# PaddleCV-SIG/MedicalSeg

Hardware: AMD Instinct MI355X
Metric: 3D-voxels/sec fwd+bwd, VNet 128^3 fp32 (higher is better)
Workload: dtype f32

## Files before the change

include/msegk.h:

```cpp
#ifndef MSEGK_H
#define MSEGK_H

#include <stddef.h>
#include <stdint.h>

#ifdef __cplusplus
extern "C" {
#endif

typedef struct msk_ctx msk_ctx;

typedef struct {
  void* p;
  int32_t n, d, h, w, c;
  int32_t ld;
} msk_tensor;

typedef struct {
  int32_t kd, kh, kw;
  int32_t sd, sh, sw;
  int32_t pd, ph, pw;
} msk_conv_desc;

int msk_version(void);
// ... 20 lines not shown
int msk_timer_start(msk_ctx* ctx);
int msk_timer_stop(msk_ctx* ctx, float* ms);
int msk_mark(msk_ctx* ctx, int idx );
int msk_mark_elapsed(msk_ctx* ctx, int a, int b, float* ms);
int msk_ctx_wait(msk_ctx* ctx, msk_ctx* other);
int msk_prof_enable(msk_ctx* ctx, int on);
int msk_prof_reset(msk_ctx* ctx);
int msk_prof_report(msk_ctx* ctx, char* buf, int buflen, int* len);
int msk_set_option(msk_ctx* ctx, const char* key, int value);
int msk_get_option(msk_ctx* ctx, const char* key, int* value);

int msk_ncdhw_to_ndhwc(msk_ctx* ctx, const float* src, msk_tensor dst);
int msk_ndhwc_to_ncdhw(msk_ctx* ctx, msk_tensor src, float* dst);

int msk_conv3d_fwd(msk_ctx* ctx, msk_conv_desc cd, msk_tensor x, const float* w,
                   const float* bias , msk_tensor y);
int msk_conv_fold_bn(msk_ctx* ctx, const float* w, const float* bias, const float* scale, const float* shift,
                     int cout, long inner, float* w_folded, float* b_folded);
int msk_conv3d_fwd_act(msk_ctx* ctx, msk_conv_desc cd, msk_tensor x, const float* w, const float* bias,
                       const float* prelu_slope, msk_tensor y);
size_t msk_conv3d_xform_bytes(msk_ctx* ctx, msk_conv_desc cd, msk_tensor x, int cout);
int msk_conv3d_fwd_ex(msk_ctx* ctx, msk_conv_desc cd, msk_tensor x, const float* w, const float* bias ,
                      msk_tensor y, float* stats_local , void* xform );
int msk_conv3d_wgrad_ex(msk_ctx* ctx, msk_conv_desc cd, msk_tensor x, msk_tensor dy, float* dw, float* db ,
                        int accumulate, const void* xform );
float* msk_amax_new(msk_ctx* ctx, int n );
int msk_conv3d_fwd_ex2(msk_ctx* ctx, msk_conv_desc cd, msk_tensor x, const float* w, const float* bias ,
                       msk_tensor y, float* stats_local , void* xform , const float* x_amax );
int msk_affine_act_fwd_amax(msk_ctx* ctx, msk_tensor x, const float* scale, const float* shift, msk_tensor res,
                            const float* alpha, msk_tensor out, float* out_amax);
int msk_affine_act_join_fwd_amax(msk_ctx* ctx, msk_tensor y, const float* scale, const float* shift, const float* alpha_inner,
                                 msk_tensor res, const float* alpha_outer, msk_tensor out, float* out_amax);
int msk_copy_scale_amax(msk_ctx* ctx, msk_tensor src, const float* mask, msk_tensor dst, int accumulate, float* dst_amax);
int msk_conv3d_dgrad_ex(msk_ctx* ctx, msk_conv_desc cd, msk_tensor dy, const float* w, msk_tensor dx, int accumulate,
                        const float* dy_amax );
int msk_conv3d_wgrad_ex2(msk_ctx* ctx, msk_conv_desc cd, msk_tensor x, msk_tensor dy, float* dw, float* db ,
                         int accumulate, const void* xform , const float* dy_amax );
int msk_conv3d_wgrad_ex3(msk_ctx* ctx, msk_conv_desc cd, msk_tensor x, msk_tensor dy, float* dw, float* db ,
                         int accumulate, const void* xform , const float* dy_amax , const float* x_amax );
typedef struct msk_bn_fin {
  const float* gamma;
  const float* beta;
  float eps, momentum;
  double count;
  float* running_mean;
  float* running_var;
  float* save_mean;
  float* save_invstd;
  float* scale;
  float* shift;
} msk_bn_fin;
int msk_conv3d_fwd_ex3(msk_ctx* ctx, msk_conv_desc cd, msk_tensor x, const float* w, const float* bias ,
                       msk_tensor y, float* stats_local , void* xform , const float* x_amax ,
                       const msk_bn_fin* fin );
int msk_bn_stats_fin(msk_ctx* ctx, msk_tensor x, float* stats_local, const msk_bn_fin* fin );
int msk_conv3d_fwd_in(msk_ctx* ctx, msk_conv_desc cd, msk_tensor x, const float* w, const float* bias , msk_tensor y,
                      float* stats, void* xform , const float* x_amax , const msk_bn_fin* fin,
                      int fin_stride);
int msk_affine_act_bwd_reduce_pg(msk_ctx* ctx, msk_tensor x, const float* scale, const float* shift, msk_tensor res,
                                 const float* alpha, const float* mean, const float* invstd, msk_tensor dout, float* sums,
                                 float* maxes , int clear_maxes, float* dgamma, float* dbeta, float* dalpha);
int msk_add_act_join_bwd_pg(msk_ctx* ctx, msk_tensor y, const float* scale, const float* shift, const float* alpha_inner,
                            msk_tensor res, const float* alpha_outer, const float* mean, const float* invstd, msk_tensor dout,
                            msk_tensor da, msk_tensor dres, int dres_accumulate, float* dalpha_outer, float* unit_sums,
                            float* maxes , int clear_maxes, float* unit_dgamma, float* unit_dbeta, float* unit_dalpha);
size_t msk_conv3d_bwd_bnact_bytes(msk_ctx* ctx, msk_conv_desc cd, msk_tensor x, msk_tensor y);
int msk_conv3d_bwd_bnact(msk_ctx* ctx, msk_conv_desc cd, msk_tensor x, const float* w, msk_tensor y, const float* scale,
                         const float* shift, const float* alpha , const float* mean, const float* invstd,
                         const float* gamma, msk_tensor dout, const float* sums_total, double M_total,
                         msk_tensor dy_scratch, msk_tensor dx, int dx_accumulate, float* dw, int dw_accumulate,
                         const void* xform , void* ybuf ,
                         const float* maxes );
int msk_conv3d_bwd_bnact_split(msk_ctx* ctx, msk_conv_desc cd, msk_tensor x, const float* w, msk_tensor y, const float* scale,
                               const float* shift, const float* alpha , const float* mean, const float* invstd,
                               const float* gamma, msk_tensor dout, const float* sums_total, double M_total,
                               msk_tensor dy_scratch, msk_tensor dx, int dx_accumulate, float* dw, int dw_accumulate,
                               const void* xform , void* ybuf , const float* maxes ,
                               msk_tensor dx_lo, msk_tensor dx_hi, int* split_done);
int msk_conv3d_bwd_bnact_acc(msk_ctx* ctx, msk_conv_desc cd, msk_tensor x, const float* w, msk_tensor y, const float* scale,
                             const float* shift, const float* alpha, const float* mean, const float* invstd, const float* gamma,
                             msk_tensor dout, const float* sums_total, double M_total, msk_tensor dy_scratch, msk_tensor dx,
                             int dx_accumulate, float* dw, int dw_accumulate, const void* xform, void* ybuf, const float* maxes,
                             msk_tensor dx_old, msk_tensor dx_lo, msk_tensor dx_hi, int* split_done);
int msk_conv3d_bwd_bnact_join(msk_ctx* ctx, msk_conv_desc cd, msk_tensor x, const float* w, msk_tensor y, const float* scale,
                              const float* shift, const float* alpha , const float* mean, const float* invstd,
                              const float* gamma, msk_tensor dout, const float* sums_total, double M_total, msk_tensor dy,
                              float* dy_amax , float* dw, int dw_accumulate, const void* xform ,
                              const float* x_amax , msk_tensor jy, const float* jscale, const float* jshift,
                              const float* jalpha_inner, msk_tensor jres, const float* jalpha_outer, const float* jmean,
                              const float* jinvstd, msk_tensor da, int da_accumulate, msk_tensor dres ,
                              int dres_accumulate, float* dalpha_outer, float* unit_sums, float* maxes, int clear_maxes,
                              float* unit_dgamma , float* unit_dbeta , float* unit_dalpha );
int msk_convT3d_bwd_bnact(msk_ctx* ctx, msk_conv_desc cd, msk_tensor x, const float* w, msk_tensor y, const float* scale,
                          const float* shift, const float* alpha , const float* mean, const float* invstd,
                          msk_tensor dout, const float* sums_total, double M_total, msk_tensor dy_scratch, msk_tensor dx,
                          int dx_accumulate, float* dw, int dw_accumulate);
int msk_conv3d_bwd_inact(msk_ctx* ctx, msk_conv_desc cd, msk_tensor x, const float* w, msk_tensor y, const float* scale,
                         const float* shift, const float* alpha , const float* mean, const float* invstd, int coef_stride,
                         msk_tensor dout, const float* sums, int sums_stride, double M_sample, msk_tensor dx, int dx_accumulate,
                         float* dw, int dw_accumulate, const void* xform, void* ybuf, const float* maxes );
int msk_conv3d_bwd_bnact_c1(msk_ctx* ctx, msk_conv_desc cd, msk_tensor x, msk_tensor y, const float* scale, const float* shift,
                            const float* alpha , const float* mean, const float* invstd, msk_tensor res,
                            msk_tensor dout, const float* sums_total, double M_total, float* dw, int dw_accumulate);
int msk_conv3d_dgrad(msk_ctx* ctx, msk_conv_desc cd, msk_tensor dy, const float* w,
                     msk_tensor dx, int accumulate);
int msk_conv3d_wgrad(msk_ctx* ctx, msk_conv_desc cd, msk_tensor x, msk_tensor dy,
                     float* dw, float* db , int accumulate);
int msk_convT3d_fwd(msk_ctx* ctx, msk_conv_desc cd, msk_tensor x, const float* w,
                    const float* bias , msk_tensor y);
int msk_convT3d_fwd_ex(msk_ctx* ctx, msk_conv_desc cd, msk_tensor x, const float* w, const float* bias, msk_tensor y,
                       float* stats_local, const msk_bn_fin* fin );
int msk_convT3d_dgrad(msk_ctx* ctx, msk_conv_desc cd, msk_tensor dy, const float* w,
                      msk_tensor dx, int accumulate);
int msk_convT3d_wgrad(msk_ctx* ctx, msk_conv_desc cd, msk_tensor x, msk_tensor dy,
                      float* dw, float* db , int accumulate);

int msk_bn_stats(msk_ctx* ctx, msk_tensor x, float* stats_local);
int msk_bn_finalize(msk_ctx* ctx, const float* gathered, int world, double count_per_rank,
                    int C, const float* gamma, const float* beta, float eps, float momentum,
                    float* running_mean, float* running_var, float* save_mean,
                    float* save_invstd, float* scale, float* shift);
int msk_bn_eval_coeffs(msk_ctx* ctx, int C, const float* gamma, const float* beta,
                       const float* running_mean, const float* running_var, float eps,
                       float* save_mean, float* save_invstd, float* scale, float* shift);
int msk_affine_act_fwd(msk_ctx* ctx, msk_tensor x, const float* scale, const float* shift,
                       msk_tensor res, const float* alpha, msk_tensor out);
int msk_affine_act_fwd_amax2(msk_ctx* ctx, msk_tensor x, const float* scale, const float* shift, msk_tensor res,
                             const float* alpha, msk_tensor out, float* out_amax , msk_tensor out2);
int msk_affine_act_bwd_reduce(msk_ctx* ctx, msk_tensor x, const float* scale, const float* shift,
                              msk_tensor res, const float* alpha, const float* mean,
                              const float* invstd, msk_tensor dout, float* sums);
int msk_affine_act_bwd_reduce_ex(msk_ctx* ctx, msk_tensor x, const float* scale, const float* shift,
                                 msk_tensor res, const float* alpha, const float* mean,
                                 const float* invstd, msk_tensor dout, float* sums, float* maxes );
int msk_affine_act_bwd_apply(msk_ctx* ctx, msk_tensor x, const float* scale, const float* shift,
                             msk_tensor res, const float* alpha, const float* mean,
                             const float* invstd, const float* gamma, msk_tensor dout,
                             const float* sums_total, double M_total, int bn_mode,
                             msk_tensor dx, msk_tensor dres, int dres_acc);
int msk_affine_act_bwd_apply_amax(msk_ctx* ctx, msk_tensor x, const float* scale, const float* shift,
                                  msk_tensor res, const float* alpha, const float* mean,
                                  const float* invstd, const float* gamma, msk_tensor dout,
                                  const float* sums_total, double M_total, int bn_mode,
                                  msk_tensor dx, msk_tensor dres, int dres_acc, float* dx_amax );
int msk_affine_act_param_grads(msk_ctx* ctx, int C, const float* sums, float* dgamma,
                               float* dbeta, float* dalpha, int accumulate);

int msk_copy_scale(msk_ctx* ctx, msk_tensor src, const float* mask, msk_tensor dst, int accumulate);
int msk_dropout_mask(msk_ctx* ctx, uint64_t seed, uint64_t step, uint32_t site, int count,
                     float p, float* mask);
int msk_channel_sum(msk_ctx* ctx, msk_tensor x, float* out, int accumulate);
int msk_argmax_c(msk_ctx* ctx, msk_tensor x, int32_t* out);
int msk_softmax_c(msk_ctx* ctx, msk_tensor x, msk_tensor out);

int msk_flip_axes(msk_ctx* ctx, msk_tensor src, msk_tensor dst, int mask);
int msk_tta_accumulate(msk_ctx* ctx, msk_tensor logits, int mask, msk_tensor acc, int first);
int msk_tta_finish(msk_ctx* ctx, msk_tensor acc, int passes, msk_tensor probs, int32_t* pred);

int msk_sw_gather(msk_ctx* ctx, msk_tensor vol, msk_tensor patches, const int32_t* origins, float cval);
int msk_sw_accumulate(msk_ctx* ctx, msk_tensor logits, const int32_t* origins, const float* td, int nd, const float* th, int nh,
                      const float* tw, int nw, msk_tensor acc);

int msk_class_weights(msk_ctx* ctx, msk_tensor logits, float* weights);
int msk_loss_fwd(msk_ctx* ctx, msk_tensor logits, const int32_t* labels, const float* weights,
                 int ignore_index, float* out, double* stats);
int msk_loss_bwd(msk_ctx* ctx, msk_tensor logits, const int32_t* labels, const float* weights,
// ... 100 lines not shown
```

medicalseg_amd/_lib.py:

```python
from __future__ import annotations

import ctypes as C
import os

_HERE = os.path.dirname(os.path.abspath(__file__))
LIB_PATH = os.environ.get("MSEGK_LIB") or os.path.join(_HERE, "lib", "libmsegk.so")


class MskError(RuntimeError):
    pass


class MskTensor(C.Structure):
    _fields_ = [("p", C.c_void_p), ("n", C.c_int32), ("d", C.c_int32), ("h", C.c_int32),
                ("w", C.c_int32), ("c", C.c_int32), ("ld", C.c_int32)]


class MskConvDesc(C.Structure):
    _fields_ = [("kd", C.c_int32), ("kh", C.c_int32), ("kw", C.c_int32),
                ("sd", C.c_int32), ("sh", C.c_int32), ("sw", C.c_int32),
                ("pd", C.c_int32), ("ph", C.c_int32), ("pw", C.c_int32)]


class MskBnFin(C.Structure):
    _fields_ = [("gamma", C.c_void_p), ("beta", C.c_void_p), ("eps", C.c_float), ("momentum", C.c_float),
                ("count", C.c_double), ("running_mean", C.c_void_p), ("running_var", C.c_void_p),
                ("save_mean", C.c_void_p), ("save_invstd", C.c_void_p), ("scale", C.c_void_p), ("shift", C.c_void_p)]


NULL_TENSOR = MskTensor(None, 0, 0, 0, 0, 0, 0)

_vp, _i, _f, _d, _sz = C.c_void_p, C.c_int, C.c_float, C.c_double, C.c_size_t
_u64, _u32 = C.c_uint64, C.c_uint32
_T, _CD = MskTensor, MskConvDesc

SIGNATURES = {
    "msk_version": (_i, []),
    "msk_device_count": (_i, [C.POINTER(_i)]),
    "msk_ctx_create": (_i, [_i, C.POINTER(_vp)]),
    "msk_ctx_destroy": (_i, [_vp]),
    "msk_last_error": (C.c_char_p, [_vp]),
    "msk_sync": (_i, [_vp]),
    "msk_join_side": (_i, [_vp]),
    "msk_device_name": (_i, [_vp, C.c_char_p, _i]),
    "msk_device_pci_bus_id": (_i, [_vp, C.c_char_p, _i]),
    "msk_malloc": (_i, [_vp, _sz, C.POINTER(_vp)]),
    "msk_free": (_i, [_vp, _vp]),
    "msk_memset": (_i, [_vp, _vp, _i, _sz]),
    "msk_weights_changed": (_i, [_vp, _vp, _sz]),
    "msk_h2d": (_i, [_vp, _vp, _vp, _sz]),
    "msk_d2h": (_i, [_vp, _vp, _vp, _sz]),
    "msk_h2d_async": (_i, [_vp, _vp, _vp, _sz]),
    "msk_d2d": (_i, [_vp, _vp, _vp, _sz]),
    "msk_pinned_alloc": (_i, [_vp, _sz, C.POINTER(_vp)]),
    "msk_pinned_free": (_i, [_vp, _vp]),
    "msk_mem_info": (_i, [_vp, C.POINTER(_sz), C.POINTER(_sz)]),
    "msk_timer_start": (_i, [_vp]),
    "msk_timer_stop": (_i, [_vp, C.POINTER(_f)]),
    "msk_mark": (_i, [_vp, _i]),
    "msk_ctx_wait": (_i, [_vp, _vp]),
    "msk_mark_elapsed": (_i, [_vp, _i, _i, C.POINTER(_f)]),
    "msk_prof_enable": (_i, [_vp, _i]),
    "msk_prof_reset": (_i, [_vp]),
    "msk_prof_report": (_i, [_vp, C.c_char_p, _i, C.POINTER(_i)]),
    "msk_set_option": (_i, [_vp, C.c_char_p, _i]),
    "msk_get_option": (_i, [_vp, C.c_char_p, C.POINTER(_i)]),
    "msk_ncdhw_to_ndhwc": (_i, [_vp, _vp, _T]),
    "msk_ndhwc_to_ncdhw": (_i, [_vp, _T, _vp]),
    "msk_conv3d_fwd": (_i, [_vp, _CD, _T, _vp, _vp, _T]),
    "msk_conv_fold_bn": (_i, [_vp, _vp, _vp, _vp, _vp, _i, C.c_long, _vp, _vp]),
    "msk_conv3d_fwd_act": (_i, [_vp, _CD, _T, _vp, _vp, _vp, _T]),
    "msk_conv3d_xform_bytes": (_sz, [_vp, _CD, _T, _i]),
    "msk_conv3d_fwd_ex": (_i, [_vp, _CD, _T, _vp, _vp, _T, _vp, _vp]),
    "msk_conv3d_wgrad_ex": (_i, [_vp, _CD, _T, _T, _vp, _vp, _i, _vp]),
    "msk_amax_new": (_vp, [_vp, _i]),
    "msk_conv3d_fwd_ex3": (_i, [_vp, _CD, _T, _vp, _vp, _T, _vp, _vp, _vp, _vp]),
    "msk_conv3d_fwd_in": (_i, [_vp, _CD, _T, _vp, _vp, _T, _vp, _vp, _vp, _vp, _i]),
    "msk_bn_stats_fin": (_i, [_vp, _T, _vp, _vp]),
    "msk_affine_act_bwd_reduce_pg": (_i, [_vp, _T, _vp, _vp, _T, _vp, _vp, _vp, _T, _vp, _vp, _i, _vp, _vp, _vp]),
    "msk_add_act_join_bwd_pg": (_i, [_vp, _T, _vp, _vp, _vp, _T, _vp, _vp, _vp, _T, _T, _T, _i, _vp, _vp, _vp, _i, _vp, _vp, _vp]),
    "msk_conv3d_fwd_ex2": (_i, [_vp, _CD, _T, _vp, _vp, _T, _vp, _vp, _vp]),
    "msk_affine_act_fwd_amax": (_i, [_vp, _T, _vp, _vp, _T, _vp, _T, _vp]),
    "msk_affine_act_fwd_amax2": (_i, [_vp, _T, _vp, _vp, _T, _vp, _T, _vp, _T]),
    "msk_affine_act_join_fwd_amax": (_i, [_vp, _T, _vp, _vp, _vp, _T, _vp, _T, _vp]),
    "msk_copy_scale_amax": (_i, [_vp, _T, _vp, _T, _i, _vp]),
    "msk_conv3d_bwd_bnact_bytes": (_sz, [_vp, _CD, _T, _T]),
    "msk_conv3d_bwd_bnact": (_i, [_vp, _CD, _T, _vp, _T, _vp, _vp, _vp, _vp, _vp, _vp, _T, _vp, _d, _T, _T, _i, _vp, _i, _vp, _vp, _vp]),
    "msk_convT3d_bwd_bnact": (_i, [_vp, _CD, _T, _vp, _T, _vp, _vp, _vp, _vp, _vp, _T, _vp, _d, _T, _T, _i, _vp, _i]),
    "msk_conv3d_bwd_bnact_split": (_i, [_vp, _CD, _T, _vp, _T, _vp, _vp, _vp, _vp, _vp, _vp, _T, _vp, _d, _T, _T, _i, _vp, _i, _vp, _vp, _vp, _T, _T, C.POINTER(_i)]),
    "msk_conv3d_bwd_bnact_acc": (_i, [_vp, _CD, _T, _vp, _T, _vp, _vp, _vp, _vp, _vp, _vp, _T, _vp, _d, _T, _T, _i, _vp, _i, _vp, _vp, _vp, _T, _T, _T, C.POINTER(_i)]),
    "msk_conv3d_bwd_inact": (_i, [_vp, _CD, _T, _vp, _T, _vp, _vp, _vp, _vp, _vp, _i, _T, _vp, _i, _d, _T, _i, _vp, _i, _vp, _vp, _vp]),
    "msk_conv3d_bwd_bnact_join": (_i, [_vp, _CD, _T, _vp, _T, _vp, _vp, _vp, _vp, _vp, _vp, _T, _vp, _d, _T, _vp, _vp, _i, _vp, _vp,
                                       _T, _vp, _vp, _vp, _T, _vp, _vp, _vp, _T, _i, _T, _i, _vp, _vp, _vp, _i, _vp, _vp, _vp]),
    "msk_conv3d_bwd_bnact_c1": (_i, [_vp, _CD, _T, _T, _vp, _vp, _vp, _vp, _vp, _T, _T, _vp, _d, _vp, _i]),
    "msk_conv3d_dgrad": (_i, [_vp, _CD, _T, _vp, _T, _i]),
    "msk_conv3d_dgrad_ex": (_i, [_vp, _CD, _T, _vp, _T, _i, _vp]),
    "msk_conv3d_wgrad_ex2": (_i, [_vp, _CD, _T, _T, _vp, _vp, _i, _vp, _vp]),
    "msk_conv3d_wgrad_ex3": (_i, [_vp, _CD, _T, _T, _vp, _vp, _i, _vp, _vp, _vp]),
    "msk_conv3d_wgrad": (_i, [_vp, _CD, _T, _T, _vp, _vp, _i]),
    "msk_convT3d_fwd": (_i, [_vp, _CD, _T, _vp, _vp, _T]),
    "msk_convT3d_fwd_ex": (_i, [_vp, _CD, _T, _vp, _vp, _T, _vp, _vp]),
    "msk_convT3d_dgrad": (_i, [_vp, _CD, _T, _vp, _T, _i]),
    "msk_convT3d_wgrad": (_i, [_vp, _CD, _T, _T, _vp, _vp, _i]),
    "msk_bn_stats": (_i, [_vp, _T, _vp]),
    "msk_bn_finalize": (_i, [_vp, _vp, _i, _d, _i, _vp, _vp, _f, _f, _vp, _vp, _vp, _vp, _vp, _vp]),
    "msk_bn_eval_coeffs": (_i, [_vp, _i, _vp, _vp, _vp, _vp, _f, _vp, _vp, _vp, _vp]),
    "msk_affine_act_fwd": (_i, [_vp, _T, _vp, _vp, _T, _vp, _T]),
    "msk_affine_act_bwd_reduce": (_i, [_vp, _T, _vp, _vp, _T, _vp, _vp, _vp, _T, _vp]),
    "msk_affine_act_bwd_reduce_ex": (_i, [_vp, _T, _vp, _vp, _T, _vp, _vp, _vp, _T, _vp, _vp]),
    "msk_affine_act_bwd_apply": (_i, [_vp, _T, _vp, _vp, _T, _vp, _vp, _vp, _vp, _T, _vp, _d, _i, _T, _T, _i]),
    "msk_affine_act_bwd_apply_amax": (_i, [_vp, _T, _vp, _vp, _T, _vp, _vp, _vp, _vp, _T, _vp, _d, _i, _T, _T, _i, _vp]),
    "msk_affine_act_param_grads": (_i, [_vp, _i, _vp, _vp, _vp, _vp, _i]),
    "msk_add_act_bwd": (_i, [_vp, _T, _T, _vp, _T, _T, _T, _i, _vp]),
    "msk_affine_act_join_fwd": (_i, [_vp, _T, _vp, _vp, _vp, _T, _vp, _T]),
    "msk_add_act_join_bwd": (_i, [_vp, _T, _vp, _vp, _vp, _T, _vp, _T, _T, _T, _i, _vp]),
    "msk_add_act_join_bwd_ex": (_i, [_vp, _T, _vp, _vp, _vp, _T, _vp, _vp, _vp, _T, _T, _T, _i, _vp, _vp, _vp]),
    "msk_bn_bias_grad": (_i, [_vp, _i, _vp, _vp, _vp, _i]),
    "msk_copy_scale": (_i, [_vp, _T, _vp, _T, _i]),
    "msk_dropout_mask": (_i, [_vp, _u64, _u64, _u32, _i, _f, _vp]),
    "msk_channel_sum": (_i, [_vp, _T, _vp, _i]),
    "msk_argmax_c": (_i, [_vp, _T, _vp]),
    "msk_softmax_c": (_i, [_vp, _T, _T]),
    "msk_flip_axes": (_i, [_vp, _T, _T, _i]),
    "msk_tta_accumulate": (_i, [_vp, _T, _i, _T, _i]),
    "msk_tta_finish": (_i, [_vp, _T, _i, _T, _vp]),
    "msk_sw_gather": (_i, [_vp, _T, _T, _vp, _f]),
    "msk_sw_accumulate": (_i, [_vp, _T, _vp, _vp, _i, _vp, _i, _vp, _i, _T]),
    "msk_class_weights": (_i, [_vp, _T, _vp]),
    "msk_loss_fwd": (_i, [_vp, _T, _vp, _vp, _i, _vp, _vp]),
    "msk_loss_bwd": (_i, [_vp, _T, _vp, _vp, _i, _vp, _f, _f, _T]),
    "msk_elu_fwd": (_i, [_vp, _T, _f, _T]),
    "msk_elu_bwd": (_i, [_vp, _T, _T, _f, _T, _i]),
    "msk_loss_fwd_ex": (_i, [_vp, _T, _vp, _vp, _i, _i, _vp, _vp, _vp]),
    "msk_loss_bwd_ex": (_i, [_vp, _T, _vp, _vp, _i, _i, _vp, _vp, _f, _f, _T]),
    "msk_bce_fwd": (_i, [_vp, _T, _vp, _i, _i, _i, _f, _vp, _vp]),
    "msk_bce_bwd": (_i, [_vp, _T, _vp, _i, _vp, _f, _i, _T]),
    "msk_sgd_momentum": (_i, [_vp, _vp, _vp, _vp, _sz, _f, _f, _f, _f]),
    "msk_sgd_momentum_eager": (_i, [_vp, _vp, _vp, _vp, _sz, _f, _f, _f, _f]),
    "msk_sgd_momentum_finish": (_i, [_vp]),
    "msk_adam": (_i, [_vp, _vp, _vp, _vp, _vp, _sz, _f, _f, _f, _f, _d, _d, _f, _f]),
    "msk_resample3d": (_i, [_vp, _vp, _i, _i, _i, _vp, _i, _i, _i, _i, _i]),
    "msk_crop_resample3d": (_i, [_vp, _vp, _i, _i, _i, _i, _i, _i, _i, _i, _i, _vp, _i, _i, _i, _i, _i]),
    "msk_flip3d": (_i, [_vp, _vp, _vp, _i, _i, _i, _i, _i]),
    "msk_rotate3d": (_i, [_vp, _vp, _vp, _i, _i, _i, _i, _i, _d, _i, _d, _i]),
    "msk_hu_norm": (_i, [_vp, _vp, _vp, _sz, _f, _f, _f]),
    "msk_minmax_norm": (_i, [_vp, _vp, _vp, _sz, _i, _f, _f]),
    "msk_max_norm": (_i, [_vp, _vp, _vp, _sz]),
    "msk_label_remap": (_i, [_vp, _vp, _sz, _vp, _vp, _i]),
    "msk_connected_components3d": (_i, [_vp, _vp, _vp, _i, _i, _i, _i, _i, _i, _i, _vp, _vp]),
    "msk_confusion3d": (_i, [_vp, _vp, _vp, _i, C.c_long, _i, _i, _vp, _i]),
    "msk_auc_pack": (_i, [_vp, _T, _vp, _vp, C.c_long, C.c_long, _vp]),
    "msk_auc_workspace": (_i, [C.c_long, _i, C.POINTER(_sz)]),
    "msk_auc_counts": (_i, [_vp, _vp, C.c_long, C.c_long, _i, _vp, _sz, _vp]),
    "msk_edt3d": (_i, [_vp, _vp, _i, _i, _i, _i, _i, _vp, _vp]),
    "msk_surface_count": (_i, [_vp, _vp, _i, _i, _i, _i, _vp]),
    "msk_surface_gather": (_i, [_vp, _vp, _i, _i, _i, _i, _vp, _vp, C.c_long, _vp]),
    "msk_interp_trilinear_fwd": (_i, [_vp, _T, _T]),
    "msk_interp_scratch_bytes": (_i, [_vp, _T, _T, C.POINTER(_sz)]),
    "msk_interp_trilinear_bwd": (_i, [_vp, _T, _T, _i, _vp, _sz]),
    "msk_dp_unique_id": (_i, [C.c_char_p]),
    "msk_dp_rccl_version": (_i, [C.POINTER(_i)]),
    "msk_dp_init": (_i, [_vp, C.c_char_p, _i, _i]),
    "msk_dp_allreduce_sum": (_i, [_vp, _vp, _sz]),
    "msk_dp_allreduce_stats": (_i, [_vp, _vp, _sz]),
    "msk_dp_allreduce_async": (_i, [_vp, _vp, _sz]),
    "msk_dp_wait": (_i, [_vp]),
    "msk_dp_allgather": (_i, [_vp, _vp, _vp, _sz]),
    "msk_dp_broadcast": (_i, [_vp, _vp, _sz, _i]),
    "msk_dp_barrier": (_i, [_vp]),
    "msk_dp_destroy": (_i, [_vp]),
}

UNIQUE_ID_BYTES = 128
# ... 38 lines not shown
```

medicalseg_amd/csrc/msk_common.h:

```cpp
#pragma once
#include <hip/hip_runtime.h>
#include <hip/hip_ext.h>

#include <cstdint>
#include <cstdio>
#include <cstring>
#include <map>
#include <set>
#include <string>
#include <utility>
#include <vector>

#include "msegk.h"

struct msk_prof_entry {
  double total_ms = 0.0;
  long calls = 0;
};

struct msk_pending_event {
  hipEvent_t a, b;
  const char* tag;
};

// ... 27 lines not shown
  bool xform_written = false;
  std::set<const void*> xform_ok;
  bool conv_fp16 = false;
  int wbf_tin_map = 1;
  int wbf_mr4 = 1;
  int wbf_variant = -1;
  int halo_tile = -1;
  int wgrad_chunk = -1;
  char prof_prefix[48] = {0};
  long wgrad_async_max_m = 0;
  float* scalar_ring = nullptr;
  int scalar_next = 0;
  long scalar_served = 0;
  float* scalar_ring_side = nullptr;
  int scalar_next_side = 0;
  long scalar_served_side = 0;
  int wbf_tpb = 0;
  void* wpack = nullptr;
  int wbf_pack_cache = 1;
  void* spack = nullptr;
  int wbf_pack_lds = 1;
  int wbf_bpf = 1;
  int wbf_ks_blocks = 2;
  int noop_after_merge = 0;
  int wgrad_c1_wpc = 2;
  int eager_tail_main = 1;
  int prof_paused = 0;
  int prof_attach = 1;
  int small_pack_cache = 1;
  int wbf_prepack = 1;
  int ks_legacy = 0;
  int wgrad_fork = 1;
  int wbf_fused_bl = 2;
  int wbf_fuse = 1;
  int conv_split = 2;
  int bwd_fuse = -1;
  int foldn_wgs = 0;
  int wgrad_wino_rounds = 0;
  int wgrad_rounds = 8;
  int poison = -1;
  hipStream_t side = nullptr;
  void* ws_side = nullptr;
  size_t ws_side_bytes = 0;
  void* ws3_side = nullptr;
  size_t ws3_side_bytes = 0;
  hipEvent_t ev_fork = nullptr, ev_join = nullptr;
  hipEvent_t ev_late = nullptr;
  bool late_valid = false;
  const float* late_ptr = nullptr;
  size_t late_count = 0;
  float* late_alpha = nullptr;
  struct { float* param = nullptr; const float* grad = nullptr; float* velocity = nullptr; size_t count = 0;
           float lr = 0, momentum = 0, weight_decay = 0, grad_scale = 0; } late_piece;
  int late_split = 1;
  bool wgrad_async = false;
  bool side_dirty = false;
  hipEvent_t fork_event = nullptr;
  int fork_attach = 1;
  bool fork_recorded = false;
  void* stage[2] = {nullptr, nullptr};
  size_t stage_bytes[2] = {0, 0};
  hipEvent_t stage_ev[2] = {nullptr, nullptr};
  int stage_next = 0;
  void* comm = nullptr;
  void* comm_grad = nullptr;
  hipStream_t comm_stream = nullptr;
  hipEvent_t ev_comm_main = nullptr, ev_comm_side = nullptr, ev_comm_done = nullptr, ev_comm_back = nullptr;
  int c1_h2 = 1;
  int dst_split = 1;
  int wgrad_reduce_rows = 1;
  int ks_stats = 1;
  int ks_lds = 1;
  int ks_nr_max = 4;
  int wgrad_lds_pad = 0;
  int kst_pair = 1;
  int tile_staging = 7;
  int wgrad_renorm = 1;
  int dy_bound_shift = 0;
  int dp_mode = 0;
  bool comm_pending = false;
  bool host_transport = false;
  std::vector<int> host_fds;
  int rank = 0, world = 1;
  int tk_join = 1;
  int num_cu = 256;
};

extern thread_local std::string g_msk_global_err;

int msk_fail(msk_ctx* ctx, const char* file, int line, const char* what, const char* detail);
void* msk_workspace(msk_ctx* ctx, size_t bytes);
void* msk_workspace2(msk_ctx* ctx, size_t bytes);
void* msk_workspace3(msk_ctx* ctx, size_t bytes);
hipEvent_t msk_prof_event(msk_ctx* ctx);
void msk_prof_begin(msk_ctx* ctx, const char* tag);
void msk_prof_end(msk_ctx* ctx);
const char* msk_intern_tag(msk_ctx* ctx, const std::string& s);
int msk_join_side_impl(msk_ctx* ctx);
void msk_set_dense12(int v);
void msk_set_reduce_vpl(int v);
void msk_set_reduce_vpl_site(int v);
void msk_set_ew_caps(int ew, int red);
void msk_weights_changed_impl(msk_ctx* ctx, const void* p, size_t bytes);
void msk_weights_freed_impl(msk_ctx* ctx, const void* p, size_t bytes);
int msk_wbf_prepack_impl(msk_ctx* ctx);
int msk_wbf_prepack_range_impl(msk_ctx* ctx, const void* p, size_t bytes);
void msk_wbf_pack_cache_free(msk_ctx* ctx);
void msk_small_pack_changed(msk_ctx* ctx, const void* p, size_t bytes);
void msk_small_pack_freed(msk_ctx* ctx, const void* p, size_t bytes);
int msk_small_prepack(msk_ctx* ctx, const void* p, size_t bytes);
void msk_small_pack_free(msk_ctx* ctx);
int msk_dp_wait_impl(msk_ctx* ctx);
int msk_join_sums_merge(msk_ctx* ctx, const float* partial, int nb, int C, float* unit_sums, float* u_dbeta, float* u_dgamma,
                        float* u_dalpha, float* dalpha);

struct msk_side_scope {
  msk_ctx* ctx;
  bool active;
  explicit msk_side_scope(msk_ctx* c, bool want = true) : ctx(c), active(want && c->wgrad_async && c->side != nullptr) {
    const bool forked = ctx->fork_recorded;
    hipEvent_t fev = forked && ctx->fork_event ? ctx->fork_event : ctx->ev_fork;
    ctx->fork_recorded = false;
    ctx->fork_event = nullptr;
    if (!active) return;
    if (!forked) hipEventRecord(ctx->ev_fork, ctx->stream);
    hipStreamWaitEvent(ctx->side, fev, 0);
    std::swap(ctx->stream, ctx->side);
    std::swap(ctx->ws, ctx->ws_side);
    std::swap(ctx->ws_bytes, ctx->ws_side_bytes);
    std::swap(ctx->ws3, ctx->ws3_side);
    std::swap(ctx->ws3_bytes, ctx->ws3_side_bytes);
    std::swap(ctx->scalar_ring, ctx->scalar_ring_side);
    std::swap(ctx->scalar_next, ctx->scalar_next_side);
    std::swap(ctx->scalar_served, ctx->scalar_served_side);
    ctx->side_dirty = true;
  }
  ~msk_side_scope() {
    if (!active) return;
    std::swap(ctx->stream, ctx->side);
    std::swap(ctx->ws, ctx->ws_side);
    std::swap(ctx->ws_bytes, ctx->ws_side_bytes);
    std::swap(ctx->ws3, ctx->ws3_side);
    std::swap(ctx->ws3_bytes, ctx->ws3_side_bytes);
    std::swap(ctx->scalar_ring, ctx->scalar_ring_side);
    std::swap(ctx->scalar_next, ctx->scalar_next_side);
    std::swap(ctx->scalar_served, ctx->scalar_served_side);
  }
};

#define MSK_CHECK_HIP(ctx, expr)                                                        \
  do {                                                                                  \
    hipError_t _e = (expr);                                                             \
    if (_e != hipSuccess) return msk_fail(ctx, __FILE__, __LINE__, #expr, hipGetErrorString(_e)); \
  } while (0)

#define MSK_REQUIRE(ctx, cond, msg)                                       \
  do {                                                                    \
    if (!(cond)) return msk_fail(ctx, __FILE__, __LINE__, #cond, msg);    \
  } while (0)

static inline bool msk_prof_selected(const msk_ctx* c, const char* tag) {
  return c->prof && ((!c->prof_paused && (c->prof_prefix[0] == 0 || strncmp(tag, c->prof_prefix, strlen(c->prof_prefix)) == 0)) ||
                     strncmp(tag, "rccl_", 5) == 0);
}
struct msk_launch_scope {
  msk_ctx* ctx;
// ... 71 lines not shown
```

medicalseg_amd/csrc/msk_conv.h:

```cpp
#pragma once
#include "msk_common.h"
struct WbfBnBwd;

struct GConv {
  const float* src;
  int sld;
  float* dst;
  int dld;
  int N, SD, SH, SW, DD, DH, DW;
  int CK, CN;
  int kd, kh, kw, sd, sh, sw, pd, ph, pw;
  int transposed;
  const float* bias;
  int accumulate;
  int flip;
  float* stats;
  void* xform;
  const float* w_amax;
  const float* in_amax;
  const struct WbfBnBwd* fuse;
  const msk_bn_fin* fin;
  int ck_real;
  int stats_ps;
  int fin_stride;
  bool w_persistent;
  float* dst_lo;
  float* dst_hi;
  int dst_csplit;
  const float* acc_src;
  const float* prelu;
};

struct WGrad {
  const float* A;
  int ald;
  const float* B;
  int bld;
  int N, AD, AH, AW, BD, BH, BW;
  int CA, CB;
  int kd, kh, kw, sd, sh, sw, pd, ph, pw;
  const void* xform;
  const void* yform;
  const float* y_amax;
  const float* y_cmax;
  const float* b_amax;
  int cb_real;
  const float* a_amax;
  const struct WbfBnBwd* yfuse;
  float* dw;
  int accumulate;
  float* db;
  int db_src;
  long vsn;
  int vsd, vsh, vsw;
};

int msk_pack_weights(msk_ctx* ctx, const float* w, int A, int B, int taps, int swap, int flip_taps,
                     int kd, int kh, int kw, int mfma, int K, int N, int KC, int npad, float* out);

const float* msk_pack_weights_get(msk_ctx* ctx, const float* w, int A, int B, int taps, int swap, int flip_taps, int kd, int kh,
                                  int kw, int mfma, int K, int N, int KC, int npad);
const float* msk_pack_scatter_get(msk_ctx* ctx, const float* w, int A, int B, int taps, int swap, int CK, int CN, int KC, int jpad);

int msk_gconv_halo_mfma(msk_ctx* ctx, const GConv& g, const float* w_canon, int A, int B, int swap);
int msk_gconv_gather_mfma(msk_ctx* ctx, const GConv& g, const float* w_canon, int A, int B, int swap);
int msk_gconv_halo_tightk(msk_ctx* ctx, const GConv& g, const float* w_canon, int A, int B, int swap);
int msk_gconv_tk_h2(msk_ctx* ctx, const GConv& g, const float* w_canon, int A, int B, int swap, struct TKJoin* join = nullptr);
struct TKJoin {
  const float* x;
  int xld;
  const float* b;
  int bld;
  float* db;
  int dbld;
  const float *scale, *shift, *alpha_in, *alpha, *mean, *invstd;
  float* maxes;
  const float* partial;
  int nb;
};
bool msk_gconv_tk_h2_accepts(const msk_ctx* ctx, const GConv& g, const struct TKJoin* join);
int msk_gconv_c1_mfma(msk_ctx* ctx, const GConv& g, const float* w_canon, int A, int B, int swap);
int msk_gconv_c1_h2(msk_ctx* ctx, const GConv& g, const float* w_canon, int A, int B, int swap);
int msk_gconv_halo_valu2(msk_ctx* ctx, const GConv& g, const float* w_canon, int A, int B, int swap);
int msk_gconv_halo_foldn(msk_ctx* ctx, const GConv& g, const float* w_canon, int A, int B, int swap, bool* act_fused);
int msk_gconv_halo_wino(msk_ctx* ctx, const GConv& g, const float* w_canon, int A, int B, int swap);
int msk_gconv_wino_bf3(msk_ctx* ctx, const GConv& g, const float* w_canon, int A, int B, int swap);
bool msk_gconv_wino_bf3_accepts(msk_ctx* ctx, const GConv& g);
int msk_wgrad_wbf(msk_ctx* ctx, const WGrad& g);
bool msk_wgrad_wbf_accepts(msk_ctx* ctx, const WGrad& g);
bool msk_wgrad_wbf_fusable(msk_ctx* ctx, const WGrad& g, size_t* y_bytes);
int msk_gconv_scatter_mfma(msk_ctx* ctx, const GConv& g, const float* w_canon, int A, int B, int swap);
int msk_gconv_ks_fwd(msk_ctx* ctx, const GConv& g, const float* w_canon, int A, int B, int swap);
int msk_gconv_ks_fwd_bnbwd(msk_ctx* ctx, const GConv& g, const float* w_canon, int A, int B, int swap, const float* y, int yld,
                           const float* dout, int dld, const float* scale, const float* shift, const float* alpha, const float* mean,
                           const float* invstd, const float* sums, double M_total, bool dry);
int msk_gconv_kst(msk_ctx* ctx, const GConv& g, const float* w_canon, int A, int B, int swap);
int msk_wgrad_mfma(msk_ctx* ctx, const WGrad& g);
bool msk_gconv_foldn_h2_accepts(const msk_ctx* ctx, msk_conv_desc cd, msk_tensor x, int cout);
int msk_wgrad_cbs(msk_ctx* ctx, const WGrad& g);
int msk_wgrad_c1(msk_ctx* ctx, const WGrad& g);
int msk_wgrad_ks(msk_ctx* ctx, const WGrad& g);
int msk_wgrad_wino(msk_ctx* ctx, const WGrad& g);

const float* msk_absmax(msk_ctx* ctx, const float* x, int ld, int C, long voxels, float* dst = nullptr);
float* msk_scalar_slots(msk_ctx* ctx, int n);
const float* msk_bn_bwd_bound(msk_ctx* ctx, int C, const float* scale, const float* sums, double M_total, const float* maxes);
int msk_wgrad_reduce_ex(msk_ctx* ctx, const float* partial, int splits, long pitch, int taps, int CA, int CB, float* dw,
                        int accumulate, int nbias, float* db, int db_accumulate);
int msk_wgrad_reduce(msk_ctx* ctx, const float* partial, int splits, int taps, int CA, int CB, float* dw,
                     int accumulate);
```

medicalseg_amd/csrc/msk_conv.hip:

```cpp
#include "msk_conv.h"
#include "msk_wbf.h"

namespace {

constexpr int kThreads = 256;

__device__ __forceinline__ float pack_weights_elem(const float* __restrict__ w, int B, int taps, int swap, int flip, int kd, int kh,
                                                   int kw, int mfma, int K, int N, int KC, int npad, long idx) {
  int tap, k, n;
  if (mfma) {
    int q = (int)(idx & 3);
    long r = idx >> 2;
    n = (int)(r % npad);
    r /= npad;
    int h = (int)(r & 1);
    r >>= 1;
    int kc = (int)(r % KC);
    tap = (int)(r / KC);
    k = kc * 8 + h * 4 + q;
  } else {
    const int NP = npad > 0 ? npad : N;
    n = (int)(idx % NP);
    long r = idx / NP;
    k = (int)(r % K);
// ... 1467 lines not shown
int msk_conv3d_wgrad(msk_ctx* ctx, msk_conv_desc cd, msk_tensor x, msk_tensor dy, float* dw, float* db, int accumulate) {
  if (check_conv_shapes(ctx, cd, x, dy, false) != 0) return -1;
  msk_side_scope side(ctx, ctx->wgrad_async_max_m <= 0 || msk_voxels(dy) <= ctx->wgrad_async_max_m);
  WGrad g{};
  g.A = (const float*)x.p; g.ald = x.ld; g.B = (const float*)dy.p; g.bld = dy.ld;
  g.N = x.n; g.AD = x.d; g.AH = x.h; g.AW = x.w; g.BD = dy.d; g.BH = dy.h; g.BW = dy.w;
  g.CA = x.c; g.CB = dy.c;
  g.kd = cd.kd; g.kh = cd.kh; g.kw = cd.kw; g.sd = cd.sd; g.sh = cd.sh; g.sw = cd.sw;
  g.pd = cd.pd; g.ph = cd.ph; g.pw = cd.pw;
  g.dw = dw; g.accumulate = accumulate;
  return run_wgrad(ctx, g, dy, db, accumulate);
}

}

static int bwd_bnact_c1(msk_ctx* ctx, const WGrad& gw, msk_tensor y, const float* scale, const float* shift, const float* alpha,
                        const float* mean, const float* invstd, msk_tensor dout, const float* sums_total, double M_total,
                        int res_is_input) {
  if (ctx->bwd_fuse == 0 || ctx->conv_impl != 0) return 1;
  if (gw.BW * 4 < ((gw.BW + 31) / 32) * 32 * 3) return 1;
  WbfBnBwd bn{};
  bn.y = (const float*)y.p; bn.yld = y.ld; bn.dout = (const float*)dout.p; bn.dld = dout.ld;
  bn.scale = scale; bn.shift = shift; bn.alpha = alpha; bn.mean = mean; bn.invstd = invstd; bn.sums = sums_total;
  bn.invM = (float)(1.0 / M_total);
  bn.res_is_input = res_is_input;
  WGrad gc = gw;
  gc.B = nullptr;
  gc.xform = nullptr;
  gc.yfuse = &bn;
  if (ctx->late_split && ctx->wgrad_async && ctx->side != nullptr) {
    msk_side_scope side(ctx, true);
    if (side.active) {
      if (!ctx->late_alpha) MSK_CHECK_HIP(ctx, hipMalloc((void**)&ctx->late_alpha, 1024 * sizeof(float)));
      if (alpha && gw.CB <= 1024) {
        MSK_CHECK_HIP(ctx, hipMemcpyAsync(ctx->late_alpha, alpha, (size_t)gw.CB * sizeof(float), hipMemcpyDeviceToDevice, ctx->stream));
        bn.alpha = ctx->late_alpha;
      }
      hipEventRecord(ctx->ev_late, ctx->stream);
    }
    const int r = msk_wgrad_c1(ctx, gc);
    if (r == 1 && side.active) {
      ctx->late_valid = true;
      ctx->late_ptr = gw.dw;
      ctx->late_count = (size_t)gw.CA * gw.CB * gw.kd * gw.kh * gw.kw;
    }
    return r < 0 ? r : (r == 1 ? 0 : 1);
  }
  const int r = msk_wgrad_c1(ctx, gc);
  return r < 0 ? r : (r == 1 ? 0 : 1);
}

extern "C" {

int msk_conv3d_bwd_bnact_c1(msk_ctx* ctx, msk_conv_desc cd, msk_tensor x, msk_tensor y, const float* scale, const float* shift,
                            const float* alpha, const float* mean, const float* invstd, msk_tensor res, msk_tensor dout,
                            const float* sums_total, double M_total, float* dw, int dw_accumulate) {
  if (check_conv_shapes(ctx, cd, x, y, false) != 0) return -1;
  MSK_REQUIRE(ctx, scale && shift && mean && invstd && sums_total && M_total > 0, "training-mode BatchNorm coefficients required");
  MSK_REQUIRE(ctx, dout.n == y.n && dout.d == y.d && dout.h == y.h && dout.w == y.w && dout.c == y.c, "dout must match y");
  if (x.c != 1) return 1;
  if (res.p && !(res.p == x.p && res.ld == x.ld && res.c == 1 && res.n == x.n && res.d == x.d && res.h == x.h && res.w == x.w)) return 1;
  const size_t per = (size_t)x.d * x.h * x.w * (x.ld > y.ld ? x.ld : y.ld) * sizeof(float);
  if (per > 0 && (size_t)x.n > kChunkBytes / per) return 1;
  WGrad gw{};
  gw.A = (const float*)x.p; gw.ald = x.ld; gw.bld = y.ld;
  gw.N = x.n; gw.AD = x.d; gw.AH = x.h; gw.AW = x.w; gw.BD = y.d; gw.BH = y.h; gw.BW = y.w;
  gw.CA = x.c; gw.CB = y.c;
  gw.kd = cd.kd; gw.kh = cd.kh; gw.kw = cd.kw; gw.sd = cd.sd; gw.sh = cd.sh; gw.sw = cd.sw;
  gw.pd = cd.pd; gw.ph = cd.ph; gw.pw = cd.pw;
  gw.dw = dw; gw.accumulate = dw_accumulate;
  return bwd_bnact_c1(ctx, gw, y, scale, shift, alpha, mean, invstd, dout, sums_total, M_total, res.p ? 1 : 0);
}

size_t msk_conv3d_bwd_bnact_bytes(msk_ctx* ctx, msk_conv_desc cd, msk_tensor x, msk_tensor y) {
  if (x.c != y.c || x.d != y.d || x.h != y.h || x.w != y.w) return 0;
  return msk_conv3d_xform_bytes(ctx, cd, y, y.c);
}

static int conv3d_bwd_bnact_impl(msk_ctx* ctx, msk_conv_desc cd, msk_tensor x, const float* w, msk_tensor y, const float* scale,
                                 const float* shift, const float* alpha, const float* mean, const float* invstd, const float* gamma,
                                 msk_tensor dout, const float* sums_total, double M_total, msk_tensor dy_scratch, msk_tensor dx,
                                 int dx_accumulate, float* dw, int dw_accumulate, const void* xform, void* ybuf, const float* maxes,
                                 int coef_stride, int sums_stride, bool fused_only, float* dx_lo = nullptr, float* dx_hi = nullptr,
                                 int dx_csplit = 0, const float* dx_old = nullptr);

int msk_conv3d_bwd_bnact(msk_ctx* ctx, msk_conv_desc cd, msk_tensor x, const float* w, msk_tensor y, const float* scale,
                         const float* shift, const float* alpha, const float* mean, const float* invstd, const float* gamma,
                         msk_tensor dout, const float* sums_total, double M_total, msk_tensor dy_scratch, msk_tensor dx,
                         int dx_accumulate, float* dw, int dw_accumulate, const void* xform, void* ybuf, const float* maxes) {
  return conv3d_bwd_bnact_impl(ctx, cd, x, w, y, scale, shift, alpha, mean, invstd, gamma, dout, sums_total, M_total, dy_scratch, dx,
                               dx_accumulate, dw, dw_accumulate, xform, ybuf, maxes, 0, 0, false);
}

int msk_conv3d_bwd_bnact_split(msk_ctx* ctx, msk_conv_desc cd, msk_tensor x, const float* w, msk_tensor y, const float* scale,
                               const float* shift, const float* alpha, const float* mean, const float* invstd, const float* gamma,
                               msk_tensor dout, const float* sums_total, double M_total, msk_tensor dy_scratch, msk_tensor dx,
                               int dx_accumulate, float* dw, int dw_accumulate, const void* xform, void* ybuf, const float* maxes,
                               msk_tensor dx_lo, msk_tensor dx_hi, int* split_done) {
  MSK_REQUIRE(ctx, split_done != nullptr, "msk_conv3d_bwd_bnact_split: split_done required");
  *split_done = 0;
  const bool ok = dx.p && dx_lo.p && dx_hi.p && dx.c % 2 == 0 && dx_lo.c == dx.c / 2 && dx_hi.c == dx.c / 2 && dx_lo.ld == dx.c / 2 &&
                  dx_hi.ld == dx.c / 2 && dx.ld == dx.c && msk_voxels(dx_lo) == msk_voxels(dx) && msk_voxels(dx_hi) == msk_voxels(dx) &&
                  dx_accumulate && ctx->dst_split != 0;
  const int rc = conv3d_bwd_bnact_impl(ctx, cd, x, w, y, scale, shift, alpha, mean, invstd, gamma, dout, sums_total, M_total, dy_scratch, dx,
                                       dx_accumulate, dw, dw_accumulate, xform, ybuf, maxes, 0, 0, false, ok ? (float*)dx_lo.p : nullptr,
                                       ok ? (float*)dx_hi.p : nullptr, ok ? dx.c / 2 : 0);
  if (rc == 0 && ctx->dst_split_done) *split_done = 1;
  ctx->dst_split_done = false;
  return rc;
}

int msk_conv3d_bwd_bnact_acc(msk_ctx* ctx, msk_conv_desc cd, msk_tensor x, const float* w, msk_tensor y, const float* scale,
                             const float* shift, const float* alpha, const float* mean, const float* invstd, const float* gamma,
                             msk_tensor dout, const float* sums_total, double M_total, msk_tensor dy_scratch, msk_tensor dx,
                             int dx_accumulate, float* dw, int dw_accumulate, const void* xform, void* ybuf, const float* maxes,
                             msk_tensor dx_old, msk_tensor dx_lo, msk_tensor dx_hi, int* split_done) {
  if (split_done) *split_done = 0;
  if (dx_old.p) {
    MSK_REQUIRE(ctx, dx.p && dx_old.n == dx.n && dx_old.d == dx.d && dx_old.h == dx.h && dx_old.w == dx.w && dx_old.c == dx.c &&
                         dx_old.ld == dx.ld && dx_old.p != dx.p, "dx_old must have the geometry and voxel stride of dx");
    dx_accumulate = 1;
  }
  const bool ok = split_done && dx.p && dx_lo.p && dx_hi.p && dx.c % 2 == 0 && dx_lo.c == dx.c / 2 && dx_hi.c == dx.c / 2 &&
                  dx_lo.ld == dx.c / 2 && dx_hi.ld == dx.c / 2 && dx.ld == dx.c && msk_voxels(dx_lo) == msk_voxels(dx) &&
                  msk_voxels(dx_hi) == msk_voxels(dx) && dx_accumulate && ctx->dst_split != 0;
  const int rc = conv3d_bwd_bnact_impl(ctx, cd, x, w, y, scale, shift, alpha, mean, invstd, gamma, dout, sums_total, M_total, dy_scratch, dx,
                                       dx_accumulate, dw, dw_accumulate, xform, ybuf, maxes, 0, 0, false, ok ? (float*)dx_lo.p : nullptr,
                                       ok ? (float*)dx_hi.p : nullptr, ok ? dx.c / 2 : 0, (const float*)dx_old.p);
  if (rc == 0 && ok && ctx->dst_split_done) *split_done = 1;
  ctx->dst_split_done = false;
  return rc;
}

int msk_conv3d_bwd_bnact_join(msk_ctx* ctx, msk_conv_desc cd, msk_tensor x, const float* w, msk_tensor y, const float* scale,
                              const float* shift, const float* alpha, const float* mean, const float* invstd, const float* gamma,
                              msk_tensor dout, const float* sums_total, double M_total, msk_tensor dy, float* dy_amax, float* dw,
                              int dw_accumulate, const void* xform, const float* x_amax, msk_tensor jy, const float* jscale,
                              const float* jshift, const float* jalpha_inner, msk_tensor jres, const float* jalpha_outer,
                              const float* jmean, const float* jinvstd, msk_tensor da, int da_accumulate, msk_tensor dres,
                              int dres_accumulate, float* dalpha_outer, float* unit_sums, float* maxes, int clear_maxes,
                              float* unit_dgamma, float* unit_dbeta, float* unit_dalpha) {
  if (check_conv_shapes(ctx, cd, x, y, false) != 0) return -1;
  MSK_REQUIRE(ctx, scale && shift && mean && invstd && sums_total && M_total > 0 && w && dw, "training-mode BatchNorm coefficients required");
  MSK_REQUIRE(ctx, dy.p && dy.n == y.n && dy.d == y.d && dy.h == y.h && dy.w == y.w && dy.c == y.c, "dy must match y");
  MSK_REQUIRE(ctx, jscale && jshift && jalpha_inner && jalpha_outer && jmean && jinvstd && dalpha_outer && unit_sums && maxes,
              "the join's coefficients, statistics, sums and maxima buffers");
  const bool same = jy.n == x.n && jy.d == x.d && jy.h == x.h && jy.w == x.w && jy.c == x.c && jres.n == x.n && jres.d == x.d &&
                    jres.h == x.h && jres.w == x.w && jres.c == x.c && da.n == x.n && da.d == x.d && da.h == x.h && da.w == x.w &&
                    da.c == x.c && jy.p && jres.p && da.p;
  MSK_REQUIRE(ctx, same, "the join's tensors must have the shape of x");
  MSK_REQUIRE(ctx, !dres.p || (dres.n == x.n && dres.d == x.d && dres.h == x.h && dres.w == x.w && dres.c == x.c), "dres must have the shape of x");
  if (ctx->conv_impl != 0 || x.c != 32 || da_accumulate || (dres.p && dres_accumulate)) return 1;
  GConv g{};
  g.src = (const float*)dy.p; g.sld = dy.ld; g.dst = (float*)da.p; g.dld = da.ld;
  g.N = x.n; g.SD = dy.d; g.SH = dy.h; g.SW = dy.w; g.DD = x.d; g.DH = x.h; g.DW = x.w;
  g.CK = dy.c; g.CN = x.c;
  g.kd = cd.kd; g.kh = cd.kh; g.kw = cd.kw; g.sd = cd.sd; g.sh = cd.sh; g.sw = cd.sw;
  g.pd = cd.pd; g.ph = cd.ph; g.pw = cd.pw;
  g.transposed = 1; g.bias = nullptr; g.accumulate = 0; g.flip = 1;
  g.w_persistent = true;
  g.in_amax = dy_amax;
  TKJoin j{};
  j.x = (const float*)jy.p; j.xld = jy.ld; j.b = (const float*)jres.p; j.bld = jres.ld;
  j.scale = jscale; j.shift = jshift; j.alpha_in = jalpha_inner; j.alpha = jalpha_outer; j.mean = jmean; j.invstd = jinvstd;
  j.maxes = maxes;
  j.db = (float*)dres.p; j.dbld = dres.ld;
  const size_t per = (size_t)x.d * x.h * x.w * (x.ld > da.ld ? x.ld : da.ld) * sizeof(float);
  if (per > 0 && (size_t)x.n > kChunkBytes / per) return 1;
  if ((size_t)x.n * x.d * x.h * x.w >= (1ull << 31) / 64) return 1;
  if (!msk_gconv_tk_h2_accepts(ctx, g, &j)) return 1;
  if (int rc = msk_affine_act_bwd_apply_amax(ctx, y, scale, shift, msk_tensor{}, alpha, mean, invstd, gamma, dout, sums_total, M_total, 1,
                                             dy, msk_tensor{}, 0, dy_amax))
    return rc;
  if (int rc = conv3d_wgrad_impl(ctx, cd, x, dy, dw, nullptr, dw_accumulate, xform, dy_amax, x_amax)) return rc;
  if (clear_maxes) MSK_CHECK_HIP(ctx, hipMemsetAsync(maxes, 0, 2 * kWbfAmaxWays * sizeof(float), ctx->stream));
  const int r = msk_gconv_tk_h2(ctx, g, w, dy.c, x.c, 0, &j);
  if (r < 0) return r;
  if (r == 0) return msk_fail(ctx, __FILE__, __LINE__, "msk_conv3d_bwd_bnact_join", "the data-gradient kernel declined a problem its plan accepted");
  return msk_join_sums_merge(ctx, j.partial, j.nb, x.c, unit_sums, unit_dbeta, unit_dgamma, unit_dalpha, dalpha_outer);
}

int msk_conv3d_bwd_inact(msk_ctx* ctx, msk_conv_desc cd, msk_tensor x, const float* w, msk_tensor y, const float* scale,
                         const float* shift, const float* alpha, const float* mean, const float* invstd, int coef_stride,
                         msk_tensor dout, const float* sums, int sums_stride, double M_sample, msk_tensor dx, int dx_accumulate,
                         float* dw, int dw_accumulate, const void* xform, void* ybuf, const float* maxes) {
  MSK_REQUIRE(ctx, coef_stride >= y.c && sums_stride >= 2 * y.c, "msk_conv3d_bwd_inact: strides smaller than the records");
  return conv3d_bwd_bnact_impl(ctx, cd, x, w, y, scale, shift, alpha, mean, invstd, nullptr, dout, sums, M_sample, msk_tensor{}, dx,
                               dx_accumulate, dw, dw_accumulate, xform, ybuf, maxes, coef_stride, sums_stride, true);
}

static int conv3d_bwd_bnact_impl(msk_ctx* ctx, msk_conv_desc cd, msk_tensor x, const float* w, msk_tensor y, const float* scale,
                                 const float* shift, const float* alpha, const float* mean, const float* invstd, const float* gamma,
                                 msk_tensor dout, const float* sums_total, double M_total, msk_tensor dy_scratch, msk_tensor dx,
                                 int dx_accumulate, float* dw, int dw_accumulate, const void* xform, void* ybuf, const float* maxes,
                                 int coef_stride, int sums_stride, bool fused_only, float* dx_lo, float* dx_hi, int dx_csplit,
                                 const float* dx_old) {
  if (check_conv_shapes(ctx, cd, x, y, false) != 0) return -1;
  ctx->dst_split_done = false;
  if (!dx_accumulate || !dx.p) dx_old = nullptr;
  MSK_REQUIRE(ctx, scale && shift && mean && invstd && sums_total && M_total > 0, "training-mode BatchNorm coefficients required");
  MSK_REQUIRE(ctx, dout.n == y.n && dout.d == y.d && dout.h == y.h && dout.w == y.w && dout.c == y.c, "dout must match y");
  MSK_REQUIRE(ctx, fused_only || (dy_scratch.p && dy_scratch.n == y.n && dy_scratch.d == y.d && dy_scratch.h == y.h && dy_scratch.w == y.w &&
                                  dy_scratch.c == y.c), "dy_scratch must match y");
  if (xform && !ctx->xform_ok.count(xform)) xform = nullptr;
  const bool split2 = wbf_pieces(ctx, cd.kd) != 3;
  bool fused = ctx->bwd_fuse != 0 && (!split2 || maxes != nullptr) && ybuf != nullptr && xform != nullptr && dx.p != nullptr && ctx->wbf && !ctx->no_winograd && ctx->conv_impl == 0 &&
               x.c == y.c && y.ld % 4 == 0 && dout.ld % 4 == 0 && (((uintptr_t)y.p) & 15) == 0 && (((uintptr_t)dout.p) & 15) == 0;
  const size_t per = (size_t)x.d * x.h * x.w * (x.ld > y.ld ? x.ld : y.ld) * sizeof(float);
  if (per > 0 && (size_t)x.n > kChunkBytes / per) fused = false;
  WGrad gw{};
  gw.A = (const float*)x.p; gw.ald = x.ld; gw.B = (const float*)dy_scratch.p; gw.bld = dy_scratch.ld;
  gw.N = x.n; gw.AD = x.d; gw.AH = x.h; gw.AW = x.w; gw.BD = y.d; gw.BH = y.h; gw.BW = y.w;
  gw.CA = x.c; gw.CB = y.c;
  gw.kd = cd.kd; gw.kh = cd.kh; gw.kw = cd.kw; gw.sd = cd.sd; gw.sh = cd.sh; gw.sw = cd.sw;
  gw.pd = cd.pd; gw.ph = cd.ph; gw.pw = cd.pw;
  gw.dw = dw; gw.accumulate = dw_accumulate;
  gw.xform = xform;
  if (x.c == 1 && !dx.p && !fused_only && !(per > 0 && (size_t)x.n > kChunkBytes / per)) {
    const int r = bwd_bnact_c1(ctx, gw, y, scale, shift, alpha, mean, invstd, dout, sums_total, M_total, 0);
    if (r <= 0) return r;
  }
  size_t y_bytes = 0;
  if (fused && !msk_wgrad_wbf_fusable(ctx, gw, &y_bytes)) fused = false;
  if (fused) {
    GConv g{};
    g.src = (const float*)dy_scratch.p; g.sld = dy_scratch.ld; g.dst = (float*)dx.p; g.dld = dx.ld;
    g.N = dx.n; g.SD = y.d; g.SH = y.h; g.SW = y.w; g.DD = dx.d; g.DH = dx.h; g.DW = dx.w;
    g.CK = y.c; g.CN = dx.c;
    g.kd = cd.kd; g.kh = cd.kh; g.kw = cd.kw; g.sd = cd.sd; g.sh = cd.sh; g.sw = cd.sw;
    g.pd = cd.pd; g.ph = cd.ph; g.pw = cd.pw;
    g.transposed = 1; g.bias = nullptr; g.accumulate = dx_accumulate; g.flip = 1;
    g.w_persistent = true;
    g.dst_lo = dx_lo; g.dst_hi = dx_hi; g.dst_csplit = dx_csplit;
    g.acc_src = dx_old;
    WbfBnBwd bn{};
    bn.y = (const float*)y.p; bn.yld = y.ld; bn.dout = (const float*)dout.p; bn.dld = dout.ld;
    bn.scale = scale; bn.shift = shift; bn.alpha = alpha; bn.mean = mean; bn.invstd = invstd; bn.sums = sums_total;
    bn.invM = (float)(1.0 / M_total);
    bn.Y = (char*)ybuf;
    bn.coef_stride = coef_stride; bn.sums_stride = sums_stride;
    bn.y_xi = (long)(y_bytes / ((cd.kd == 5) ? 8 : 6));
    if (split2) g.w_amax = (const float*)xform + kWbfAmaxWays;

    const bool side_on = ctx->wgrad_async && ctx->side != nullptr &&
                         (ctx->wgrad_async_max_m <= 0 || msk_voxels(y) <= ctx->wgrad_async_max_m);
    int form = ctx->bwd_fuse > 0 ? ctx->bwd_fuse : ((side_on && !split2) ? 2 : 1);
    if (fused_only) form = 1;
    if (fused_only && split2 && !maxes) return 1;
    if (wbf_pieces(ctx, cd.kd) == 2 && form == 1) {
      bn.y_cmax = msk_scalar_slots(ctx, (y.c + kWbfAmaxWays - 1) / kWbfAmaxWays);
      if (!bn.y_cmax) return -1;
    }
    if (split2) {
      if (form == 1) {
        float* slot = msk_scalar_slots(ctx, 1);
        if (!slot) return -1;
        bn.amax = slot;
        bn.maxes = maxes;
      } else {
        bn.amax = msk_bn_bwd_bound(ctx, y.c, scale, sums_total, M_total, maxes);
        if (!bn.amax) return -1;
      }
    }
    if (form == 2) {
      bn.Y = nullptr;
      g.fuse = &bn;
      if (msk_gconv_wino_bf3_accepts(ctx, g)) {
        {
          msk_side_scope side(ctx, side_on);
          gw.yfuse = &bn;
          const int rw = msk_wgrad_wbf(ctx, gw);
          if (rw < 0) return rw;
          if (rw == 0) return msk_fail(ctx, __FILE__, __LINE__, "msk_conv3d_bwd_bnact", "weight-gradient pipeline declined a problem its plan accepted");
        }
        const int r = msk_gconv_wino_bf3(ctx, g, w, y.c, x.c, 0);
        if (r < 0) return r;
        if (r == 0) return msk_fail(ctx, __FILE__, __LINE__, "msk_conv3d_bwd_bnact", "data-gradient pipeline declined a problem its plan accepted");
        return 0;
      }
    } else {
      g.fuse = &bn;
      const int r = msk_gconv_wino_bf3(ctx, g, w, y.c, x.c, 0);
      if (r < 0) return r;
      if (r == 1) {
        msk_side_scope side(ctx, side_on);
        gw.yform = ybuf;
        gw.y_amax = bn.amax;
        gw.y_cmax = bn.y_cmax;
        const int rw = msk_wgrad_wbf(ctx, gw);
        if (rw < 0) return rw;
        if (rw == 0) return msk_fail(ctx, __FILE__, __LINE__, "msk_conv3d_bwd_bnact", "weight-gradient pipeline declined a problem its plan accepted");
        return 0;
      }
    }
  }
  if (fused_only) return 1;
  (void)gamma;
  if (dx_old) {
    msk_tensor so = dx;
    so.p = (void*)dx_old;
    if (int rc = msk_copy_scale(ctx, so, nullptr, dx, 0)) return rc;
  }
  if (int rc = msk_affine_act_bwd_apply(ctx, y, scale, shift, msk_tensor{}, alpha, mean, invstd, gamma, dout, sums_total, M_total, 1,
                                        dy_scratch, msk_tensor{}, 0))
    return rc;
  const float* dy_amax = nullptr;
  if (ctx->conv_split == 2 && ctx->conv_impl == 0 && y.c <= 4 && cd.kd == 5 && cd.kh == 5 && cd.kw == 5) {
    dy_amax = msk_absmax(ctx, (const float*)dy_scratch.p, dy_scratch.ld, dy_scratch.c, msk_voxels(dy_scratch));
    if (!dy_amax) return -1;
  }
  if (int rc = conv3d_wgrad_impl(ctx, cd, x, dy_scratch, dw, nullptr, dw_accumulate, xform, dy_amax)) return rc;
  if (dx.p) return conv3d_dgrad_impl(ctx, cd, dy_scratch, w, dx, dx_accumulate, dy_amax);
  return 0;
}

int msk_convT3d_fwd(msk_ctx* ctx, msk_conv_desc cd, msk_tensor x, const float* w, const float* bias, msk_tensor y) {
  if (check_conv_shapes(ctx, cd, x, y, true) != 0) return -1;
  GConv g{};
  g.src = (const float*)x.p; g.sld = x.ld; g.dst = (float*)y.p; g.dld = y.ld;
  g.N = x.n; g.SD = x.d; g.SH = x.h; g.SW = x.w; g.DD = y.d; g.DH = y.h; g.DW = y.w;
  g.CK = x.c; g.CN = y.c;
  g.kd = cd.kd; g.kh = cd.kh; g.kw = cd.kw; g.sd = cd.sd; g.sh = cd.sh; g.sw = cd.sw;
  g.pd = 0; g.ph = 0; g.pw = 0;
  g.transposed = 1; g.bias = bias; g.accumulate = 0; g.flip = 0;
  return run_gconv(ctx, g, w, x.c, y.c, 0, "convT3d_fwd_direct");
}

int msk_convT3d_fwd_ex(msk_ctx* ctx, msk_conv_desc cd, msk_tensor x, const float* w, const float* bias, msk_tensor y,
                       float* stats_local, const msk_bn_fin* fin) {
  if (check_conv_shapes(ctx, cd, x, y, true) != 0) return -1;
  if (fin && !fin->scale) fin = nullptr;
  MSK_REQUIRE(ctx, stats_local != nullptr, "msk_convT3d_fwd_ex: stats_local required");
  GConv g{};
  g.src = (const float*)x.p; g.sld = x.ld; g.dst = (float*)y.p; g.dld = y.ld;
  g.N = x.n; g.SD = x.d; g.SH = x.h; g.SW = x.w; g.DD = y.d; g.DH = y.h; g.DW = y.w;
  g.CK = x.c; g.CN = y.c;
  g.kd = cd.kd; g.kh = cd.kh; g.kw = cd.kw; g.sd = cd.sd; g.sh = cd.sh; g.sw = cd.sw;
  g.pd = 0; g.ph = 0; g.pw = 0;
  g.transposed = 1; g.bias = bias; g.accumulate = 0; g.flip = 0;
  g.w_persistent = true;
  const size_t sper = (size_t)g.SD * g.SH * g.SW * g.sld * sizeof(float), dper = (size_t)g.DD * g.DH * g.DW * g.dld * sizeof(float);
  const size_t per = sper > dper ? sper : dper;
  const bool chunked = per > 0 && (size_t)g.N > kChunkBytes / per;
  ctx->stats_fused = false;
  if (!chunked) {
    g.stats = stats_local;
    g.fin = fin;
  }
  if (int rc = run_gconv(ctx, g, w, x.c, y.c, 0, "convT3d_fwd_direct")) return rc;
  if (!ctx->stats_fused) return msk_bn_stats_fin(ctx, y, stats_local, fin);
  return 0;
}

int msk_convT3d_dgrad(msk_ctx* ctx, msk_conv_desc cd, msk_tensor dy, const float* w, msk_tensor dx, int accumulate) {
  if (check_conv_shapes(ctx, cd, dx, dy, true) != 0) return -1;
  GConv g{};
  g.src = (const float*)dy.p; g.sld = dy.ld; g.dst = (float*)dx.p; g.dld = dx.ld;
  g.N = dx.n; g.SD = dy.d; g.SH = dy.h; g.SW = dy.w; g.DD = dx.d; g.DH = dx.h; g.DW = dx.w;
  g.CK = dy.c; g.CN = dx.c;
  g.kd = cd.kd; g.kh = cd.kh; g.kw = cd.kw; g.sd = cd.sd; g.sh = cd.sh; g.sw = cd.sw;
  g.pd = 0; g.ph = 0; g.pw = 0;
  g.transposed = 0; g.bias = nullptr; g.accumulate = accumulate; g.flip = 0;
  return run_gconv(ctx, g, w, dx.c, dy.c, 1, "convT3d_dgrad_direct");
}

int msk_convT3d_bwd_bnact(msk_ctx* ctx, msk_conv_desc cd, msk_tensor x, const float* w, msk_tensor y, const float* scale,
                          const float* shift, const float* alpha, const float* mean, const float* invstd, msk_tensor dout,
                          const float* sums_total, double M_total, msk_tensor dy, msk_tensor dx, int dx_accumulate, float* dw,
                          int dw_accumulate) {
  if (check_conv_shapes(ctx, cd, x, y, true) != 0) return -1;
  MSK_REQUIRE(ctx, scale && shift && mean && invstd && sums_total && w && dw, "msk_convT3d_bwd_bnact: null argument");
  MSK_REQUIRE(ctx, dout.c == y.c && msk_voxels(dout) == msk_voxels(y) && dy.c == y.c && msk_voxels(dy) == msk_voxels(y) &&
                       dx.c == x.c && msk_voxels(dx) == msk_voxels(x), "msk_convT3d_bwd_bnact: shape mismatch");
  GConv g{};
  g.src = (const float*)y.p; g.sld = y.ld; g.dst = (float*)dx.p; g.dld = dx.ld;
  g.N = dx.n; g.SD = y.d; g.SH = y.h; g.SW = y.w; g.DD = dx.d; g.DH = dx.h; g.DW = dx.w;
  g.CK = y.c; g.CN = dx.c;
  g.kd = cd.kd; g.kh = cd.kh; g.kw = cd.kw; g.sd = cd.sd; g.sh = cd.sh; g.sw = cd.sw;
  g.transposed = 0; g.bias = nullptr; g.accumulate = dx_accumulate; g.flip = 0;
// ... 39 lines not shown
```

medicalseg_amd/csrc/msk_conv_wbf.hip:

```cpp
#include <type_traits>
#include "msk_wbf.h"
#ifndef WBF_TIN_SYNC
#define WBF_TIN_SYNC 1
#endif

#ifndef WBF_PROBE
#define WBF_PROBE 0
#endif
typedef _Float16 f16x8 __attribute__((ext_vector_type(8)));
typedef _Float16 f16x2 __attribute__((ext_vector_type(2)));

namespace {

constexpr int nxi_of(int K) { return K == 5 ? 8 : 6; }

__device__ __forceinline__ void split3_one(float x, unsigned short& hi, unsigned short& mid, unsigned short& lo) {
  hi = __builtin_bit_cast(unsigned short, (__bf16)x);
  const float r = x - __uint_as_float((unsigned)hi << 16);
  mid = __builtin_bit_cast(unsigned short, (__bf16)r);
  const float r2 = r - __uint_as_float((unsigned)mid << 16);
  lo = __builtin_bit_cast(unsigned short, (__bf16)r2);
}
__device__ __forceinline__ unsigned pack_f16_pair(float a, float b) {
  f32x2 v = {a, b};
// ... 740 lines not shown
      const int cur = tap & 1, nx = cur ^ 1;
      const int bcur = tap % BR;
      if (tap + BPF < T2) {
        const unsigned ub = (unsigned)(tap + BPF) * utap + ukc;
#pragma unroll
        for (int p = 0; p < NP; ++p) {
          bq[(tap + BPF) % BR][p] = buf_load16(ures, ulane, ub + p * ustep);
        }
      }
      if (tap + 1 < T2) {
#pragma unroll
        for (int mr = 0; mr < MR; ++mr) {
          const uint4* ap = lds + arow[mr] + ((tap + 1) / K) * HPt + ((tap + 1) % K);
#pragma unroll
          for (int p = 0; p < NP; ++p) {
            aq[nx][mr][p] = ap[p * 2 * NSLOT];
          }
        }
      }
      __builtin_amdgcn_sched_barrier(0);
      if (NP == 3) {
#pragma unroll
        for (int mr = 0; mr < MR; ++mr) WBF_MFMA(acc[mr], aq[cur][mr][NP - 1], bq[bcur][0]);
#pragma unroll
        for (int mr = 0; mr < MR; ++mr) WBF_MFMA(acc[mr], aq[cur][mr][0], bq[bcur][NP - 1]);
#pragma unroll
        for (int mr = 0; mr < MR; ++mr) WBF_MFMA(acc[mr], aq[cur][mr][NP / 2], bq[bcur][NP / 2]);
#pragma unroll
        for (int mr = 0; mr < MR; ++mr) WBF_MFMA(acc[mr], aq[cur][mr][NP / 2], bq[bcur][0]);
#pragma unroll
        for (int mr = 0; mr < MR; ++mr) WBF_MFMA(acc[mr], aq[cur][mr][0], bq[bcur][NP / 2]);
#pragma unroll
        for (int mr = 0; mr < MR; ++mr) WBF_MFMA(acc[mr], aq[cur][mr][0], bq[bcur][0]);
      } else if (NP == 2) {
        const uint4 bdown = wbf_hi_down(bq[bcur][0]);
#pragma unroll
        for (int mr = 0; mr < MR; ++mr) WBF_MFMA_H(acc[mr], aq[cur][mr][NP - 1], bdown);
#pragma unroll
        for (int mr = 0; mr < MR; ++mr) WBF_MFMA_H(acc[mr], aq[cur][mr][0], bq[bcur][NP - 1]);
#pragma unroll
        for (int mr = 0; mr < MR; ++mr) WBF_MFMA_H(acc[mr], aq[cur][mr][0], bq[bcur][0]);
      } else {
#pragma unroll
        for (int mr = 0; mr < MR; ++mr) WBF_MFMA_H(acc[mr], aq[cur][mr][0], bq[bcur][0]);
      }
      __builtin_amdgcn_sched_barrier(0);
    }
  }

  const int co = (grp * WN + wn) * 32 + li;
  float* mbase = a.M + ((long)ks * NXI + xi) * a.m_xi + ((long)(n * a.T + t) * a.LD) * a.LH * a.CN + co;
#pragma unroll
  for (int mr = 0; mr < MR; ++mr) {
#pragma unroll
    for (int j = 0; j < 16; ++j) {
      int fa, fb;
      frag_pos<TH>((j & 3) + 8 * (j >> 2) + 4 * lh, fa, fb);
      const int d = tdi * TD + (wm * MR + mr) * (32 / TH) + fa, h = thi * TH + fb;
      if (d < a.LD && h < a.LH) mbase[((long)d * a.LH + h) * a.CN] = acc[mr][j];
    }
  }
  }
}

struct FusedArgs {
  GemmArgs g;
  float* dst;
  int dld;
  long dvn;
  int dvd, dvh, dvw;
  const float* bias;
  const float* prelu;
  int accumulate;
  const float* in_amax;
  const float* w_amax;
  int scaled;
  float* stat_partial;
  int per_xcd;
  int LW;
  float* st_lo;
  float* st_hi;
  int csplit;
  const float* acc_src;
};

struct WfRec {
  float n, mean, m2;
};
__device__ __forceinline__ WfRec wfrec_merge(WfRec a, WfRec b) {
  if (b.n == 0.f) return a;
  if (a.n == 0.f) return b;
  WfRec r;
  r.n = a.n + b.n;
  const float d = b.mean - a.mean, f = b.n / r.n;
  r.mean = a.mean + d * f;
  r.m2 = a.m2 + b.m2 + d * d * a.n * f;
  return r;
}

template <int K>
__device__ __forceinline__ void at_column(int xi, float& c0, float& c1, float& c2, float& c3) {
  const int last = K == 5 ? 7 : 5;
  c0 = xi == last ? 0.f : 1.f;
  if (xi == 0) { c1 = c2 = c3 = 0.f; return; }
  if (xi == last) { c1 = c2 = 0.f; c3 = 1.f; return; }
  const float sg = (xi & 1) ? 1.f : -1.f;
  const int pr = (xi - 1) >> 1;
  const float p = pr == 0 ? 1.f : (pr == 1 ? 2.f : 0.5f);
  c1 = sg * p;
  c2 = p * p;
  c3 = sg * p * p * p;
}

#ifndef WBF_FUSED_BPF
#define WBF_FUSED_BPF 3
#endif
template <int MR, int WM, int WN, int TD, int TH, int K, int NP, bool STATS, int BPF = (NP == 2 ? WBF_FUSED_BPF : 1), int BL = 0>
__global__ void __launch_bounds__(WM * WN * 64, 2)
wbf_gemm_fused_k(FusedArgs f) {
  static_assert(WM * WN == 4 && WM * MR * 32 == TD * TH, "tile shape");
  const GemmArgs& a = f.g;
  constexpr int NT = WM * WN * 64;
  constexpr int NXI = nxi_of(K), T2 = K * K, PADK = (K - 1) / 2;
  constexpr int HDt = TD + K - 1, HPt = TH + K - 1, NSLOT = HDt * HPt, NPL = 2 * NP, NIT = NPL * NSLOT, ROUNDS = (NIT + NT - 1) / NT;
  constexpr int NBF = T2 * NP;
  constexpr int BROUNDS = (NBF + WM * WN - 1) / (WM * WN);
  static_assert(BL == 0 || NIT % 64 == 0, "weights through LDS: wave-granular tile");
  static_assert(BL != 1 || WN == 1, "B through LDS, whole stage: one column fragment");
  constexpr int PH = WN == 1 ? 4 : 5;
  constexpr int PQ_T[6] = {0, T2 * 1 / PH, T2 * 2 / PH, T2 * 3 / PH, PH > 4 ? T2 * 4 / PH : T2, T2};
  constexpr int PQ_FR = (T2 - PQ_T[PH - 1]) * NP * WN;
  constexpr int PQ_SLOT = PQ_FR * 64;
  static_assert(BL != 2 || (NP == 2 && WM * WN == 4 && WN <= 2 && PQ_T[1] * NP * WN >= 4), "pipelined form: fp16 x 2 pieces, four wavefronts");
  __shared__ uint4 lds[BL == 2 ? 2 * NIT + 2 * PQ_SLOT : (BL ? NIT + NBF * 64 : ROUNDS * NT)];

  const int tid = threadIdx.x;
  const int wave = __builtin_amdgcn_readfirstlane(tid >> 6), lane = tid & 63, li = lane & 31, lh = lane >> 5;
  const int wm = wave / WN, wn = wave % WN;

  int b = (blockIdx.x & 7) * f.per_xcd + (blockIdx.x >> 3);
  if ((int)(blockIdx.x >> 3) >= f.per_xcd || b >= a.nblk) return;
  const int tile_id = b;
  const int thi = b % a.tiles_h;
  b /= a.tiles_h;
  const int tdi = b % a.tiles_d;
  b /= a.tiles_d;
  const int t = b % a.T;
  const int n = b / a.T;

  unsigned voff[ROUNDS];
#pragma unroll
  for (int r = 0; r < ROUNDS; ++r) {
    int it = r * NT + tid;
    if (it >= NIT) it = 0;
    const int pk = it / NSLOT, slot = it - pk * NSLOT;
    const int row = slot / HPt, col = slot - row * HPt;
    voff[r] = (unsigned)(pk * a.v_plane + ((long)row * a.HP + col) * 16);
  }
  const char* vtile0 = a.V + ((long)(n * a.T + t) * a.KC) * NPL * a.v_plane +
                       ((long)(tdi * TD + 2 - PADK) * a.HP + thi * TH + 2 - PADK) * 16;
  const unsigned ulane = (unsigned)(lh * a.CN + wn * 32 + li) * 16u;
  const unsigned ustep = (unsigned)a.CN * 32u;
  const unsigned uchunk = (unsigned)NP * ustep;
  const unsigned utap = (unsigned)a.KC * uchunk;

  int arow[MR];
#pragma unroll
  for (int mr = 0; mr < MR; ++mr) {
    int fa, fb;
    frag_pos<TH>(li, fa, fb);
    arow[mr] = lh * NSLOT + ((wm * MR + mr) * (32 / TH) + fa) * HPt + fb;
  }

  f32x16 yo[4][MR];
#pragma unroll
  for (int i = 0; i < 4; ++i)
#pragma unroll
    for (int mr = 0; mr < MR; ++mr)
#pragma unroll
      for (int j = 0; j < 16; ++j) yo[i][mr][j] = 0.f;

  if constexpr (BL == 2) {
    const unsigned lds0 = (unsigned)(unsigned long)(__attribute__((address_space(3))) void*)lds;
    const int NS = NXI * a.KC;
    const unsigned voff_last = (ROUNDS - 1) * NT + wave * 64 < NIT ? voff[ROUNDS - 1] : voff[ROUNDS - 2];
    const int r_last = (ROUNDS - 1) * NT + wave * 64 < NIT ? ROUNDS - 1 : ROUNDS - 2;
    auto rsrc_of = [](const char* p_) {
      const unsigned long pa = (unsigned long)p_;
      i32x4 r_ = {(int)__builtin_amdgcn_readfirstlane((unsigned)pa), (int)(__builtin_amdgcn_readfirstlane((unsigned)(pa >> 32)) & 0xffffu),
                  (int)0xFFFFFFF0u, 0x00020000};
      return r_;
    };
    auto fill_tile = [&](int s_) {
      const int xi_ = s_ / a.KC, kc_ = s_ - xi_ * a.KC;
      const i32x4 vr = rsrc_of(vtile0 + (long)xi_ * a.v_xi);
      const unsigned so = (unsigned)(kc_ * NPL * a.v_plane);
      const unsigned dst = lds0 + (unsigned)((s_ & 1) * NIT + wave * 64) * 16u;
#pragma unroll
      for (int r = 0; r < ROUNDS - 1; ++r) wbf_dma16(vr, dst + (unsigned)(r * NT) * 16u, voff[r], so);
      wbf_dma16(vr, dst + (unsigned)(r_last * NT) * 16u, voff_last, so);
    };
    auto fill_weights = [&](int s_, auto qc) {
// ... 212 lines not shown
        for (int p = 0; p < NP; ++p) aq[0][mr][p] = ap[p * 2 * NSLOT];
      }
#pragma unroll
      for (int tap = 0; tap < T2; ++tap) {
        const int cur = tap & 1, nx = cur ^ 1;
        const int bcur = tap % BR;
        if (tap + BPF < T2) {
          const unsigned ub = (unsigned)(tap + BPF) * utap + ukc;
#pragma unroll
          for (int p = 0; p < NP; ++p) { if (WBF_PROBE & 2) bq[(tap + BPF) % BR][p] = bq[bcur][p]; else bq[(tap + BPF) % BR][p] = buf_load16(ures, ulane, ub + p * ustep); }
        }
        if (tap + 1 < T2) {
#pragma unroll
          for (int mr = 0; mr < MR; ++mr) {
            const uint4* ap = lds + arow[mr] + ((tap + 1) / K) * HPt + ((tap + 1) % K);
#pragma unroll
            for (int p = 0; p < NP; ++p) { if (WBF_PROBE & 4) aq[nx][mr][p] = aq[cur][mr][p]; else aq[nx][mr][p] = ap[p * 2 * NSLOT]; }
          }
        }
        __builtin_amdgcn_sched_barrier(0);
        if (NP == 3) {
#pragma unroll
          for (int mr = 0; mr < MR; ++mr) WBF_MFMA(acc[mr], aq[cur][mr][NP - 1], bq[bcur][0]);
#pragma unroll
          for (int mr = 0; mr < MR; ++mr) WBF_MFMA(acc[mr], aq[cur][mr][0], bq[bcur][NP - 1]);
#pragma unroll
          for (int mr = 0; mr < MR; ++mr) WBF_MFMA(acc[mr], aq[cur][mr][NP / 2], bq[bcur][NP / 2]);
#pragma unroll
          for (int mr = 0; mr < MR; ++mr) WBF_MFMA(acc[mr], aq[cur][mr][NP / 2], bq[bcur][0]);
#pragma unroll
          for (int mr = 0; mr < MR; ++mr) WBF_MFMA(acc[mr], aq[cur][mr][0], bq[bcur][NP / 2]);
#pragma unroll
          for (int mr = 0; mr < MR; ++mr) WBF_MFMA(acc[mr], aq[cur][mr][0], bq[bcur][0]);
        } else if (NP == 2 && (WBF_PROBE & 16)) {
#pragma unroll
          for (int mr = 0; mr < MR; ++mr)
#pragma unroll
            for (int p = 0; p < NP; ++p)
              asm volatile("" ::"v"(aq[cur][mr][p].x), "v"(aq[cur][mr][p].y), "v"(aq[cur][mr][p].z), "v"(aq[cur][mr][p].w),
                           "v"(bq[bcur][p].x), "v"(bq[bcur][p].y), "v"(bq[bcur][p].z), "v"(bq[bcur][p].w));
        } else if (NP == 2) {
          const uint4 bdown = wbf_hi_down(bq[bcur][0]);
#pragma unroll
          for (int mr = 0; mr < MR; ++mr) WBF_MFMA_H(acc[mr], aq[cur][mr][NP - 1], bdown);
#pragma unroll
          for (int mr = 0; mr < MR; ++mr) WBF_MFMA_H(acc[mr], aq[cur][mr][0], bq[bcur][NP - 1]);
#pragma unroll
          for (int mr = 0; mr < MR; ++mr) WBF_MFMA_H(acc[mr], aq[cur][mr][0], bq[bcur][0]);
        } else {
#pragma unroll
          for (int mr = 0; mr < MR; ++mr) WBF_MFMA_H(acc[mr], aq[cur][mr][0], bq[bcur][0]);
        }
        __builtin_amdgcn_sched_barrier(0);
      }
      }
    }
    float c0, c1, c2, c3;
    at_column<K>(xi, c0, c1, c2, c3);
#pragma unroll
    for (int mr = 0; mr < MR; ++mr)
#pragma unroll
      for (int j = 0; j < 16; ++j) {
        const float m = acc[mr][j];
        yo[0][mr][j] = fmaf(c0, m, yo[0][mr][j]);
        yo[1][mr][j] = fmaf(c1, m, yo[1][mr][j]);
        yo[2][mr][j] = fmaf(c2, m, yo[2][mr][j]);
        yo[3][mr][j] = fmaf(c3, m, yo[3][mr][j]);
      }
  }

  }
  const int co = wn * 32 + li;
  const float osc = f.scaled ? 1.f / (wbf_scale_of(f.in_amax) * wbf_scale_of(f.w_amax)) : 1.f;
  const float bv = f.bias ? f.bias[co] : 0.f;
  const float sl = f.prelu ? f.prelu[co] : 1.f;
  float* obase = f.dst + ((long)n * f.dvn + (long)(4 * t) * f.dvw) * f.dld + co;
  const long wst = (long)f.dvw * f.dld;
  const bool split_st = f.st_lo != nullptr;
  float* sbase = split_st ? (co < f.csplit ? f.st_lo + co : f.st_hi + (co - f.csplit)) + (((long)n * f.dvn + (long)(4 * t) * f.dvw) * f.dld >> 1) : obase;
  const long swst = split_st ? (wst >> 1) : wst;
  const long aoff = f.acc_src ? (f.acc_src - f.dst) : 0;
  const int wlim = f.LW - 4 * t;
  float sk = 0.f, s1 = 0.f, s2 = 0.f, cnt = 0.f;
#pragma unroll
  for (int mr = 0; mr < MR; ++mr) {
#pragma unroll
    for (int jq = 0; jq < 4; ++jq) {
      float* op[4];
      bool ok[4];
#pragma unroll
      for (int jj = 0; jj < 4; ++jj) {
        int fa, fb;
        frag_pos<TH>(jj + 8 * jq + 4 * lh, fa, fb);
        const int d = tdi * TD + (wm * MR + mr) * (32 / TH) + fa, h = thi * TH + fb;
        ok[jj] = d < a.LD && h < a.LH;
        op[jj] = obase + ((long)d * f.dvd + (long)h * f.dvh) * f.dld;
      }
      float old[4][4];
      if (f.accumulate) {
#pragma unroll
        for (int jj = 0; jj < 4; ++jj)
#pragma unroll
          for (int i = 0; i < 4; ++i) old[jj][i] = (ok[jj] && i < wlim) ? __builtin_nontemporal_load(op[jj] + aoff + i * wst) : 0.f;
      }
#pragma unroll
      for (int jj = 0; jj < 4; ++jj) {
        if (!ok[jj]) continue;
#pragma unroll
        for (int i = 0; i < 4; ++i) {
          if (i >= wlim) break;
          float r = fmaf(yo[i][mr][jq * 4 + jj], osc, bv);
          if (f.accumulate) r += old[jj][i];
          if (f.prelu) r = r > 0.f ? r : sl * r;
          if ((WBF_PROBE & 8) && r != 12345.678f) continue;
          if (split_st) sbase[((op[jj] - obase) >> 1) + i * swst] = r;
          else op[jj][i * wst] = r;
          if (STATS) {
            if (cnt == 0.f) sk = r;
            const float dlt = r - sk;
            s1 += dlt;
            s2 = fmaf(dlt, dlt, s2);
            cnt += 1.f;
          }
        }
      }
    }
  }
  if (STATS) {
    WfRec w = {0.f, 0.f, 0.f};
    if (cnt > 0.f) {
      w.n = cnt;
      w.mean = sk + s1 / cnt;
      w.m2 = fmaxf(s2 - s1 * s1 / cnt, 0.f);
    }
    WfRec o;
    o.n = __shfl_xor(w.n, 32, 64);
    o.mean = __shfl_xor(w.mean, 32, 64);
    o.m2 = __shfl_xor(w.m2, 32, 64);
    w = lh == 0 ? wfrec_merge(w, o) : wfrec_merge(o, w);
    __syncthreads();
    float* sh = reinterpret_cast<float*>(lds);
    if (lh == 0) {
      float* p_ = sh + (wave * 32 + li) * 3;
      p_[0] = w.n; p_[1] = w.mean; p_[2] = w.m2;
    }
    __syncthreads();
    if (wm == 0 && lh == 0) {
      WfRec r = w;
#pragma unroll
      for (int q = 1; q < WM; ++q) {
        const float* p_ = sh + ((q * WN + wn) * 32 + li) * 3;
        WfRec e = {p_[0], p_[1], p_[2]};
        r = wfrec_merge(r, e);
      }
      float* g_ = f.stat_partial + ((long)tile_id * a.CN + co) * 3;
      g_[0] = r.n; g_[1] = r.mean; g_[2] = r.m2;
    }
  }
}

struct ToutArgs {
  const float* M;
  long m_xi;
  int ksplit;
  int N, T, LD, LH, LW, CN;
  float* dst;
  int dld;
  long dvn;
  int dvd, dvh, dvw;
  const float* bias;
  const float* prelu;
  int accumulate;
  const float* acc_src;
  const float* in_amax;
  const float* w_amax;
  int scaled;
  float* stat_partial;
};

template <int K>
__device__ __forceinline__ void at_apply(const float (&m)[8], float (&y)[4]) {
  const float s12 = m[1] + m[2], d12 = m[1] - m[2];
  const float s34 = m[3] + m[4], d34 = m[3] - m[4];
  if (K == 5) {
    const float s56 = m[5] + m[6], d56 = m[5] - m[6];
    y[0] = ((m[0] + s12) + s34) + s56;
    y[1] = (d12 + 2.f * d34) + 0.5f * d56;
    y[2] = (s12 + 4.f * s34) + 0.25f * s56;
    y[3] = ((d12 + 8.f * d34) + 0.125f * d56) + m[7];
  } else {
    y[0] = (m[0] + s12) + s34;
    y[1] = d12 + 2.f * d34;
    y[2] = s12 + 4.f * s34;
    y[3] = (d12 + 8.f * d34) + m[5];
  }
}

template <bool STATS, int K>
__global__ void __launch_bounds__(256)
wbf_tout_k(ToutArgs a) {
  constexpr int NXI = nxi_of(K);
  const int c4n = a.CN >> 2;
  float sk[4] = {0.f, 0.f, 0.f, 0.f}, s1[4] = {0.f, 0.f, 0.f, 0.f}, s2[4] = {0.f, 0.f, 0.f, 0.f};
  float cnt = 0.f;
  const float osc = a.scaled ? 1.f / (wbf_scale_of(a.in_amax) * wbf_scale_of(a.w_amax)) : 1.f;
  const long total = (long)a.N * a.T * a.LD * a.LH * c4n;
  for (long idx = (long)blockIdx.x * blockDim.x + threadIdx.x; idx < total; idx += (long)gridDim.x * blockDim.x) {
    const int c4 = (int)(idx % c4n);
    long r_ = idx / c4n;
    const int h = (int)(r_ % a.LH);
    r_ /= a.LH;
    const int d = (int)(r_ % a.LD);
    r_ /= a.LD;
    const int t = (int)(r_ % a.T);
    const int n = (int)(r_ / a.T);
    float mx[8], my[8], mz[8], mw[8];
    {
      float4 s[NXI];
#pragma unroll
      for (int xi = 0; xi < NXI; ++xi) s[xi] = *reinterpret_cast<const float4*>(a.M + (long)xi * a.m_xi + idx * 4);
      for (int z = 1; z < a.ksplit; ++z) {
        float4 q[NXI];
#pragma unroll
        for (int xi = 0; xi < NXI; ++xi) q[xi] = *reinterpret_cast<const float4*>(a.M + ((long)z * NXI + xi) * a.m_xi + idx * 4);
#pragma unroll
        for (int xi = 0; xi < NXI; ++xi) {
          s[xi].x += q[xi].x; s[xi].y += q[xi].y; s[xi].z += q[xi].z; s[xi].w += q[xi].w;
        }
      }
#pragma unroll
      for (int xi = 0; xi < 8; ++xi) {
        if (xi < NXI) {
          mx[xi] = s[xi < NXI ? xi : 0].x; my[xi] = s[xi < NXI ? xi : 0].y; mz[xi] = s[xi < NXI ? xi : 0].z; mw[xi] = s[xi < NXI ? xi : 0].w;
        } else {
          mx[xi] = my[xi] = mz[xi] = mw[xi] = 0.f;
        }
      }
    }
    float yx[4], yy[4], yz[4], yw[4];
    at_apply<K>(mx, yx);
    at_apply<K>(my, yy);
    at_apply<K>(mz, yz);
    at_apply<K>(mw, yw);
    float4 bv = make_float4(0.f, 0.f, 0.f, 0.f), sl = make_float4(1.f, 1.f, 1.f, 1.f);
    if (a.bias) bv = reinterpret_cast<const float4*>(a.bias)[c4];
    if (a.prelu) sl = reinterpret_cast<const float4*>(a.prelu)[c4];
    float* o = a.dst + ((long)n * a.dvn + (long)d * a.dvd + (long)h * a.dvh + (long)(4 * t) * a.dvw) * a.dld + c4 * 4;
    float4 old4[4];
#pragma unroll
    for (int i = 0; i < 4; ++i)
      old4[i] = (a.accumulate && 4 * t + i < a.LW) ? *reinterpret_cast<const float4*>((a.acc_src ? a.acc_src + (o - a.dst) : o) + (long)i * a.dvw * a.dld) : make_float4(0.f, 0.f, 0.f, 0.f);
#pragma unroll
    for (int i = 0; i < 4; ++i) {
      if (4 * t + i < a.LW) {
        float4* op = reinterpret_cast<float4*>(o + (long)i * a.dvw * a.dld);
        float4 r = make_float4(fmaf(yx[i], osc, bv.x), fmaf(yy[i], osc, bv.y), fmaf(yz[i], osc, bv.z), fmaf(yw[i], osc, bv.w));
        if (a.accumulate) {
          const float4 e = old4[i];
          r.x += e.x; r.y += e.y; r.z += e.z; r.w += e.w;
        }
        r.x = r.x > 0.f ? r.x : sl.x * r.x;
        r.y = r.y > 0.f ? r.y : sl.y * r.y;
        r.z = r.z > 0.f ? r.z : sl.z * r.z;
        r.w = r.w > 0.f ? r.w : sl.w * r.w;
        *op = r;
        if (STATS) {
          const float rv[4] = {r.x, r.y, r.z, r.w};
          if (cnt == 0.f) {
#pragma unroll
            for (int j = 0; j < 4; ++j) sk[j] = rv[j];
          }
#pragma unroll
          for (int j = 0; j < 4; ++j) {
            const float dlt = rv[j] - sk[j];
            s1[j] += dlt;
            s2[j] = fmaf(dlt, dlt, s2[j]);
          }
          cnt += 1.f;
        }
      }
    }
  }
  if (STATS) {
    __shared__ WfRec sh[4][256];
    const int t = threadIdx.x, vl = t / c4n, VL = 256 / c4n;
#pragma unroll
    for (int j = 0; j < 4; ++j) {
      WfRec w = {0.f, 0.f, 0.f};
      if (cnt > 0.f) {
        w.n = cnt;
        w.mean = sk[j] + s1[j] / cnt;
        w.m2 = fmaxf(s2[j] - s1[j] * s1[j] / cnt, 0.f);
      }
      sh[j][t] = w;
    }
    __syncthreads();
    for (int s_ = VL >> 1; s_ > 0; s_ >>= 1) {
      if (vl < s_) {
#pragma unroll
        for (int j = 0; j < 4; ++j) sh[j][t] = wfrec_merge(sh[j][t], sh[j][t + s_ * c4n]);
      }
      __syncthreads();
    }
    if (vl == 0) {
      const int c = (t % c4n) * 4;
#pragma unroll
      for (int j = 0; j < 4; ++j) {
        float* p_ = a.stat_partial + ((long)blockIdx.x * a.CN + c + j) * 3;
        p_[0] = sh[j][t].n;
        p_[1] = sh[j][t].mean;
        p_[2] = sh[j][t].m2;
      }
    }
  }
}

template <int MR, int WM, int WN, int TD, int TH, int K, int NP>
void launch_gemm(msk_ctx* ctx, const char* tag, const GemmArgs& a, long nblk) {
  GemmArgs b = a;
  b.nblk = (int)nblk;
  int tpb = ctx->wbf_tpb > 0 ? ctx->wbf_tpb : 1;
  while (tpb > 1 && nblk / tpb < 6L * ctx->num_cu) tpb >>= 1;
  long grid = (nblk + tpb - 1) / tpb;
  grid = (grid + 7) & ~7L;
  b.tpb = (int)((nblk + grid - 1) / grid);
  const bool deep = MR == 2 && (ctx->wbf_bpf == 4 || (ctx->wbf_bpf == 0 && nblk <= 8L * ctx->num_cu));
  if constexpr (MR == 2) {
    if (deep) {
      MSK_LAUNCH_TIMED(ctx, tag, (wbf_gemm_k<MR, WM, WN, TD, TH, K, NP, 4>), dim3((unsigned)grid), dim3(WM * WN * 64), 0, b);
      return;
    }
  }
  MSK_LAUNCH_TIMED(ctx, tag, (wbf_gemm_k<MR, WM, WN, TD, TH, K, NP>), dim3((unsigned)grid), dim3(WM * WN * 64), 0, b);
}

struct Var { int id, MR, WM, WN, TD, TH; };
const Var kVars[7] = {{4, 2, 4, 1, 16, 16}, {0, 4, 4, 1, 16, 32},
                      {5, 2, 2, 2, 8, 16},  {1, 4, 2, 2, 16, 16},
                      {3, 2, 1, 4, 8, 8},   {2, 4, 1, 4, 8, 16},
                      {6, 4, 2, 1, 16, 16}};
const Var* pick_variant(const msk_ctx* ctx, const WbfGeom& geo, int CN, int K) {
  int v0;
  if (CN == 32) v0 = 0;
  else if (CN == 64) v0 = 2;
  else if (CN >= 128 && CN % 128 == 0) v0 = 4;
  else return nullptr;
  if (K == 5 && CN == 32 && ctx->wbf_variant == 6 && wbf_tile_ok(geo, 16, 16)) return &kVars[6];
  if (K == 5 && ctx->wbf_variant < 0 && ctx->wbf_mr4 && CN >= 64) {
    const Var& m4 = kVars[v0 + 1];
    bool first = wbf_tile_ok(geo, m4.TD, m4.TH);
    if (first && CN == 64) {
      const Var& m2 = kVars[v0];
      const long tiles2 = (long)geo.T * ((geo.LD + m2.TD - 1) / m2.TD) * ((geo.LH + m2.TH - 1) / m2.TH);
      first = ctx->wbf_fuse == 0 || (ctx->wbf_fuse != 2 && tiles2 < (long)ctx->num_cu);
    }
    if (first) return &m4;
  }
  for (int c = v0; c < v0 + (K == 5 ? 2 : 1); ++c) {
    const Var& v = kVars[c];
    if (K == 5 && ctx->wbf_variant >= 0 && ctx->wbf_variant != v.id) continue;
    if (wbf_tile_ok(geo, v.TD, v.TH)) return &v;
  }
  return nullptr;
}

template <int K, int NP>
void launch_gemm_variant(msk_ctx* ctx, const char* tag, int variant, const GemmArgs& ga, long nblk) {
  switch (variant) {
    case 3: launch_gemm<2, 1, 4, 8, 8, K, NP>(ctx, tag, ga, nblk); break;
    case 4: launch_gemm<2, 4, 1, 16, 16, K, NP>(ctx, tag, ga, nblk); break;
    case 5: launch_gemm<2, 2, 2, 8, 16, K, NP>(ctx, tag, ga, nblk); break;
    default:
      if constexpr (K == 5) {
        if (variant == 6) launch_gemm<4, 2, 1, 16, 16, 5, NP>(ctx, tag, ga, nblk);
        else if (variant == 0) launch_gemm<4, 4, 1, 16, 32, 5, NP>(ctx, tag, ga, nblk);
        else if (variant == 1) launch_gemm<4, 2, 2, 16, 16, 5, NP>(ctx, tag, ga, nblk);
        else launch_gemm<4, 1, 4, 8, 16, 5, NP>(ctx, tag, ga, nblk);
      }
      break;
  }
}

struct WbfPackEntry {
  WbfPackDesc d{};
  int K = 0, NP = 0;
  size_t u_bytes = 0;
  bool live = false, valid = false;
  long last_use = 0;
};
struct WbfPackCache {
  static constexpr int kRows = 250;
  WbfPackEntry e[kRows];
  WbfPackDesc* table = nullptr;
  float* amax = nullptr;
  long epoch = 1;
};
// ... 46 lines not shown
  for (const auto& kc : kClasses) {
    WbfPackList l{};
    long most = 0;
    for (int r : rows) {
      const WbfPackEntry& e = c->e[r];
      if (e.K != kc[0] || e.NP != kc[1]) continue;
      l.row[l.n++] = (unsigned char)r;
      const long blocks = ((long)e.K * e.K * e.d.KC * 16 * e.d.CN + 255) / 256;
      if (blocks > most) most = blocks;
    }
    if (l.n == 0) continue;
    bool lds_ok = ctx->wbf_pack_lds != 0;
    long most_lds = 0;
    for (int i = 0; i < l.n && lds_ok; ++i) {
      const WbfPackDesc& dd = c->e[l.row[i]].d;
      lds_ok = dd.CK == dd.KC * 16 && dd.CN % 8 == 0 && dd.B % 4 == 0 && (((uintptr_t)dd.w) & 15) == 0 &&
               (dd.swap ? dd.B >= dd.CK : dd.B >= dd.CN);
      const long blocks = (long)dd.KC * (dd.CN / 8);
      if (blocks > most_lds) most_lds = blocks;
    }
    if (lds_ok) {
      if (most_lds > 4L * ctx->num_cu) most_lds = 4L * ctx->num_cu;
      const dim3 grid((unsigned)most_lds, (unsigned)l.n);
      if (one) l.n = -1;
      const size_t lds = (size_t)128 * kc[0] * kc[0] * kc[0] * sizeof(float);
      msk_launch_scope ls(ctx, "wbf_pack_weights");
      if (kc[0] == 5 && kc[1] == 2) hipLaunchKernelGGL((wbf_pack_weights_lds_k<5, 2>), grid, dim3(256), lds, ctx->stream, c->table, l, single);
      else if (kc[0] == 5) hipLaunchKernelGGL((wbf_pack_weights_lds_k<5, 3>), grid, dim3(256), lds, ctx->stream, c->table, l, single);
      else if (kc[1] == 2) hipLaunchKernelGGL((wbf_pack_weights_lds_k<3, 2>), grid, dim3(256), lds, ctx->stream, c->table, l, single);
      else if (kc[1] == 3) hipLaunchKernelGGL((wbf_pack_weights_lds_k<3, 3>), grid, dim3(256), lds, ctx->stream, c->table, l, single);
      else hipLaunchKernelGGL((wbf_pack_weights_lds_k<3, 1>), grid, dim3(256), lds, ctx->stream, c->table, l, single);
      MSK_LAUNCH_CHECK(ctx);
      continue;
    }
    if (most > 8L * ctx->num_cu) most = 8L * ctx->num_cu;
    const dim3 grid((unsigned)most, (unsigned)l.n);
    if (one) l.n = -1;
    msk_launch_scope ls(ctx, "wbf_pack_weights");
    if (kc[0] == 5 && kc[1] == 2) hipLaunchKernelGGL((wbf_pack_weights_k<5, 2>), grid, dim3(256), 0, ctx->stream, c->table, l, single);
    else if (kc[0] == 5) hipLaunchKernelGGL((wbf_pack_weights_k<5, 3>), grid, dim3(256), 0, ctx->stream, c->table, l, single);
    else if (kc[1] == 2) hipLaunchKernelGGL((wbf_pack_weights_k<3, 2>), grid, dim3(256), 0, ctx->stream, c->table, l, single);
    else if (kc[1] == 3) hipLaunchKernelGGL((wbf_pack_weights_k<3, 3>), grid, dim3(256), 0, ctx->stream, c->table, l, single);
    else hipLaunchKernelGGL((wbf_pack_weights_k<3, 1>), grid, dim3(256), 0, ctx->stream, c->table, l, single);
    MSK_LAUNCH_CHECK(ctx);
  }
  for (int r : rows) c->e[r].valid = true;
  return 0;
}

int pack_row_lookup(msk_ctx* ctx, WbfPackCache* c, const WbfPackDesc& key, int K, int NP, size_t u_bytes) {
  int free_row = -1, lru = -1;
  for (int r = 0; r < WbfPackCache::kRows - 1; ++r) {
    WbfPackEntry& e = c->e[r];
    if (!e.live) {
      if (free_row < 0) free_row = r;
      continue;
    }
    const WbfPackDesc& d = e.d;
    if (d.w == key.w && e.K == K && e.NP == NP && d.A == key.A && d.B == key.B && d.swap == key.swap && d.flip == key.flip &&
        d.CK == key.CK && d.CN == key.CN && d.KC == key.KC && d.tsd == key.tsd && d.tsh == key.tsh && d.tsw == key.tsw) {
      e.last_use = c->epoch;
      return r;
    }
    if (lru < 0 || e.last_use < c->e[lru].last_use) lru = r;
  }
  if (free_row < 0) {
    pack_row_drop(ctx, c->e[lru]);
    free_row = lru;
  }
  WbfPackEntry& e = c->e[free_row];
  e.d = key;
  e.K = K; e.NP = NP; e.u_bytes = u_bytes;
  if (hipMalloc((void**)&e.d.out, u_bytes) != hipSuccess) {
    msk_fail(ctx, __FILE__, __LINE__, "pack_row_lookup", "hipMalloc failed");
    return -1;
  }
  e.d.amax = c->amax + (size_t)free_row * kWbfAmaxWays;
  e.live = true; e.valid = false; e.last_use = c->epoch;
  hipLaunchKernelGGL(wbf_pack_desc_store_k, dim3(1), dim3(1), 0, ctx->stream, c->table + free_row, e.d);
  return free_row;
}

template <int MR, int WM, int WN, int TD, int TH, int K, int NP>
void launch_fused(msk_ctx* ctx, const char* tag, const FusedArgs& fa, bool stats, bool fork) {
  const dim3 grid((unsigned)(8 * fa.per_xcd));
  constexpr int NITc = 2 * NP * (TD + K - 1) * (TH + K - 1);
  if constexpr (WN == 2 && WM == 2 && NP == 2 && NITc % 64 == 0) {
    if (ctx->wbf_fused_bl == 2 && fa.g.CN == 64) {
      if (stats) MSK_LAUNCH_TIMED_F(ctx, tag, fork, (wbf_gemm_fused_k<MR, WM, WN, TD, TH, K, NP, true, 1, 2>), grid, dim3(WM * WN * 64), 0, fa);
      else MSK_LAUNCH_TIMED_F(ctx, tag, fork, (wbf_gemm_fused_k<MR, WM, WN, TD, TH, K, NP, false, 1, 2>), grid, dim3(WM * WN * 64), 0, fa);
      return;
    }
  }
  if constexpr (WN == 1 && NP == 2 && NITc % 64 == 0) {
    if (ctx->wbf_fused_bl == 2 && fa.g.CN == 32) {
      if (stats) MSK_LAUNCH_TIMED_F(ctx, tag, fork, (wbf_gemm_fused_k<MR, WM, WN, TD, TH, K, NP, true, 1, 2>), grid, dim3(WM * WN * 64), 0, fa);
      else MSK_LAUNCH_TIMED_F(ctx, tag, fork, (wbf_gemm_fused_k<MR, WM, WN, TD, TH, K, NP, false, 1, 2>), grid, dim3(WM * WN * 64), 0, fa);
      return;
    }
    if (ctx->wbf_fused_bl && fa.g.CN == 32) {
      if (stats) MSK_LAUNCH_TIMED_F(ctx, tag, fork, (wbf_gemm_fused_k<MR, WM, WN, TD, TH, K, NP, true, 1, 1>), grid, dim3(WM * WN * 64), 0, fa);
      else MSK_LAUNCH_TIMED_F(ctx, tag, fork, (wbf_gemm_fused_k<MR, WM, WN, TD, TH, K, NP, false, 1, 1>), grid, dim3(WM * WN * 64), 0, fa);
      return;
    }
  }
  if (stats) MSK_LAUNCH_TIMED_F(ctx, tag, fork, (wbf_gemm_fused_k<MR, WM, WN, TD, TH, K, NP, true>), grid, dim3(WM * WN * 64), 0, fa);
  else MSK_LAUNCH_TIMED_F(ctx, tag, fork, (wbf_gemm_fused_k<MR, WM, WN, TD, TH, K, NP, false>), grid, dim3(WM * WN * 64), 0, fa);
}
template <int K, int NP>
void launch_fused_variant(msk_ctx* ctx, const char* tag, int variant, const FusedArgs& fa, bool stats, bool fork) {
  switch (variant) {
    case 3: launch_fused<2, 1, 4, 8, 8, K, NP>(ctx, tag, fa, stats, fork); break;
    case 4: launch_fused<2, 4, 1, 16, 16, K, NP>(ctx, tag, fa, stats, fork); break;
    default: launch_fused<2, 2, 2, 8, 16, K, NP>(ctx, tag, fa, stats, fork); break;
  }
}

template <int K, int NP>
int run_pipeline(msk_ctx* ctx, const GConv& g, const float* w_canon, int A, int B, int swap, const WbfGeom& geo, const Var* bv, bool dry) {
  constexpr int NXI = nxi_of(K), NPL = 2 * NP;
  const int TD = bv->TD, TH = bv->TH, variant = bv->id;
  const int* pm = geo.perm;
  const int LD = geo.LD, LH = geo.LH, LW = geo.LW;
  const int vstr[3] = {g.DH * g.DW, g.DW, 1};
  const int tstr[3] = {K * K, K, 1};
  const int T = geo.T, KC = g.CK / 16;
  const int tiles_d = (LD + TD - 1) / TD, tiles_h = (LH + TH - 1) / TH;
  const int DP = geo.DP, HP = geo.HP;
  const int WN = bv->WN;
  const int ngrp = g.CN / (WN * 32);

  const long base_blocks = (long)NXI * ngrp * tiles_h * tiles_d * T * g.N;
  int ksplit = 1, kc_per = KC;
  if (base_blocks < 3L * ctx->num_cu && ctx->wbf_fuse != 2) {
    long want = ((long)ctx->wbf_ks_blocks * ctx->num_cu + base_blocks - 1) / base_blocks;
    if (want > KC) want = KC;
    kc_per = (int)((KC + want - 1) / want);
    ksplit = (KC + kc_per - 1) / kc_per;
  }
  const long nblk = base_blocks * ksplit;
  if (nblk > 0x7fffffffL) return 0;

  const size_t v_plane = (size_t)DP * HP * 16;
  const size_t v_xi = (size_t)g.N * T * KC * NPL * v_plane;
  const size_t m_xi = (size_t)g.N * T * LD * LH * g.CN;
  if (v_xi >= 0xFFFFFFF0ull) return 0;
  const size_t u_xi = (size_t)K * K * KC * NPL * g.CN * 16;
  if (u_xi >= 0xFFFFFFF0ull) return 0;
  if (dry) return 1;
  const bool fuse_out = ctx->wbf_fuse != 0 && ksplit == 1 && ngrp == 1 && (variant == 3 || variant == 4 || variant == 5) &&
                        NXI * u_xi <= ((size_t)3584 << 10) && (base_blocks / NXI >= 2L * ctx->num_cu || ctx->wbf_fuse == 2);
  const size_t v_bytes = (NXI * v_xi + 255) & ~(size_t)255;
  const size_t m_bytes = fuse_out ? 0 : (((size_t)ksplit * NXI * m_xi * sizeof(float) + 255) & ~(size_t)255);
  long tout_blocks = ((long)m_xi / 4 + 255) / 256;
  if (tout_blocks > 16L * ctx->num_cu) tout_blocks = 16L * ctx->num_cu;
  const int c4n = g.CN / 4;
  const bool fuse_stats = g.stats != nullptr && !g.accumulate && !g.prelu && (fuse_out || (!g.stats_ps && c4n <= 256 && (c4n & (c4n - 1)) == 0));
  const long stat_rows = fuse_out ? base_blocks / NXI : tout_blocks;
  const size_t s_bytes = fuse_stats ? (size_t)stat_rows * g.CN * 3 * sizeof(float) : 0;
  char* wsp = (char*)msk_workspace(ctx, (g.xform ? 0 : v_bytes) + m_bytes + s_bytes + 256);
  if (!wsp) return -1;
  char* V = g.xform ? (char*)g.xform + kWbfXformHeader : wsp;
  float* M = (float*)(g.xform ? wsp : wsp + v_bytes);
  float* SP = (float*)((char*)M + m_bytes);
  char* U = nullptr;
  const float* w_amax = nullptr;
  {
    WbfPackDesc key{};
    key.w = w_canon; key.A = A; key.B = B; key.swap = swap; key.flip = g.transposed ? 1 : 0; key.CK = g.CK; key.CN = g.CN; key.KC = KC;
    key.tsd = tstr[pm[0]]; key.tsh = tstr[pm[1]]; key.tsw = tstr[pm[2]];
    key.xi_stride = (long)(u_xi / 2);
    key.count = (long)K * K * K * A * B;
    WbfPackCache* c = pack_cache(ctx);
    if (!c) return -1;
    const bool cached = g.w_persistent && ctx->wbf_pack_cache != 0;
    int row;
    if (cached) {
      row = pack_row_lookup(ctx, c, key, K, NP, NXI * u_xi);
      if (row < 0) return -1;
    } else {
      row = WbfPackCache::kRows - 1;
      WbfPackEntry& e = c->e[row];
      key.out = (unsigned short*)msk_workspace2(ctx, NXI * u_xi);
      if (!key.out) return -1;
      key.amax = c->amax + (size_t)row * kWbfAmaxWays;
      e.d = key; e.K = K; e.NP = NP; e.valid = false; e.live = false;
    }
    if (!c->e[row].valid) {
      if (pack_rows_build(ctx, c, std::vector<int>{row}) != 0) return -1;
      if (!cached) c->e[row].valid = false;
    }
    U = (char*)c->e[row].d.out;
    w_amax = c->e[row].d.amax;
  }
  const float* in_amax = nullptr;
  if (NP != 3) {
    if (g.fuse) in_amax = g.fuse->amax;
    else if (g.in_amax) in_amax = g.in_amax;
    else in_amax = msk_absmax(ctx, g.src, g.sld, g.ck_real > 0 ? g.ck_real : g.CK, (long)g.N * g.SD * g.SH * g.SW, g.xform ? (float*)g.xform : nullptr);
    if (!in_amax) return -1;
  }
  float* hdr_copy = (NP != 3 && g.xform && !g.fuse && in_amax != (const float*)g.xform) ? (float*)g.xform : nullptr;

  {
    WbfTinArgs ta{};
    ta.src = g.src; ta.sld = g.sld;
    ta.svn = (long)g.DD * g.DH * g.DW; ta.svd = vstr[pm[0]]; ta.svh = vstr[pm[1]]; ta.svw = vstr[pm[2]];
    ta.N = g.N; ta.LD = LD; ta.LH = LH; ta.LW = LW; ta.T = T; ta.CK = g.CK; ta.KC = KC;
    ta.DP = DP; ta.HP = HP; ta.V = V; ta.v_xi = (long)v_xi;
    ta.amax = in_amax;
    ta.amax_copy = hdr_copy;
    ta.c_real = g.ck_real;
    if (g.fuse) {
      if (msk_wbf_transform_dual(ctx, K, NP, ta, *g.fuse, true) != 0) return -1;
      if (g.fuse->Y && ctx->wgrad_async && ctx->side != nullptr && ctx->wgrad_fork == 0) {
        hipEventRecord(ctx->ev_fork, ctx->stream);
        ctx->fork_recorded = true;
      }
    } else if (msk_wbf_transform(ctx, 0, K, NP, ta) != 0) {
      return -1;
    }
  }
  const bool fork_after = g.fuse && g.fuse->Y && ctx->wgrad_async && ctx->side != nullptr && ctx->wgrad_fork == 1 && ctx->fork_attach != 0;
  GemmArgs ga{};
  ga.V = V; ga.U = U; ga.M = M;
  ga.N = g.N; ga.T = T; ga.KC = KC; ga.CN = g.CN; ga.LD = LD; ga.LH = LH; ga.DP = DP; ga.HP = HP;
  ga.tiles_d = tiles_d; ga.tiles_h = tiles_h; ga.ngrp = ngrp; ga.ksplit = ksplit; ga.kc_per = kc_per;
  ga.v_xi = (long)v_xi; ga.v_plane = (long)v_plane; ga.u_xi = (long)u_xi; ga.m_xi = (long)m_xi;
  const char* tag = NP == 3 ? "wbf_gemm_k" : (NP == 2 ? "wbf_gemm_h2_k" : "wbf_gemm_f16_k");
  if (ctx->prof && ctx->prof_shapes) {
    char buf[200];
    snprintf(buf, sizeof(buf), "%s[ck=%d,cn=%d,n=%d,dhw=%dx%dx%d,k=%d,ks=%d%s]", tag, g.CK, g.CN, g.N, g.DD, g.DH, g.DW, K, ksplit,
             fuse_out ? ",fused" : "");
    tag = msk_intern_tag(ctx, buf);
  }
  if (fuse_out) {
    FusedArgs fa{};
    fa.g = ga;
    fa.g.nblk = (int)(base_blocks / NXI);
    fa.dst = g.dst; fa.dld = g.dld;
    fa.dvn = (long)g.DD * g.DH * g.DW; fa.dvd = vstr[pm[0]]; fa.dvh = vstr[pm[1]]; fa.dvw = vstr[pm[2]];
    fa.bias = g.bias; fa.prelu = g.prelu; fa.accumulate = g.accumulate;
    fa.acc_src = g.accumulate ? g.acc_src : nullptr;
    fa.in_amax = in_amax; fa.w_amax = w_amax; fa.scaled = NP != 3 ? 1 : 0;
    fa.stat_partial = SP;
    fa.per_xcd = (fa.g.nblk + 7) / 8;
    fa.LW = LW;
    if (g.dst_lo && g.dst_hi && g.dst_csplit > 0 && g.accumulate && g.dld == 2 * g.dst_csplit && g.CN == 2 * g.dst_csplit && !fuse_stats) {
      fa.st_lo = g.dst_lo; fa.st_hi = g.dst_hi; fa.csplit = g.dst_csplit;
      ctx->dst_split_done = true;
    }
    launch_fused_variant<K, NP>(ctx, tag, variant, fa, fuse_stats, fork_after);
    MSK_LAUNCH_CHECK(ctx);
    if (fuse_stats) {
      if (g.stats_ps) {
        const int tps = fa.g.nblk / g.N;
        for (int n = 0; n < g.N; ++n) {
          msk_bn_fin fn{};
          if (g.fin) {
            fn = *g.fin;
            const long o = (long)n * g.fin_stride;
            fn.save_mean += o; fn.save_invstd += o; fn.scale += o; fn.shift += o;
          }
          if (msk_bn_stats_merge(ctx, SP + (size_t)n * tps * g.CN * 3, tps, g.CN, g.stats + (size_t)n * 2 * g.CN, g.fin ? &fn : nullptr) != 0) return -1;
        }
      } else if (msk_bn_stats_merge(ctx, SP, fa.g.nblk, g.CN, g.stats, g.fin) != 0) {
        return -1;
      }
      ctx->stats_fused = true;
    }
    if (g.xform) ctx->xform_written = true;
    return 1;
  }
  launch_gemm_variant<K, NP>(ctx, tag, variant, ga, nblk);
  MSK_LAUNCH_CHECK(ctx);
  {
    ToutArgs oa{};
    oa.M = M; oa.m_xi = (long)m_xi; oa.ksplit = ksplit;
    oa.N = g.N; oa.T = T; oa.LD = LD; oa.LH = LH; oa.LW = LW; oa.CN = g.CN;
    oa.dst = g.dst; oa.dld = g.dld;
    oa.dvn = (long)g.DD * g.DH * g.DW; oa.dvd = vstr[pm[0]]; oa.dvh = vstr[pm[1]]; oa.dvw = vstr[pm[2]];
    oa.bias = g.bias; oa.prelu = g.prelu; oa.accumulate = g.accumulate;
    oa.acc_src = g.accumulate ? g.acc_src : nullptr;
    oa.stat_partial = SP;
    oa.in_amax = in_amax;
    oa.w_amax = w_amax;
    oa.scaled = NP != 3 ? 1 : 0;
    if (fuse_stats) MSK_LAUNCH_TIMED_F(ctx, "wbf_tout_k", false, (wbf_tout_k<true, K>), dim3((unsigned)tout_blocks), dim3(256), 0, oa);
    else MSK_LAUNCH_TIMED_F(ctx, "wbf_tout_k", fork_after, (wbf_tout_k<false, K>), dim3((unsigned)tout_blocks), dim3(256), 0, oa);
    MSK_LAUNCH_CHECK(ctx);
    if (fuse_stats) {
      if (msk_bn_stats_merge(ctx, SP, (int)tout_blocks, g.CN, g.stats, g.fin) != 0) return -1;
      ctx->stats_fused = true;
    }
  }
  if (g.xform) ctx->xform_written = true;
  return 1;
}

}

#ifndef WBF_TIN_MIN_PER
#define WBF_TIN_MIN_PER 2
#endif
static int wbf_tiles_per_group(const msk_ctx* ctx, long groups, int T) {
  const long want = ctx->wbf_tin_groups >= 0 ? ctx->wbf_tin_groups : 8L * ctx->num_cu;
  if (groups >= want || T <= WBF_TIN_MIN_PER) return T;
  long chunks = (want + groups - 1) / groups;
  int per = (int)((T + chunks - 1) / chunks);
  if (per < WBF_TIN_MIN_PER) per = WBF_TIN_MIN_PER;
  return per;
}

int msk_wbf_transform(msk_ctx* ctx, int mode, int K, int NP, const WbfTinArgs& ta_in) {
  WbfTinArgs ta = ta_in;
  ta.lane_map = ctx->wbf_tin_map;
  const int pblocks = (ta.DP * ta.HP + 63) / 64;
  ta.t_per = wbf_tiles_per_group(ctx, (long)pblocks * (ta.CK / 32) * ta.N, ta.T);
  const dim3 grid((unsigned)(pblocks * (ta.CK / 32)), ta.N, (unsigned)((ta.T + ta.t_per - 1) / ta.t_per));
  const char* tag = mode == 0 ? "wbf_tin_k" : "wbf_ty_k";
  if (ctx->prof && ctx->prof_shapes) {
    char buf[160];
    snprintf(buf, sizeof(buf), "%s[c=%d,n=%d,l=%dx%dx%d,k=%d,np=%d]", tag, ta.CK, ta.N, ta.LD, ta.LH, ta.LW, K, NP);
    tag = msk_intern_tag(ctx, buf);
  }
  msk_launch_scope ls(ctx, tag);
#define WBF_TIN_LAUNCH(M_, K_, P_) hipLaunchKernelGGL((wbf_tin_k<M_, K_, P_>), grid, dim3(256), 0, ctx->stream, ta)
  if (K == 5 && NP == 2) {
    if (mode == 0) WBF_TIN_LAUNCH(0, 5, 2);
    else WBF_TIN_LAUNCH(1, 5, 2);
  } else if (K == 5) {
    if (mode == 0) WBF_TIN_LAUNCH(0, 5, 3);
    else WBF_TIN_LAUNCH(1, 5, 3);
  } else if (NP == 2) {
    if (mode == 0) WBF_TIN_LAUNCH(0, 3, 2);
    else WBF_TIN_LAUNCH(1, 3, 2);
  } else if (NP == 3) {
    if (mode == 0) WBF_TIN_LAUNCH(0, 3, 3);
    else WBF_TIN_LAUNCH(1, 3, 3);
  } else {
    if (mode == 0) WBF_TIN_LAUNCH(0, 3, 1);
    else WBF_TIN_LAUNCH(1, 3, 1);
  }
#undef WBF_TIN_LAUNCH
  MSK_LAUNCH_CHECK(ctx);
  return 0;
}

int msk_wbf_transform_dual(msk_ctx* ctx, int K, int NP, const WbfTinArgs& ta_in, const WbfBnBwd& bn, bool write_v) {
  DualArgs da{};
  da.t = ta_in;
  da.t.lane_map = 1;
  da.y = bn.y; da.yld = bn.yld; da.dout = bn.dout; da.dld = bn.dld;
  da.scale = bn.scale; da.shift = bn.shift; da.alpha = bn.alpha; da.mean = bn.mean; da.invstd = bn.invstd; da.sums = bn.sums;
  da.invM = bn.invM; da.C = ta_in.CK; da.Y = bn.Y; da.y_xi = bn.y_xi; da.amax = bn.amax; da.maxes = bn.maxes;
  da.y_cmax = bn.Y ? bn.y_cmax : nullptr;
  da.coef_stride = bn.coef_stride; da.sums_stride = bn.sums_stride;
  da.bound_shift = ctx->dy_bound_shift;
  const bool write_y = bn.Y != nullptr;
  if (!write_v && !write_y) return 0;
  const int pblocks = (da.t.DP * da.t.HP + 63) / 64;
  da.t.t_per = wbf_tiles_per_group(ctx, (long)pblocks * (da.t.CK / 32) * da.t.N, da.t.T);
  const dim3 grid((unsigned)(pblocks * (da.t.CK / 32)), da.t.N, (unsigned)((da.t.T + da.t.t_per - 1) / da.t.t_per));
  const char* tag = write_v ? (write_y ? "wbf_tin_dual_k" : "wbf_tin_bn_k") : "wbf_ty_bn_k";
  if (ctx->prof && ctx->prof_shapes) {
    char buf[160];
    snprintf(buf, sizeof(buf), "%s[c=%d,n=%d,l=%dx%dx%d,k=%d,np=%d]", tag, da.t.CK, da.t.N, da.t.LD, da.t.LH, da.t.LW, K, NP);
    tag = msk_intern_tag(ctx, buf);
  }
  msk_launch_scope ls(ctx, tag);
#define WBF_DUAL_LAUNCH(K_, P_)                                                                                        \
  do {                                                                                                                 \
    if (write_v && write_y) hipLaunchKernelGGL((wbf_tin_dual_k<K_, P_, true, true>), grid, dim3(256), 0, ctx->stream, da);   \
// ... 126 lines not shown
```

medicalseg_amd/csrc/msk_ctx.hip:

```cpp
#include <cstdlib>

#include "msk_common.h"

thread_local std::string g_msk_global_err;

int msk_fail(msk_ctx* ctx, const char* file, int line, const char* what, const char* detail) {
  char buf[1024];
  const char* base = strrchr(file, '/');
  snprintf(buf, sizeof(buf), "%s:%d: %s: %s", base ? base + 1 : file, line, what, detail ? detail : "");
  if (ctx) ctx->err = buf;
  g_msk_global_err = buf;
  return -1;
}

static void* grow(msk_ctx* ctx, void** p, size_t* cur, size_t bytes) {
  if (bytes <= *cur) return *p;
  if (*p) {
    hipStreamSynchronize(ctx->stream);
    hipFree(*p);
    *p = nullptr;
    *cur = 0;
  }
  size_t want = bytes + (bytes >> 2);
  if (hipMalloc(p, want) != hipSuccess) {
// ... 495 lines not shown
    ctx->ks_lds = value;
    return 0;
  }
  if (strcmp(key, "dense12") == 0) {
    msk_set_dense12(value);
    return 0;
  }
  if (strcmp(key, "reduce_vpl") == 0) {
    msk_set_reduce_vpl(value);
    return 0;
  }
  if (strcmp(key, "reduce_vpl_site") == 0) {
    msk_set_reduce_vpl_site(value);
    return 0;
  }
  if (strcmp(key, "reduce_cap") == 0) {
    msk_set_ew_caps(0, value);
    return 0;
  }
  if (strcmp(key, "dy_bound_shift") == 0) {
    ctx->dy_bound_shift = value;
    return 0;
  }
  if (strcmp(key, "late_split") == 0) {
    ctx->late_split = value != 0;
    return 0;
  }
  if (strcmp(key, "c1_h2") == 0) {
    ctx->c1_h2 = value < 0 ? 0 : (value > 2 ? 2 : value);
    return 0;
  }
  if (strcmp(key, "ks_nr_max") == 0) {
    ctx->ks_nr_max = value >= 4 ? 4 : (value >= 2 ? 2 : 1);
    return 0;
  }
  if (strcmp(key, "wgrad_lds_pad") == 0) {
    ctx->wgrad_lds_pad = value > 0 ? value : 0;
    return 0;
  }
  if (strcmp(key, "kst_pair") == 0) {
    ctx->kst_pair = value != 0;
    return 0;
  }
  if (strcmp(key, "tile_staging") == 0) {
    ctx->tile_staging = value;
    return 0;
  }
  if (strcmp(key, "wgrad_renorm") == 0) {
    ctx->wgrad_renorm = value != 0;
    return 0;
  }
  if (strcmp(key, "ks_legacy") == 0) {
    ctx->ks_legacy = value;
    return 0;
  }
  if (strcmp(key, "wgrad_fork") == 0) {
    ctx->wgrad_fork = value;
    return 0;
  }
  if (strcmp(key, "wbf_fuse") == 0) {
    ctx->wbf_fuse = value;
    return 0;
  }
  if (strcmp(key, "wbf_fused_bl") == 0) {
    ctx->wbf_fused_bl = value;
    return 0;
  }
  if (strcmp(key, "wbf_tpb") == 0) {
    ctx->wbf_tpb = value > 0 ? value : 0;
    return 0;
  }
  if (strcmp(key, "conv_split") == 0) {
    ctx->conv_split = value == 2 ? 2 : 3;
    return 0;
  }
  if (strcmp(key, "bwd_fuse") == 0) {
    ctx->bwd_fuse = value < 0 ? -1 : (value > 2 ? 2 : value);
    return 0;
  }
  if (strcmp(key, "tk_join") == 0) {
    ctx->tk_join = value != 0;
    return 0;
  }
  if (strcmp(key, "foldn_wgs") == 0) {
    ctx->foldn_wgs = value > 0 ? value : 0;
    return 0;
  }
  if (strcmp(key, "wgrad_wino_rounds") == 0) {
    ctx->wgrad_wino_rounds = value > 0 ? value : 0;
    return 0;
  }
  if (strcmp(key, "wgrad_rounds") == 0) {
    ctx->wgrad_rounds = value > 0 ? value : 8;
    return 0;
  }
  if (strcmp(key, "wgrad_chunk") == 0) {
    ctx->wgrad_chunk = value;
    return 0;
  }
  if (strcmp(key, "wgrad_async") == 0) {
    if (msk_join_side_impl(ctx) != 0) return -1;
    ctx->wgrad_async = value != 0;
    return 0;
  }
  if (strcmp(key, "prof_shapes") == 0) {
    ctx->prof_shapes = value != 0;
    return 0;
  }
  if (strcmp(key, "poison_scratch") == 0) {
    ctx->poison = value;
    if (value >= 0) {
      hipStreamSynchronize(ctx->stream);
      if (ctx->ws) hipMemsetAsync(ctx->ws, value, ctx->ws_bytes, ctx->stream);
      if (ctx->ws2) hipMemsetAsync(ctx->ws2, value, ctx->ws2_bytes, ctx->stream);
    }
    return 0;
  }
  return msk_fail(ctx, __FILE__, __LINE__, "msk_set_option", "unknown key");
}

}
```

medicalseg_amd/csrc/msk_elementwise.hip:

```cpp
#include "msk_common.h"
#include "msk_wbf.h"

namespace {

constexpr int kThreads = 256;

inline int pow2ceil(int v) {
  int p = 1;
  while (p < v) p <<= 1;
  return p;
}

struct ChanGeom {
  int CB, VPB, cblocks;
};
inline ChanGeom chan_geom(int C) {
  ChanGeom g;
  g.CB = pow2ceil(C) < kThreads ? pow2ceil(C) : kThreads;
  g.VPB = kThreads / g.CB;
  g.cblocks = (C + g.CB - 1) / g.CB;
  return g;
}

#ifndef EW_LB
// ... 1101 lines not shown
    }
    if (dx) st12(dx + 12 * g, o);
    if (dres) {
      if (dres_acc) {
        float a[12];
        ld12(dres + 12 * g, a);
#pragma unroll
        for (int s = 0; s < 12; ++s) du[s] += a[s];
      }
      st12(dres + 12 * g, du);
    }
  }
  if (dx_amax) block_atomic_max(dx_amax, mx);
}

inline bool d12_ok(const msk_tensor& t) { return t.p == nullptr || (t.ld == t.c && (((uintptr_t)t.p) % 16 == 0)); }
inline bool d12_shape(const msk_tensor& x, long voxels) {
  return (x.c == 1 || x.c == 2 || x.c == 3 || x.c == 6) && (voxels * x.c) % 12 == 0;
}
int g_dense12 = 1;

inline bool vec4_ok(const msk_tensor& t) {
  return t.p == nullptr || ((t.c % 4 == 0) && (t.ld % 4 == 0) && (((uintptr_t)t.p) % 16 == 0));
}
inline int ew_blocks(long total, int num_cu) {
  long b = (total + kThreads - 1) / kThreads;
  long cap = (long)num_cu * g_ew_cap;
  if (b > cap) b = cap;
  if (b < 1) b = 1;
  return (int)b;
}
inline bool same_shape(const msk_tensor& a, const msk_tensor& b) {
  return a.n == b.n && a.d == b.d && a.h == b.h && a.w == b.w && a.c == b.c;
}

}

extern "C" {

int msk_ncdhw_to_ndhwc(msk_ctx* ctx, const float* src, msk_tensor dst) {
  long V = (long)dst.d * dst.h * dst.w;
  msk_launch_scope ls(ctx, "layout_ncdhw_to_ndhwc");
  dim3 grid(msk_cdiv(V, 32), msk_cdiv(dst.c, 32), dst.n);
  hipLaunchKernelGGL(ncdhw_to_ndhwc_k, grid, dim3(256), 0, ctx->stream, src, (float*)dst.p, dst.ld, V, dst.c);
  MSK_LAUNCH_CHECK(ctx);
  return 0;
}
int msk_ndhwc_to_ncdhw(msk_ctx* ctx, msk_tensor src, float* dst) {
  long V = (long)src.d * src.h * src.w;
  msk_launch_scope ls(ctx, "layout_ndhwc_to_ncdhw");
  dim3 grid(msk_cdiv(V, 32), msk_cdiv(src.c, 32), src.n);
  hipLaunchKernelGGL(ndhwc_to_ncdhw_k, grid, dim3(256), 0, ctx->stream, (const float*)src.p, src.ld, dst, V, src.c);
  MSK_LAUNCH_CHECK(ctx);
  return 0;
}

}

namespace {
__global__ void noop_k() {}
inline void noop_launches(msk_ctx* ctx) {
  for (int i = 0; i < ctx->noop_after_merge; ++i) hipLaunchKernelGGL(noop_k, dim3(1), dim3(64), 0, ctx->stream);
}
}

int msk_bn_stats_merge(msk_ctx* ctx, const float* partial, int nb, int C, float* stats, const msk_bn_fin* fin) {
  msk_launch_scope ls(ctx, "bn_stats_merge");
  hipLaunchKernelGGL(bn_stats_merge, dim3(C), dim3(merge_threads(nb)), 0, ctx->stream, partial, nb, C, C, stats, fin ? *fin : msk_bn_fin{});
  MSK_LAUNCH_CHECK(ctx);
  noop_launches(ctx);
  return 0;
}

int msk_join_sums_merge(msk_ctx* ctx, const float* partial, int nb, int C, float* unit_sums, float* u_dbeta, float* u_dgamma,
                        float* u_dalpha, float* dalpha) {
  msk_launch_scope ls(ctx, "sums_merge");
  hipLaunchKernelGGL(sums_merge_k, dim3(4 * C), dim3(nb > 256 ? 256 : 64), 0, ctx->stream, partial, nb, C, 4 * pow2ceil(C / 4), 4, unit_sums, 0,
                     u_dbeta, u_dgamma, u_dalpha, dalpha);
  MSK_LAUNCH_CHECK(ctx);
  noop_launches(ctx);
  return 0;
}

extern "C" {

int msk_bn_stats(msk_ctx* ctx, msk_tensor x, float* stats_local) { return msk_bn_stats_fin(ctx, x, stats_local, nullptr); }

int msk_bn_stats_fin(msk_ctx* ctx, msk_tensor x, float* stats_local, const msk_bn_fin* fin) {
  const long voxels = msk_voxels(x);
  MSK_REQUIRE(ctx, voxels > 0 && x.c > 0, "empty tensor");
  if (x.c % 4 == 0 && x.c / 4 <= kThreads && vec4_ok(x)) {
    const int QCB = pow2ceil(x.c / 4), VL = kThreads / QCB;
    const int nb = reduce_blocks(voxels, VL, ctx->num_cu, 0);
    float* partial = (float*)msk_workspace(ctx, (size_t)nb * 4 * QCB * 3 * sizeof(float));
    if (!partial) return -1;
    {
      msk_launch_scope ls(ctx, "bn_stats_partial");
      hipLaunchKernelGGL(bn_stats_partial_v4, dim3(nb), dim3(kThreads), 0, ctx->stream, (const float*)x.p, voxels, x.c,
                         x.ld, QCB, VL, partial);
      MSK_LAUNCH_CHECK(ctx);
    }
    msk_launch_scope ls(ctx, "bn_stats_merge");
    hipLaunchKernelGGL(bn_stats_merge, dim3(x.c), dim3(merge_threads(nb)), 0, ctx->stream, partial, nb, x.c, 4 * QCB, stats_local,
                       fin ? *fin : msk_bn_fin{});
    MSK_LAUNCH_CHECK(ctx);
    noop_launches(ctx);
    return 0;
  }
  ChanGeom g = chan_geom(x.c);
  int nb = reduce_blocks(voxels, g.VPB, ctx->num_cu, 0);
  size_t bytes = (size_t)g.cblocks * nb * g.CB * 3 * sizeof(float);
  float* partial = (float*)msk_workspace(ctx, bytes);
  if (!partial) return -1;
  if (g_dense12 && d12_shape(x, voxels) && d12_ok(x)) {
    const long groups = voxels * x.c / 12;
    {
      msk_launch_scope ls(ctx, "bn_stats_partial");
#define D12_ST(C_) hipLaunchKernelGGL(bn_stats_partial_d12_k<C_>, dim3(nb), dim3(kThreads), 0, ctx->stream, (const float*)x.p, groups, g.CB, partial)
      if (x.c == 1) D12_ST(1); else if (x.c == 2) D12_ST(2); else if (x.c == 3) D12_ST(3); else D12_ST(6);
#undef D12_ST
      MSK_LAUNCH_CHECK(ctx);
    }
    msk_launch_scope ls(ctx, "bn_stats_merge");
    hipLaunchKernelGGL(bn_stats_merge, dim3(x.c), dim3(merge_threads(nb)), 0, ctx->stream, partial, nb, x.c, g.CB, stats_local,
                       fin ? *fin : msk_bn_fin{});
    MSK_LAUNCH_CHECK(ctx);
    noop_launches(ctx);
    return 0;
  }
  {
    msk_launch_scope ls(ctx, "bn_stats_partial");
    hipLaunchKernelGGL(bn_stats_partial, dim3(nb, g.cblocks), dim3(kThreads), 0, ctx->stream,
                       (const float*)x.p, voxels, x.c, x.ld, g.CB, g.VPB, partial);
    MSK_LAUNCH_CHECK(ctx);
  }
  {
    msk_launch_scope ls(ctx, "bn_stats_merge");
    hipLaunchKernelGGL(bn_stats_merge, dim3(x.c), dim3(merge_threads(nb)), 0, ctx->stream, partial, nb, x.c, g.CB, stats_local,
                       fin ? *fin : msk_bn_fin{});
    MSK_LAUNCH_CHECK(ctx);
    noop_launches(ctx);
  }
  return 0;
}

int msk_bn_finalize(msk_ctx* ctx, const float* gathered, int world, double count_per_rank, int C,
                    const float* gamma, const float* beta, float eps, float momentum,
                    float* running_mean, float* running_var, float* save_mean, float* save_invstd,
                    float* scale, float* shift) {
  msk_launch_scope ls(ctx, "bn_finalize");
  hipLaunchKernelGGL(bn_finalize_k, dim3(msk_cdiv(C, 64)), dim3(64), 0, ctx->stream, gathered, world,
                     count_per_rank, C, gamma, beta, eps, momentum, running_mean, running_var, save_mean,
                     save_invstd, scale, shift);
  MSK_LAUNCH_CHECK(ctx);
  return 0;
}

int msk_bn_eval_coeffs(msk_ctx* ctx, int C, const float* gamma, const float* beta, const float* running_mean,
                       const float* running_var, float eps, float* save_mean, float* save_invstd,
                       float* scale, float* shift) {
  msk_launch_scope ls(ctx, "bn_eval_coeffs");
  hipLaunchKernelGGL(bn_eval_coeffs_k, dim3(msk_cdiv(C, 64)), dim3(64), 0, ctx->stream, C, gamma, beta,
                     running_mean, running_var, eps, save_mean, save_invstd, scale, shift);
  MSK_LAUNCH_CHECK(ctx);
  return 0;
}
// ... 597 lines not shown
```

medicalseg_amd/csrc/msk_wbf.h:

```cpp
#pragma once
#include "msk_conv.h"

typedef __bf16 bf16x8 __attribute__((ext_vector_type(8)));
typedef __bf16 bf16x2 __attribute__((ext_vector_type(2)));
typedef float f32x16 __attribute__((ext_vector_type(16)));
typedef float f32x4 __attribute__((ext_vector_type(4)));
typedef float f32x2 __attribute__((ext_vector_type(2)));

__device__ __forceinline__ void wbf_split3_pair(float x0, float x1, unsigned& hi, unsigned& mid, unsigned& lo) {
  f32x2 x = {x0, x1};
  hi = __builtin_bit_cast(unsigned, __builtin_convertvector(x, bf16x2));
  f32x2 r = {x0 - __uint_as_float(hi << 16), x1 - __uint_as_float(hi & 0xffff0000u)};
  mid = __builtin_bit_cast(unsigned, __builtin_convertvector(r, bf16x2));
  f32x2 r2 = {r.x - __uint_as_float(mid << 16), r.y - __uint_as_float(mid & 0xffff0000u)};
  lo = __builtin_bit_cast(unsigned, __builtin_convertvector(r2, bf16x2));
}

typedef _Float16 wbf_f16x2 __attribute__((ext_vector_type(2)));
__device__ __forceinline__ void wbf_split2h_pair(float x0, float x1, unsigned& hi, unsigned& lo) {
  f32x2 x = {x0, x1};
  const wbf_f16x2 h = __builtin_convertvector(x, wbf_f16x2);
  hi = __builtin_bit_cast(unsigned, h);
  const f32x2 hf = __builtin_convertvector(h, f32x2);
  f32x2 r = {x0 - hf.x, x1 - hf.y};
// ... 47 lines not shown
    if (m > 0.f) (void)atomicMax(amax + (blockIdx.x + blockIdx.y * 7u) % kWbfAmaxWays, __float_as_uint(m));
  }
}

struct WbfTinArgs {
  const float* src;
  int sld;
  long svn;
  int svd, svh, svw;
  int N, LD, LH, LW, T, CK, KC;
  int DP, HP;
  char* V;
  long v_xi;
  int lane_map;
  const float* amax;
  float* amax_copy;
  int t_per;
  int c_real;
  float* cmax;
};
__device__ __forceinline__ int wbf_chan_shift(float tensor_amax, float chan_max) {
  if (!(chan_max > 0.f) || !(tensor_amax > 0.f) || !(tensor_amax < 3.0e38f)) return 0;
  int ea, ec;
  (void)frexpf(tensor_amax, &ea);
  (void)frexpf(chan_max, &ec);
  const int s = ea - ec;
  return s < 0 ? 0 : (s > 15 ? 15 : s);
}
#ifndef WBF_CMAX_PRECHECK
#define WBF_CMAX_PRECHECK 1
#endif
__device__ __forceinline__ void wbf_cmax_commit(float* cmax, int cg, float (&mx)[8], bool wave_cg) {
  unsigned* q = reinterpret_cast<unsigned*>(cmax) + cg * 8;
#if WBF_CMAX_PRECHECK
  const bool precheck = gridDim.x * gridDim.y * gridDim.z > 1024u;
  unsigned cur[8] = {0u, 0u, 0u, 0u, 0u, 0u, 0u, 0u};
  if (precheck) {
#pragma unroll
    for (int j = 0; j < 8; ++j) cur[j] = __hip_atomic_load(q + j, __ATOMIC_RELAXED, __HIP_MEMORY_SCOPE_AGENT);
  }
#endif
#pragma unroll
  for (int j = 0; j < 8; ++j) {
    float m = mx[j];
#pragma unroll
    for (int o = 32; o >= 4; o >>= 1) m = fmaxf(m, __shfl_xor(m, o, 64));
    if (wave_cg) {
      m = fmaxf(m, __shfl_xor(m, 2, 64));
      m = fmaxf(m, __shfl_xor(m, 1, 64));
    }
    mx[j] = m;
  }
  const int lane = threadIdx.x & 63;
  if (lane < (wave_cg ? 1 : 4)) {
#if WBF_CMAX_PRECHECK
#pragma unroll
    for (int j = 0; j < 8; ++j)
      if (mx[j] > 0.f && __float_as_uint(mx[j]) > cur[j]) atomicMax(q + j, __float_as_uint(mx[j]));
#else
#pragma unroll
    for (int j = 0; j < 8; ++j)
      if (mx[j] > 0.f) atomicMax(q + j, __float_as_uint(mx[j]));
#endif
  }
}
int msk_wbf_transform(msk_ctx* ctx, int mode, int K, int NP, const WbfTinArgs& a);

struct WbfBnBwd {
  const float* y;
  int yld;
  const float* dout;
  int dld;
  const float *scale, *shift, *alpha, *mean, *invstd, *sums;
  float invM;
  char* Y;
  const float* amax;
  long y_xi;
  const float* maxes;
  float* y_cmax;
  int coef_stride;
  int sums_stride;
  int res_is_input;
};
int msk_wbf_transform_dual(msk_ctx* ctx, int K, int NP, const WbfTinArgs& a, const WbfBnBwd& bn, bool write_v);
inline int wbf_pieces(const msk_ctx* ctx, int K) { return (K == 3 && ctx->conv_fp16) ? 1 : (ctx->conv_split == 2 ? 2 : 3); }

struct WbfGeom {
  int perm[3];
  int LD, LH, LW, T;
  int DP, HP;
  double max_pad;
};
inline void wbf_min_tile(int cout, int* td, int* th) {
  *td = cout == 32 ? 16 : 8;
  *th = cout <= 64 ? 16 : 8;
}
#ifndef WBF_RAGGED_W
#define WBF_RAGGED_W 1
#endif
constexpr bool kWbfRaggedW = WBF_RAGGED_W != 0;
constexpr double kWbfMaxPad = 1.8;
constexpr double kWbfMaxPadLast = 4.0;
inline bool wbf_pick_geom(int D, int H, int W, int minTD, int minTH, WbfGeom* out) {
  static const int kPerms[6][3] = {{0, 1, 2}, {1, 0, 2}, {0, 2, 1}, {2, 0, 1}, {1, 2, 0}, {2, 1, 0}};
  const int dims[3] = {D, H, W};
  int best = -1;
  double best_cost = 0, limit = kWbfMaxPad;
  for (int pass = 0; pass < 2 && best < 0; ++pass) {
    limit = pass == 0 ? kWbfMaxPad : kWbfMaxPadLast;
    for (int i = 0; i < 6; ++i) {
      const int ld = dims[kPerms[i][0]], lh = dims[kPerms[i][1]], lw = dims[kPerms[i][2]];
      const int lw4 = (lw + 3) / 4 * 4;
      if (lw % 4 && !kWbfRaggedW) continue;
      if ((double)((ld + minTD - 1) / minTD * minTD) * ((lh + minTH - 1) / minTH * minTH) * lw4 > limit * (double)ld * lh * lw) continue;
      const double cost = (double)((ld + 7) / 8 * 8) * ((lh + 7) / 8 * 8) * lw4 / ((double)ld * lh * lw);
      if (best < 0 || cost < best_cost - 1e-9) {
        best = i;
        best_cost = cost;
      }
    }
  }
  if (best < 0) return false;
  for (int j = 0; j < 3; ++j) out->perm[j] = kPerms[best][j];
  out->LD = dims[out->perm[0]];
  out->LH = dims[out->perm[1]];
  out->LW = dims[out->perm[2]];
  out->T = (out->LW + 3) / 4;
  out->max_pad = limit;
  const int rd = out->LD >= 16 ? 16 : 8, rh = out->LH >= 32 ? 32 : (out->LH >= 16 ? 16 : 8);
  out->DP = (out->LD + rd - 1) / rd * rd + 4;
  out->HP = (out->LH + rh - 1) / rh * rh + 4;
  return true;
}
inline bool wbf_tile_ok(const WbfGeom& g, int TD, int TH) {
  const int td = (g.LD + TD - 1) / TD * TD, th = (g.LH + TH - 1) / TH * TH;
  const int lw4 = (g.LW + 3) / 4 * 4;
  return td + 4 <= g.DP && th + 4 <= g.HP && (double)td * th * lw4 <= g.max_pad * (double)g.LD * g.LH * g.LW;
}
size_t msk_wbf_xform_bytes(int n, int d, int h, int w, int c, int cout, int K, int NP);
size_t msk_wbf_fwd_xform_bytes(const msk_ctx* ctx, int n, int d, int h, int w, int c, int cout, int K);
int msk_bn_stats_merge(msk_ctx* ctx, const float* partial, int nb, int C, float* stats, const msk_bn_fin* fin = nullptr);
```

medicalseg_amd/models/vnet.py:

```python
from __future__ import annotations

import os

import numpy as np

from .. import nn
from ..cvlibs import manager
from ..device import Tensor, get_device, to_tensor
from ..nn import AddAct, ConvBNAct, copy_scale

DENSE_TWIN = os.environ.get("MSEGK_DENSE_TWIN", "1") != "0"
SPLIT_CONCAT_GRAD = os.environ.get("MSEGK_SPLIT_CONCAT_GRAD", "1") != "0"


class LUConv(nn.Layer):

    def __init__(self, nchan, elu):
        super(LUConv, self).__init__()
        self.relu1 = nn.ELU() if elu else nn.PReLU(nchan)
        self.conv1 = nn.Conv3D(nchan, nchan, kernel_size=5, padding=2)
        self.bn1 = nn.BatchNorm3D(nchan)
        self._unit = ConvBNAct(self.conv1, self.bn1, self.relu1)

    def forward(self, x):
        return self._unit.forward(x)

    def backward(self, dout):
        self._unit.backward(dout)


def _join_fusable(t, res):
    return (t.c % 4 == 0 and res.c == t.c and all(x.ld % 4 == 0 and x.ptr % 16 == 0 for x in (t, res))
            and os.environ.get("MSEGK_JOIN_FUSE", "1") != "0")


def _run_ops(ops, x, res):
    ops = list(ops)
    out = x
    for op in ops[:-1]:
        out = op(out)
    if not ops:
        return out, None
    last = ops[-1]
    if isinstance(last, LUConv) and _join_fusable(out, res):
        out = last._unit.forward(out, defer_act=True)
        return out, (last._unit if last._unit.deferred else None)
    return last(out), None


def _make_nConv(nchan, depth, elu):
    return nn.Sequential(*[LUConv(nchan, elu) for _ in range(depth)])


class InputTransition(nn.Layer):

    def __init__(self, in_channels, elu):
        super(InputTransition, self).__init__()
        self.num_features = 16
        self.in_channels = in_channels
        if self.num_features % in_channels:
            raise ValueError("in_channels must divide 16 (x.tile in the reference, vnet.py:76-78)")
        self.conv1 = nn.Conv3D(self.in_channels, self.num_features, kernel_size=5, padding=2)
        self.bn1 = nn.BatchNorm3D(self.num_features)
        self.relu1 = nn.ELU() if elu else nn.PReLU(self.num_features)
        self._unit = ConvBNAct(self.conv1, self.bn1, self.relu1)

    def forward(self, x, out=None, out2=None):
        return self._unit.forward(x, res=x, out=out, out2=out2)

    def backward(self, dout):
        self._unit.backward(dout, need_dx=False, res_needs_grad=False)


class DownTransition(nn.Layer):

    def __init__(self, inChans, nConvs, elu, dropout=False, downsample_stride=(2, 2, 2), kernel=(2, 2, 2)):
        super(DownTransition, self).__init__()
        outChans = 2 * inChans
        self.if_dropout = dropout
        self.down_conv = nn.Conv3D(inChans, outChans, kernel_size=kernel, stride=downsample_stride)
        self.bn1 = nn.BatchNorm3D(outChans)
        self.relu1 = nn.ELU() if elu else nn.PReLU(outChans)
        self.relu2 = nn.ELU() if elu else nn.PReLU(outChans)
        self.dropout = nn.Dropout3D()
        self.ops = _make_nConv(outChans, nConvs, elu)
        self._down = ConvBNAct(self.down_conv, self.bn1, self.relu1)
        self._join = AddAct(self.relu2)

    def forward(self, x, out=None):
        down = self._down.forward(x)
        self._mask = self.dropout.make_mask(down) if self.if_dropout else None
        if self._mask is not None:
            t = down.empty_like()
            copy_scale(down, self._mask, t)
        else:
            t = down
        self._dropped = t
        self._t_down = down
        t, unit = _run_ops(self.ops, t, down)
        self._t_ops = t
        return self._join.forward(t, down, unit=unit, out=out)

    def backward(self, dout):
        down = self._t_down
        ops = list(self.ops)
        self._join.backward(dout, share_b=bool(ops) and self._mask is None and ops[0]._unit.x is down)
        for op in reversed(ops):
            g = op._unit.out.grad
            op.backward(g)
        nn.materialize_grad(down)
        if self._mask is not None:
            copy_scale(self._dropped.grad, self._mask, down.grad, accumulate=True)
        self._down.backward(down.grad)


class UpTransition(nn.Layer):

    def __init__(self, inChans, outChans, nConvs, elu, dropout=False, dropout2=False,
                 upsample_stride_size=(2, 2, 2), kernel=(2, 2, 2)):
        super(UpTransition, self).__init__()
        self.up_conv = nn.Conv3DTranspose(inChans, outChans // 2, kernel_size=kernel, stride=upsample_stride_size)
        self.bn1 = nn.BatchNorm3D(outChans // 2)
        self.relu1 = nn.ELU() if elu else nn.PReLU(outChans // 2)
        self.relu2 = nn.ELU() if elu else nn.PReLU(outChans)
        self.if_dropout = dropout
        self.if_dropout2 = dropout2
        self.dropout1 = nn.Dropout3D()
        self.dropout2 = nn.Dropout3D()
        self.ops = _make_nConv(outChans, nConvs, elu)
        self.outChans = outChans
        self._up = ConvBNAct(self.up_conv, self.bn1, self.relu1)
        self._join = AddAct(self.relu2)

    def reserve_concat(self, dev, n, dims):
        self._reserved = None
        if self.if_dropout2 or os.environ.get("MSEGK_ZERO_COPY_SKIP", "1") == "0":
            return None
        half = self.outChans // 2
        xcat = Tensor.empty(dev, n, dims[0], dims[1], dims[2], self.outChans)
        if nn.PRODUCER_AMAX:
            xcat.amax = dev.amax_new()
        self._reserved = xcat
        self._reserved_skip = xcat.channel_slice(half, self.outChans)
        return self._reserved_skip

    def forward(self, x, skipx):
        dev = x.dev
        self._x, self._skip = x, skipx
        self._m1 = self.dropout1.make_mask(x) if self.if_dropout else None
        self._m2 = self.dropout2.make_mask(skipx) if self.if_dropout2 else None
        xin = x
        if self._m1 is not None:
            xin = x.empty_like()
            copy_scale(x, self._m1, xin)
        self._xin = xin
        half = self.outChans // 2
        od, oh, ow = self.up_conv.out_dims(xin)
        if (od, oh, ow) != (skipx.d, skipx.h, skipx.w) or skipx.c != self.outChans - half:
            raise ValueError(f"skip connection shape {skipx.shape} does not match the up-sampled "
                             f"({x.n}, {half}, {od}, {oh}, {ow})")
        res = getattr(self, "_reserved", None)
        self._reserved = None
        self._skip_in_place = (res is not None and self._m2 is None and skipx.ld == res.ld and
                               skipx.ptr == res.ptr + 4 * half and res.gen == dev.arena.gen)
        if self._skip_in_place:
            xcat, s_skip = res, skipx
        else:
            xcat = Tensor.empty(dev, x.n, od, oh, ow, self.outChans)
            if nn.PRODUCER_AMAX:
                xcat.amax = dev.amax_new()
            s_skip = xcat.channel_slice(half, self.outChans)
        s_up = xcat.channel_slice(0, half)
        self._up.forward(xin, out=s_up)
        if not self._skip_in_place:
            copy_scale(skipx, self._m2, s_skip)
        if xcat.amax is None or s_up.amax != xcat.amax or s_skip.amax != xcat.amax:
            xcat.amax = None
        self._xcat = xcat
        out, unit = _run_ops(self.ops, xcat, xcat)
        return self._join.forward(out, xcat, unit=unit)

    def join_for_consumer(self):
        ops = list(self.ops)
        return self._join, bool(ops) and ops[0]._unit.x is self._xcat

    def backward(self, dout):
        xcat, half = self._xcat, self.outChans // 2
        ops = list(self.ops)
        self._join.backward(dout, share_b=bool(ops) and ops[0]._unit.x is xcat)
        g_lo = g_hi = None
        skip = self._skip
        first = ops[0]._unit if ops else None
        if (first is not None and SPLIT_CONCAT_GRAD and self._skip_in_place and skip.grad is None and half * 4 < 128 and self._m1 is None):
            dev = xcat.dev
            g_lo = Tensor.empty(dev, xcat.n, xcat.d, xcat.h, xcat.w, half)
            g_hi = Tensor.empty(dev, xcat.n, xcat.d, xcat.h, xcat.w, half)
            first.dx_split = (g_lo, g_hi)
        if first is not None:
            first.dx_split_done = False
        for op in reversed(ops):
            op.backward(op._unit.out.grad)
        nn.materialize_grad(xcat)
        gcat = xcat.grad
        split_done = g_lo is not None and getattr(first, "dx_split_done", False)
        if first is not None:
            first.dx_split = None
        if split_done:
            skip.grad = g_hi
        elif self._skip_in_place and skip.grad is None:
            skip.grad = gcat.channel_slice(half, self.outChans)
        else:
            sg = skip.ensure_grad()
            copy_scale(gcat.channel_slice(half, self.outChans), self._m2, sg, accumulate=skip.grad_written)
        skip.grad_written = True
        self._up.backward(g_lo if split_done else gcat.channel_slice(0, half))
        if self._m1 is not None:
            x = self._x
            xg = x.ensure_grad()
            copy_scale(self._xin.grad, self._m1, xg, accumulate=x.grad_written)
            x.grad_written = True


class OutputTransition(nn.Layer):

    def __init__(self, in_channels, num_classes, elu):
        super(OutputTransition, self).__init__()
        self.conv1 = nn.Conv3D(in_channels, num_classes, kernel_size=5, padding=2)
        self.bn1 = nn.BatchNorm3D(num_classes)
        self.conv2 = nn.Conv3D(num_classes, num_classes, kernel_size=1)
        self.relu1 = nn.ELU() if elu else nn.PReLU(num_classes)
        self._unit = ConvBNAct(self.conv1, self.bn1, self.relu1)

    def forward(self, x):
        o = self._unit.forward(x)
        self._o = o
        return self.conv2.run_forward(o)

    def backward(self, dlogits, join=None):
        self.conv2.run_backward(self._o, dlogits, need_dx=True)
        self._unit.backward(self._o.grad, join=join)


@manager.MODELS.add_component
class VNet(nn.Layer):

    def __init__(self, elu=False, in_channels=1, num_classes=4, pretrained=None,
                 kernel_size=((2, 2, 2), (2, 2, 2), (2, 2, 2), (2, 2, 2)),
                 stride_size=((2, 2, 2), (2, 2, 2), (2, 2, 2), (2, 2, 2))):
        super().__init__()
        self.best_loss = 1000000
        self.num_classes = num_classes
        self.in_channels = in_channels

        self.in_tr = InputTransition(in_channels, elu=elu)
        self.down_tr32 = DownTransition(16, 1, elu, downsample_stride=stride_size[0], kernel=kernel_size[0])
        self.down_tr64 = DownTransition(32, 2, elu, downsample_stride=stride_size[1], kernel=kernel_size[1])
        self.down_tr128 = DownTransition(64, 3, elu, dropout=True, downsample_stride=stride_size[2],
                                         kernel=kernel_size[2])
        self.down_tr256 = DownTransition(128, 2, elu, dropout=True, downsample_stride=stride_size[3],
                                         kernel=kernel_size[3])
        self.up_tr256 = UpTransition(256, 256, 2, elu, dropout=True, dropout2=True,
                                     upsample_stride_size=stride_size[3], kernel=kernel_size[3])
        self.up_tr128 = UpTransition(256, 128, 2, elu, dropout=True, dropout2=True,
                                     upsample_stride_size=stride_size[2], kernel=kernel_size[2])
        self.up_tr64 = UpTransition(128, 64, 1, elu, upsample_stride_size=stride_size[1], kernel=kernel_size[1])
        self.up_tr32 = UpTransition(64, 32, 1, elu, upsample_stride_size=stride_size[0], kernel=kernel_size[0])
        self.out_tr = OutputTransition(32, num_classes, elu)

        self.pretrained = pretrained
        self._post_backward_hooks = []
        self._grad_ready_hooks = []
        self._build()
        self.init_weight()

    def _build(self):
        dev = get_device()
        params, frozen = [], []
        for name, p in self.named_parameters():
            p.name = name
            (frozen if getattr(p, "frozen", False) else params).append(p)
        bufs = []
        for name, p in self.named_buffers():
            p.name = name
            bufs.append(p)
# ... 90 lines not shown
```

medicalseg_amd/nn.py:

```python
from __future__ import annotations

import ctypes as C
import os
import warnings
from collections import OrderedDict

import numpy as np

from . import _lib
from ._lib import NULL_TENSOR, MskBnFin, MskConvDesc, MskError
from .device import Tensor, get_device

BN_EPS = 1e-5
BN_MOMENTUM = 0.9


def _triple(v):
    if isinstance(v, (list, tuple)):
        if len(v) != 3:
            raise ValueError(f"expected 3 values, got {v}")
        return tuple(int(i) for i in v)
    return (int(v),) * 3


# ... 457 lines not shown
                     _fp(sc["scale"]), _fp(sc["shift"]))
            dev.call("msk_conv_fold_bn", _fp(conv.weight.ptr), _fp(conv.bias.ptr), _fp(sc["scale"]), _fp(sc["shift"]),
                     conv.cout, C.c_long(conv.weight.size // conv.cout), _fp(self._fold_w), _fp(self._fold_b))
            self._fold_epoch = _FUSED_INFERENCE["epoch"]
        if out is None:
            od, oh, ow = conv.out_dims(x)
            out = Tensor.empty(dev, x.n, od, oh, ow, conv.cout)
        alpha = _act_alpha(self.act)
        dev.call("msk_conv3d_fwd_act", conv.desc(), x.msk(), _fp(self._fold_w), _fp(self._fold_b), _fp(alpha), out.msk())
        out.amax = None
        self.x, self.res, self.y, self.out, self.bn_mode = x, None, None, out, 3
        return out

    def forward(self, x: Tensor, res: Tensor | None = None, out: Tensor | None = None, defer_act=False, out2: Tensor | None = None) -> Tensor:
        dev = x.dev
        self.deferred = False
        if (_FUSED_INFERENCE["on"] and not self.bn.training and res is None and type(self.conv) is Conv3D
                and (self.act is None or isinstance(self.act, PReLU))):
            return self._forward_folded(x, out)
        self.x, self.res = x, res
        bn, sc = self.bn, self.bn.scratch(dev)
        Cn = bn.num_features
        fin = None
        multi = (dev.world > 1 or BatchNorm3D.force_collectives) and BatchNorm3D.sync and not BatchNorm3D.dry_run
        if bn.training and FUSE_SMALL and not multi:
            od, oh, ow = self.conv.out_dims(x)
            fin = MskBnFin(bn.weight.ptr, bn.bias.ptr, bn.epsilon, bn.momentum, float(x.n * od * oh * ow), bn._mean.ptr,
                           bn._variance.ptr, sc["mean"], sc["invstd"], sc["scale"], sc["shift"])
        if bn.training and type(self.conv) is Conv3D:
            y = self.conv.run_forward(x, stats_ptr=sc["stats"], keep_xform=True, fin=fin)
        elif bn.training and type(self.conv) is Conv3DTranspose and KS_STATS:
            conv = self.conv
            if x.c != conv.cin:
                raise ValueError(f"Conv3DTranspose expects {conv.cin} input channels, got {x.c}")
            od, oh, ow = conv.out_dims(x)
            y = Tensor.empty(dev, x.n, od, oh, ow, conv.cout)
            _count_flops(conv, x.n, x.d * x.h * x.w, 1)
            dev.call("msk_convT3d_fwd_ex", conv.desc(), x.msk(), _fp(conv.weight.ptr), _fp(conv.bias.ptr), y.msk(), _fp(sc["stats"]),
                     C.byref(fin) if fin is not None else None)
        else:
            y = self.conv.run_forward(x)
            if bn.training:
                if fin is not None:
                    dev.call("msk_bn_stats_fin", y.msk(), _fp(sc["stats"]), C.byref(fin))
                else:
                    dev.call("msk_bn_stats", y.msk(), _fp(sc["stats"]))
        self.y = y
        if bn.training:
            if fin is None:
                gathered, nstat = sc["stats"], 1
                if multi:
                    dev.call("msk_dp_allgather", _fp(sc["stats"]), _fp(sc["gathered"]), C.c_size_t(2 * Cn))
                    gathered, nstat = sc["gathered"], dev.world
                dev.call("msk_bn_finalize", _fp(gathered), nstat, C.c_double(y.voxels), Cn, _fp(bn.weight.ptr),
                         _fp(bn.bias.ptr), C.c_float(bn.epsilon), C.c_float(bn.momentum), _fp(bn._mean.ptr),
                         _fp(bn._variance.ptr), _fp(sc["mean"]), _fp(sc["invstd"]), _fp(sc["scale"]), _fp(sc["shift"]))
            self.bn_mode = 1
        else:
            dev.call("msk_bn_eval_coeffs", Cn, _fp(bn.weight.ptr), _fp(bn.bias.ptr), _fp(bn._mean.ptr),
                     _fp(bn._variance.ptr), C.c_float(bn.epsilon), _fp(sc["mean"]), _fp(sc["invstd"]),
                     _fp(sc["scale"]), _fp(sc["shift"]))
            self.bn_mode = 2
        if out is None:
            out = y.empty_like()
        alpha = _act_alpha(self.act)
        if defer_act and res is None and alpha is not None:
            self.deferred = True
        else:
            if isinstance(self.act, ELU):
                dev.call("msk_affine_act_fwd", y.msk(), _fp(sc["scale"]), _fp(sc["shift"]),
                         res.msk() if res is not None else NULL_TENSOR, _fp(alpha), out.msk())
                dev.call("msk_elu_fwd", out.msk(), C.c_float(self.act.alpha), out.msk())
                out.amax = None
            elif out2 is not None:
                dev.call("msk_affine_act_fwd_amax2", y.msk(), _fp(sc["scale"]), _fp(sc["shift"]),
                         res.msk() if res is not None else NULL_TENSOR, _fp(alpha), out.msk(), _amax_for(out), out2.msk())
                out2.amax = out.amax
            else:
                dev.call("msk_affine_act_fwd_amax", y.msk(), _fp(sc["scale"]), _fp(sc["shift"]),
                         res.msk() if res is not None else NULL_TENSOR, _fp(alpha), out.msk(), _amax_for(out))
        self.out = out
        return out

    def backward(self, dout: Tensor, need_dx=True, res_needs_grad=True, join=None):
        if self.bn_mode == 3:
            raise RuntimeError("backward through a forward pass run under nn.fused_inference() (BN folded into the "
                               "convolution: no pre-activation tensor was kept)")
        dev = dout.dev
        bn, sc = self.bn, self.bn.scratch(dev)
        Cn = bn.num_features
        y, res = self.y, self.res
        alpha = _act_alpha(self.act)
        if isinstance(self.act, ELU):
            g = Tensor.empty(dev, dout.n, dout.d, dout.h, dout.w, dout.c)
            dev.call("msk_elu_bwd", self.out.msk(), dout.msk(), C.c_float(self.act.alpha), g.msk(), 0)
            dout = g
        resm = res.msk() if res is not None else NULL_TENSOR
        fuse = (FUSE_BN_BACKWARD and type(self.conv) is Conv3D and res is None and self.bn_mode == 1 and need_dx
                and self.conv.cin == self.conv.cout)
        if not fuse:
            materialize_grad(self.x)
        want_maxes = fuse and Cn % 4 == 0 and y.ld % 4 == 0 and dout.ld % 4 == 0 and y.ptr % 16 == 0 and dout.ptr % 16 == 0
        pg_done = False
        maxes = sc["maxes"]
        if getattr(self, "presummed", False):
            self.presummed = False
            want_maxes = fuse
            pg_done = getattr(self, "presummed_pg", False)
            maxes = getattr(self, "presummed_maxes", None) or sc["maxes"]
        elif want_maxes and FUSE_SMALL:
            maxes = dev.amax_new(2)
            dev.call("msk_affine_act_bwd_reduce_pg", y.msk(), _fp(sc["scale"]), _fp(sc["shift"]), resm, _fp(alpha),
                     _fp(sc["mean"]), _fp(sc["invstd"]), dout.msk(), _fp(sc["sums"]), _fp(maxes), 0,
                     _fp(bn.weight.grad_ptr), _fp(bn.bias.grad_ptr), _fp(_act_alpha_grad(self.act)))
            pg_done = True
        elif want_maxes:
            dev.call("msk_affine_act_bwd_reduce_ex", y.msk(), _fp(sc["scale"]), _fp(sc["shift"]), resm, _fp(alpha),
                     _fp(sc["mean"]), _fp(sc["invstd"]), dout.msk(), _fp(sc["sums"]), _fp(sc["maxes"]))
        elif FUSE_SMALL:
            dev.call("msk_affine_act_bwd_reduce_pg", y.msk(), _fp(sc["scale"]), _fp(sc["shift"]), resm, _fp(alpha),
                     _fp(sc["mean"]), _fp(sc["invstd"]), dout.msk(), _fp(sc["sums"]), None, 0,
                     _fp(bn.weight.grad_ptr), _fp(bn.bias.grad_ptr), _fp(_act_alpha_grad(self.act)))
            pg_done = True
        else:
            dev.call("msk_affine_act_bwd_reduce", y.msk(), _fp(sc["scale"]), _fp(sc["shift"]), resm, _fp(alpha),
                     _fp(sc["mean"]), _fp(sc["invstd"]), dout.msk(), _fp(sc["sums"]))
        sums_total, m_total = sc["sums"], float(y.voxels)
        if (self.bn_mode == 1 and (dev.world > 1 or BatchNorm3D.force_collectives) and BatchNorm3D.sync
                and not BatchNorm3D.dry_run):
            dev.d2d(sc["sums_total"], sc["sums"], 2 * Cn * 4)
            dev.call("msk_dp_allreduce_stats", _fp(sc["sums_total"]), C.c_size_t(2 * Cn))
            sums_total, m_total = sc["sums_total"], float(y.voxels) * dev.world
        if not pg_done:
            dev.call("msk_affine_act_param_grads", Cn, _fp(sc["sums"]), _fp(bn.weight.grad_ptr), _fp(bn.bias.grad_ptr),
                     _fp(_act_alpha_grad(self.act)), 1)
        dy = y.empty_like()
        if (FUSE_BN_BACKWARD and FUSE_BN_BACKWARD_C1 and type(self.conv) is Conv3D and self.bn_mode == 1 and not need_dx
                and self.conv.cin == 1 and self.conv.k == (5, 5, 5) and self.conv.s == (1, 1, 1)
                and (res is None or (res.ptr == self.x.ptr and res.c == 1 and not res_needs_grad))):
            conv, x = self.conv, self.x
            rc = dev.lib.msk_conv3d_bwd_bnact_c1(dev.ctx, conv.desc(), x.msk(), y.msk(), _fp(sc["scale"]), _fp(sc["shift"]),
                                                 _fp(alpha), _fp(sc["mean"]), _fp(sc["invstd"]), resm, dout.msk(),
                                                 _fp(sums_total), C.c_double(m_total), _fp(conv.weight.grad_ptr), 1)
            if rc < 0:
                raise MskError(f"msk_conv3d_bwd_bnact_c1 failed: {_lib.last_error(dev.ctx)}")
            if rc == 0:
                _count_flops(conv, x.n, y.d * y.h * y.w, 1)
                conv._xform = None
                self.dy = None
                return
        if fuse:
            conv, x = self.conv, self.x
            xf = getattr(conv, "_xform", None)
            xfp = xf[0] if (xf is not None and xf[1] == x.ptr and xf[2] == dev.arena.gen) else None
            ybuf = None
            if xfp is not None:
                nbytes = int(dev.lib.msk_conv3d_bwd_bnact_bytes(dev.ctx, conv.desc(), x.msk(), y.msk()))
                if nbytes > 0:
                    ybuf = dev.arena.alloc(nbytes)
            dx = x.ensure_grad()
            _count_flops(conv, x.n, y.d * y.h * y.w, 2)
            split = getattr(self, "dx_split", None)
            self.dx_split, self.dx_split_done = None, False
            old = getattr(x, "grad_from", None)
            if old is not None and (old.ld != dx.ld or old.c != dx.c or x.grad_written):
                materialize_grad(x)
                old = None
            if old is not None:
                x.grad_from = None
                done = C.c_int(0)
                dev.call("msk_conv3d_bwd_bnact_acc", conv.desc(), x.msk(), _fp(conv.weight.ptr), y.msk(), _fp(sc["scale"]),
                         _fp(sc["shift"]), _fp(alpha), _fp(sc["mean"]), _fp(sc["invstd"]), _fp(bn.weight.ptr), dout.msk(),
                         _fp(sums_total), C.c_double(m_total), dy.msk(), dx.msk(), 1,
                         _fp(conv.weight.grad_ptr), 1, _fp(xfp), _fp(ybuf), _fp(maxes) if want_maxes else None,
                         old.msk(), split[0].msk() if split is not None else NULL_TENSOR,
                         split[1].msk() if split is not None else NULL_TENSOR, C.byref(done))
                self.dx_split_done = bool(done.value)
            elif split is not None and x.grad_written:
                done = C.c_int(0)
                dev.call("msk_conv3d_bwd_bnact_split", conv.desc(), x.msk(), _fp(conv.weight.ptr), y.msk(), _fp(sc["scale"]),
                         _fp(sc["shift"]), _fp(alpha), _fp(sc["mean"]), _fp(sc["invstd"]), _fp(bn.weight.ptr), dout.msk(),
                         _fp(sums_total), C.c_double(m_total), dy.msk(), dx.msk(), 1,
                         _fp(conv.weight.grad_ptr), 1, _fp(xfp), _fp(ybuf), _fp(maxes) if want_maxes else None,
                         split[0].msk(), split[1].msk(), C.byref(done))
                self.dx_split_done = bool(done.value)
            else:
                dev.call("msk_conv3d_bwd_bnact", conv.desc(), x.msk(), _fp(conv.weight.ptr), y.msk(), _fp(sc["scale"]),
                         _fp(sc["shift"]), _fp(alpha), _fp(sc["mean"]), _fp(sc["invstd"]), _fp(bn.weight.ptr), dout.msk(),
                         _fp(sums_total), C.c_double(m_total), dy.msk(), dx.msk(), 1 if x.grad_written else 0,
                         _fp(conv.weight.grad_ptr), 1, _fp(xfp), _fp(ybuf), _fp(maxes) if want_maxes else None)
            x.grad_written = True
            conv._xform = None
            self.dy = dy if ybuf is None else None
            return
        if (FUSE_BN_BACKWARD and FUSE_BN_BACKWARD_T and type(self.conv) is Conv3DTranspose and self.bn_mode == 1 and need_dx
                and res is None and not isinstance(self.act, ELU) and self.conv.cout <= 16):
            conv, x = self.conv, self.x
            dx = x.ensure_grad()
            rc = dev.lib.msk_convT3d_bwd_bnact(dev.ctx, conv.desc(), x.msk(), _fp(conv.weight.ptr), y.msk(), _fp(sc["scale"]),
                                               _fp(sc["shift"]), _fp(alpha), _fp(sc["mean"]), _fp(sc["invstd"]), dout.msk(),
                                               _fp(sums_total), C.c_double(m_total), dy.msk(), dx.msk(),
                                               1 if x.grad_written else 0, _fp(conv.weight.grad_ptr), 1)
            if rc < 0:
                raise MskError(f"msk_convT3d_bwd_bnact failed: {_lib.last_error(dev.ctx)}")
            if rc == 0:
                _count_flops(conv, x.n, x.d * x.h * x.w, 2)
                x.grad_written = True
                self.dy = dy
                return
        if (join is not None and res is None and need_dx and type(self.conv) is Conv3D and self.bn_mode == 1
                and not isinstance(self.act, ELU) and self.conv.s == (1, 1, 1)
                and join[0].backward_in_dgrad(self, join[1], dout, dy, sums_total, m_total)):
            self.dy = dy
            return
        dres = NULL_TENSOR
        dres_acc = 0
        if res is not None and res_needs_grad and res.c == y.c:
            g = res.ensure_grad()
            dres, dres_acc = g.msk(), 1 if res.grad_written else 0
            res.grad_written = True
        dya = _amax_for(dy) if type(self.conv) is Conv3D and self.conv.s == (1, 1, 1) else None
        dev.call("msk_affine_act_bwd_apply_amax", y.msk(), _fp(sc["scale"]), _fp(sc["shift"]), resm, _fp(alpha),
                 _fp(sc["mean"]), _fp(sc["invstd"]), _fp(bn.weight.ptr), dout.msk(), _fp(sums_total),
                 C.c_double(m_total), self.bn_mode, dy.msk(), dres, dres_acc, dya)
        self.dy = dy
        if self.bn_mode == 2:
            dev.call("msk_bn_bias_grad", Cn, _fp(sc["sums"]), _fp(sc["scale"]), _fp(self.conv.bias.grad_ptr), 1)
        self.conv.run_backward(self.x, dy, need_dx=need_dx, bias_grad=False)


class AddAct:

    def __init__(self, act: PReLU):
        self.act = act
        self._sums = None

    def forward(self, a: Tensor, b: Tensor, unit: "ConvBNAct | None" = None, out: Tensor | None = None) -> Tensor:
        self.a, self.b = a, b
        self._bwd_done = False
        self.unit = unit if (unit is not None and getattr(unit, "deferred", False)) else None
        if out is None:
            out = a.empty_like()
        if isinstance(self.act, ELU):
            a.dev.call("msk_affine_act_fwd", a.msk(), None, None, b.msk(), None, out.msk())
            a.dev.call("msk_elu_fwd", out.msk(), C.c_float(self.act.alpha), out.msk())
            out.amax = None
            self.out = out
            return out
        if self.unit is not None:
            u, sc = self.unit, self.unit.bn.scratch(a.dev)
            a.dev.call("msk_affine_act_join_fwd_amax", u.y.msk(), _fp(sc["scale"]), _fp(sc["shift"]), _fp(u.act._weight.ptr),
# ... 115 lines not shown
```

Measured before the change: 249.9 million.

## Fuse producer unit's BN/PReLU backward reductions into consumer dgrad epilogue

Adds a dgrad variant that, while writing dx in the Winograd output epilogue, also loads the producer unit's pre-activation and accumulates its BN/PReLU backward reductions (sum of dy, sum of dy*xhat, dalpha) plus amax values. A small merge kernel then finalizes them. The VNet blocks pass the preceding LUConv as producer so that unit can skip its own separate reduce pass over dx and y. The cost is extra y loads and registers in the fused and tout kernels, and a fallback path when the kernel does not accept the shape.

After: 249.0 million. No clear change (-0.4%).

```diff
diff --git a/include/msegk.h b/include/msegk.h
--- a/include/msegk.h
+++ b/include/msegk.h
@@ -126,6 +126,14 @@
                              msk_tensor dout, const float* sums_total, double M_total, msk_tensor dy_scratch, msk_tensor dx,
                              int dx_accumulate, float* dw, int dw_accumulate, const void* xform, void* ybuf, const float* maxes,
                              msk_tensor dx_old, msk_tensor dx_lo, msk_tensor dx_hi, int* split_done);
+int msk_conv3d_bwd_bnact_sums(msk_ctx* ctx, msk_conv_desc cd, msk_tensor x, const float* w, msk_tensor y, const float* scale,
+                              const float* shift, const float* alpha, const float* mean, const float* invstd, const float* gamma,
+                              msk_tensor dout, const float* sums_total, double M_total, msk_tensor dy_scratch, msk_tensor dx,
+                              int dx_accumulate, float* dw, int dw_accumulate, const void* xform, void* ybuf, const float* maxes,
+                              msk_tensor dx_old , msk_tensor dx_lo , msk_tensor dx_hi ,
+                              int* split_done , int pc0, msk_tensor py, const float* pscale, const float* pshift,
+                              const float* palpha, const float* pmean, const float* pinvstd, float* psums, float* pmaxes,
+                              int clear_pmaxes, float* pdgamma , float* pdbeta , float* pdalpha );
 int msk_conv3d_bwd_bnact_join(msk_ctx* ctx, msk_conv_desc cd, msk_tensor x, const float* w, msk_tensor y, const float* scale,
                               const float* shift, const float* alpha , const float* mean, const float* invstd,
                               const float* gamma, msk_tensor dout, const float* sums_total, double M_total, msk_tensor dy,
diff --git a/medicalseg_amd/_lib.py b/medicalseg_amd/_lib.py
--- a/medicalseg_amd/_lib.py
+++ b/medicalseg_amd/_lib.py
@@ -89,6 +89,8 @@
     "msk_convT3d_bwd_bnact": (_i, [_vp, _CD, _T, _vp, _T, _vp, _vp, _vp, _vp, _vp, _T, _vp, _d, _T, _T, _i, _vp, _i]),
     "msk_conv3d_bwd_bnact_split": (_i, [_vp, _CD, _T, _vp, _T, _vp, _vp, _vp, _vp, _vp, _vp, _T, _vp, _d, _T, _T, _i, _vp, _i, _vp, _vp, _vp, _T, _T, C.POINTER(_i)]),
     "msk_conv3d_bwd_bnact_acc": (_i, [_vp, _CD, _T, _vp, _T, _vp, _vp, _vp, _vp, _vp, _vp, _T, _vp, _d, _T, _T, _i, _vp, _i, _vp, _vp, _vp, _T, _T, _T, C.POINTER(_i)]),
+    "msk_conv3d_bwd_bnact_sums": (_i, [_vp, _CD, _T, _vp, _T, _vp, _vp, _vp, _vp, _vp, _vp, _T, _vp, _d, _T, _T, _i, _vp, _i, _vp, _vp, _vp, _T, _T, _T, C.POINTER(_i),
+                                       _i, _T, _vp, _vp, _vp, _vp, _vp, _vp, _vp, _i, _vp, _vp, _vp]),
     "msk_conv3d_bwd_inact": (_i, [_vp, _CD, _T, _vp, _T, _vp, _vp, _vp, _vp, _vp, _i, _T, _vp, _i, _d, _T, _i, _vp, _i, _vp, _vp, _vp]),
     "msk_conv3d_bwd_bnact_join": (_i, [_vp, _CD, _T, _vp, _T, _vp, _vp, _vp, _vp, _vp, _vp, _T, _vp, _d, _T, _vp, _vp, _i, _vp, _vp,
                                        _T, _vp, _vp, _vp, _T, _vp, _vp, _vp, _T, _i, _T, _i, _vp, _vp, _vp, _i, _vp, _vp, _vp]),
diff --git a/medicalseg_amd/csrc/msk_common.h b/medicalseg_amd/csrc/msk_common.h
--- a/medicalseg_amd/csrc/msk_common.h
+++ b/medicalseg_amd/csrc/msk_common.h
@@ -133,6 +133,7 @@
   bool host_transport = false;
   std::vector<int> host_fds;
   int rank = 0, world = 1;
+  int dgrad_sums = 1;
   int tk_join = 1;
   int num_cu = 256;
 };
diff --git a/medicalseg_amd/csrc/msk_conv.h b/medicalseg_amd/csrc/msk_conv.h
--- a/medicalseg_amd/csrc/msk_conv.h
+++ b/medicalseg_amd/csrc/msk_conv.h
@@ -1,6 +1,7 @@
 #pragma once
 #include "msk_common.h"
 struct WbfBnBwd;
+struct WbfUnitSums;
 
 struct GConv {
   const float* src;
@@ -28,6 +29,7 @@
   float* dst_hi;
   int dst_csplit;
   const float* acc_src;
+  const struct WbfUnitSums* usum;
   const float* prelu;
 };
 
diff --git a/medicalseg_amd/csrc/msk_conv.hip b/medicalseg_amd/csrc/msk_conv.hip
--- a/medicalseg_amd/csrc/msk_conv.hip
+++ b/medicalseg_amd/csrc/msk_conv.hip
@@ -1573,7 +1573,7 @@
                                  msk_tensor dout, const float* sums_total, double M_total, msk_tensor dy_scratch, msk_tensor dx,
                                  int dx_accumulate, float* dw, int dw_accumulate, const void* xform, void* ybuf, const float* maxes,
                                  int coef_stride, int sums_stride, bool fused_only, float* dx_lo = nullptr, float* dx_hi = nullptr,
-                                 int dx_csplit = 0, const float* dx_old = nullptr);
+                                 int dx_csplit = 0, const float* dx_old = nullptr, const WbfUnitSums* usum = nullptr, int usum_clear = 0);
 
 int msk_conv3d_bwd_bnact(msk_ctx* ctx, msk_conv_desc cd, msk_tensor x, const float* w, msk_tensor y, const float* scale,
                          const float* shift, const float* alpha, const float* mean, const float* invstd, const float* gamma,
@@ -1618,6 +1618,39 @@
   const int rc = conv3d_bwd_bnact_impl(ctx, cd, x, w, y, scale, shift, alpha, mean, invstd, gamma, dout, sums_total, M_total, dy_scratch, dx,
                                        dx_accumulate, dw, dw_accumulate, xform, ybuf, maxes, 0, 0, false, ok ? (float*)dx_lo.p : nullptr,
                                        ok ? (float*)dx_hi.p : nullptr, ok ? dx.c / 2 : 0, (const float*)dx_old.p);
+  if (rc == 0 && ok && ctx->dst_split_done) *split_done = 1;
+  ctx->dst_split_done = false;
+  return rc;
+}
+
+int msk_conv3d_bwd_bnact_sums(msk_ctx* ctx, msk_conv_desc cd, msk_tensor x, const float* w, msk_tensor y, const float* scale,
+                              const float* shift, const float* alpha, const float* mean, const float* invstd, const float* gamma,
+                              msk_tensor dout, const float* sums_total, double M_total, msk_tensor dy_scratch, msk_tensor dx,
+                              int dx_accumulate, float* dw, int dw_accumulate, const void* xform, void* ybuf, const float* maxes,
+                              msk_tensor dx_old, msk_tensor dx_lo, msk_tensor dx_hi, int* split_done, int pc0, msk_tensor py,
+                              const float* pscale, const float* pshift, const float* palpha, const float* pmean, const float* pinvstd,
+                              float* psums, float* pmaxes, int clear_pmaxes, float* pdgamma, float* pdbeta, float* pdalpha) {
+  if (split_done) *split_done = 0;
+  MSK_REQUIRE(ctx, dx.p && py.p && pscale && pshift && pmean && pinvstd && psums && pmaxes, "msk_conv3d_bwd_bnact_sums: the producer unit's tensors");
+  MSK_REQUIRE(ctx, py.n == dx.n && py.d == dx.d && py.h == dx.h && py.w == dx.w && pc0 >= 0 && pc0 + py.c <= dx.c,
+              "msk_conv3d_bwd_bnact_sums: the producer's pre-activation must have dx's geometry and its channels lie inside dx");
+  if (!ctx->dgrad_sums || !palpha) return 1;
+  if (dx_old.p) {
+    MSK_REQUIRE(ctx, dx_old.n == dx.n && dx_old.d == dx.d && dx_old.h == dx.h && dx_old.w == dx.w && dx_old.c == dx.c &&
+                         dx_old.ld == dx.ld && dx_old.p != dx.p, "dx_old must have the geometry and voxel stride of dx");
+    dx_accumulate = 1;
+  }
+  const bool ok = split_done && dx_lo.p && dx_hi.p && dx.c % 2 == 0 && dx_lo.c == dx.c / 2 && dx_hi.c == dx.c / 2 &&
+                  dx_lo.ld == dx.c / 2 && dx_hi.ld == dx.c / 2 && dx.ld == dx.c && msk_voxels(dx_lo) == msk_voxels(dx) &&
+                  msk_voxels(dx_hi) == msk_voxels(dx) && dx_accumulate && ctx->dst_split != 0;
+  WbfUnitSums u{};
+  u.d.y = (const float*)py.p; u.d.yld = py.ld; u.d.c0 = pc0; u.d.cu = py.c;
+  u.d.scale = pscale; u.d.shift = pshift; u.d.alpha = palpha; u.d.mean = pmean; u.d.invstd = pinvstd;
+  u.d.maxes = (unsigned*)pmaxes;
+  u.sums = psums; u.dgamma = pdgamma; u.dbeta = pdbeta; u.dalpha = pdalpha;
+  const int rc = conv3d_bwd_bnact_impl(ctx, cd, x, w, y, scale, shift, alpha, mean, invstd, gamma, dout, sums_total, M_total, dy_scratch, dx,
+                                       dx_accumulate, dw, dw_accumulate, xform, ybuf, maxes, 0, 0, false, ok ? (float*)dx_lo.p : nullptr,
+                                       ok ? (float*)dx_hi.p : nullptr, ok ? dx.c / 2 : 0, (const float*)dx_old.p, &u, clear_pmaxes);
   if (rc == 0 && ok && ctx->dst_split_done) *split_done = 1;
   ctx->dst_split_done = false;
   return rc;
@@ -1685,7 +1718,7 @@
                                  msk_tensor dout, const float* sums_total, double M_total, msk_tensor dy_scratch, msk_tensor dx,
                                  int dx_accumulate, float* dw, int dw_accumulate, const void* xform, void* ybuf, const float* maxes,
                                  int coef_stride, int sums_stride, bool fused_only, float* dx_lo, float* dx_hi, int dx_csplit,
-                                 const float* dx_old) {
+                                 const float* dx_old, const WbfUnitSums* usum, int usum_clear) {
   if (check_conv_shapes(ctx, cd, x, y, false) != 0) return -1;
   ctx->dst_split_done = false;
   if (!dx_accumulate || !dx.p) dx_old = nullptr;
@@ -1707,7 +1740,7 @@
   gw.pd = cd.pd; gw.ph = cd.ph; gw.pw = cd.pw;
   gw.dw = dw; gw.accumulate = dw_accumulate;
   gw.xform = xform;
-  if (x.c == 1 && !dx.p && !fused_only && !(per > 0 && (size_t)x.n > kChunkBytes / per)) {
+  if (x.c == 1 && !dx.p && !fused_only && !usum && !(per > 0 && (size_t)x.n > kChunkBytes / per)) {
     const int r = bwd_bnact_c1(ctx, gw, y, scale, shift, alpha, mean, invstd, dout, sums_total, M_total, 0);
     if (r <= 0) return r;
   }
@@ -1732,6 +1765,13 @@
     bn.coef_stride = coef_stride; bn.sums_stride = sums_stride;
     bn.y_xi = (long)(y_bytes / ((cd.kd == 5) ? 8 : 6));
     if (split2) g.w_amax = (const float*)xform + kWbfAmaxWays;
+    if (usum) {
+      g.usum = usum;
+      g.fuse = &bn;
+      if (!msk_gconv_wino_bf3_accepts(ctx, g)) return 1;
+      g.fuse = nullptr;
+      if (usum_clear) MSK_CHECK_HIP(ctx, hipMemsetAsync(usum->d.maxes, 0, 2 * kWbfAmaxWays * sizeof(float), ctx->stream));
+    }
 
     const bool side_on = ctx->wgrad_async && ctx->side != nullptr &&
                          (ctx->wgrad_async_max_m <= 0 || msk_voxels(y) <= ctx->wgrad_async_max_m);
@@ -1785,7 +1825,7 @@
       }
     }
   }
-  if (fused_only) return 1;
+  if (fused_only || usum) return 1;
   (void)gamma;
   if (dx_old) {
     msk_tensor so = dx;
diff --git a/medicalseg_amd/csrc/msk_conv_wbf.hip b/medicalseg_amd/csrc/msk_conv_wbf.hip
--- a/medicalseg_amd/csrc/msk_conv_wbf.hip
+++ b/medicalseg_amd/csrc/msk_conv_wbf.hip
@@ -846,6 +846,7 @@
   float* st_hi;
   int csplit;
   const float* acc_src;
+  WbfUsumDev us;
 };
 
 struct WfRec {
@@ -879,9 +880,10 @@
 #ifndef WBF_FUSED_BPF
 #define WBF_FUSED_BPF 3
 #endif
-template <int MR, int WM, int WN, int TD, int TH, int K, int NP, bool STATS, int BPF = (NP == 2 ? WBF_FUSED_BPF : 1), int BL = 0>
+template <int MR, int WM, int WN, int TD, int TH, int K, int NP, bool STATS, int BPF = (NP == 2 ? WBF_FUSED_BPF : 1), int BL = 0, bool USUM = false>
 __global__ void __launch_bounds__(WM * WN * 64, 2)
 wbf_gemm_fused_k(FusedArgs f) {
+  static_assert(!USUM || (BL == 2 && !STATS), "unit sums: pipelined form, no forward statistics");
   static_assert(WM * WN == 4 && WM * MR * 32 == TD * TH, "tile shape");
   const GemmArgs& a = f.g;
   constexpr int NT = WM * WN * 64;
@@ -1260,6 +1262,28 @@
   const long aoff = f.acc_src ? (f.acc_src - f.dst) : 0;
   const int wlim = f.LW - 4 * t;
   float sk = 0.f, s1 = 0.f, s2 = 0.f, cnt = 0.f;
+  const int ucj = co - f.us.c0;
+  const bool uact = USUM && ucj >= 0 && ucj < f.us.cu;
+  float usc = 0.f, usf = 0.f, ual = 1.f, umu = 0.f, uis = 0.f;
+  float u_du = 0.f, u_dux = 0.f, u_da = 0.f, um_du = 0.f, um_xh = 0.f;
+  if (uact) {
+    usc = f.us.scale[ucj]; usf = f.us.shift[ucj]; ual = f.us.alpha[ucj]; umu = f.us.mean[ucj]; uis = f.us.invstd[ucj];
+  }
+  const float* ysb = f.us.y + ((long)n * f.dvn + (long)(4 * t) * f.dvw) * f.us.yld;
+  const unsigned ycl = uact ? (unsigned)ucj : 0u;
+  auto load_y = [&](int ch, float (&yv)[4][4]) {
+    const int mr_ = ch >> 2, jq_ = ch & 3;
+#pragma unroll
+    for (int jj = 0; jj < 4; ++jj) {
+      int fa, fb;
+      frag_pos<TH>(jj + 8 * jq_ + 4 * lh, fa, fb);
+      const int d = tdi * TD + (wm * MR + mr_) * (32 / TH) + fa, h = thi * TH + fb;
+      const bool in = uact && d < a.LD && h < a.LH;
+      const unsigned yo_ = (unsigned)(d * f.dvd + h * f.dvh) * (unsigned)f.us.yld + ycl;
+#pragma unroll
+      for (int i = 0; i < 4; ++i) yv[jj][i] = (in && i < wlim) ? __builtin_nontemporal_load(ysb + (yo_ + (unsigned)(i * f.dvw * f.us.yld))) : 0.f;
+    }
+  };
 #pragma unroll
   for (int mr = 0; mr < MR; ++mr) {
 #pragma unroll
@@ -1293,6 +1317,7 @@
           if ((WBF_PROBE & 8) && r != 12345.678f) continue;
           if (split_st) sbase[((op[jj] - obase) >> 1) + i * swst] = r;
           else op[jj][i * wst] = r;
+          if constexpr (USUM) yo[i][mr][jq * 4 + jj] = r;
           if (STATS) {
             if (cnt == 0.f) sk = r;
             const float dlt = r - sk;
@@ -1334,6 +1359,67 @@
       float* g_ = f.stat_partial + ((long)tile_id * a.CN + co) * 3;
       g_[0] = r.n; g_[1] = r.mean; g_[2] = r.m2;
     }
+  }
+  if constexpr (USUM) {
+    float yq[2][4][4];
+    load_y(0, yq[0]);
+#pragma unroll
+    for (int ch = 0; ch < MR * 4; ++ch) {
+      __builtin_amdgcn_sched_barrier(0);
+      if (ch + 1 < MR * 4) load_y(ch + 1, yq[(ch + 1) & 1]);
+      const int mr = ch >> 2, jq = ch & 3;
+      float c_du = 0.f, c_dux = 0.f, c_da = 0.f;
+#pragma unroll
+      for (int jj = 0; jj < 4; ++jj) {
+        int fa, fb;
+        frag_pos<TH>(jj + 8 * jq + 4 * lh, fa, fb);
+        const int d = tdi * TD + (wm * MR + mr) * (32 / TH) + fa, h = thi * TH + fb;
+        if (!(uact && d < a.LD && h < a.LH)) continue;
+        float r_du = 0.f, r_dux = 0.f, r_da = 0.f;
+#pragma unroll
+        for (int i = 0; i < 4; ++i) {
+          if (i >= wlim) break;
+          const float r = yo[i][mr][jq * 4 + jj];
+          const float xv = yq[ch & 1][jj][i];
+          const float tt = fmaf(xv, usc, usf);
+          const float u = tt + 0.f;
+          float g = r;
+          if (!(u > 0.f)) {
+            g = ual * r;
+            r_da = fmaf(r, u, r_da);
+          }
+          const float xh = (xv - umu) * uis;
+          r_du += g;
+          r_dux = fmaf(g, xh, r_dux);
+          um_du = fmaxf(um_du, fabsf(g));
+          um_xh = fmaxf(um_xh, fabsf(xh));
+        }
+        c_du += r_du; c_dux += r_dux; c_da += r_da;
+      }
+      u_du += c_du; u_dux += c_dux; u_da += c_da;
+    }
+    u_du += __shfl_xor(u_du, 32, 64);
+    u_dux += __shfl_xor(u_dux, 32, 64);
+    u_da += __shfl_xor(u_da, 32, 64);
+    __syncthreads();
+    float* sh = reinterpret_cast<float*>(lds);
+    if (lh == 0) {
+      float* p_ = sh + (wave * 32 + li) * 3;
+      p_[0] = u_du; p_[1] = u_dux; p_[2] = u_da;
+    }
+    __syncthreads();
+    if (wm == 0 && lh == 0 && uact) {
+      float r0 = u_du, r1 = u_dux, r2 = u_da;
+#pragma unroll
+      for (int q = 1; q < WM; ++q) {
+        const float* p_ = sh + ((q * WN + wn) * 32 + li) * 3;
+        r0 += p_[0]; r1 += p_[1]; r2 += p_[2];
+      }
+      float* g_ = f.us.partial + (long)tile_id * 3 * f.us.cb + ucj;
+      g_[0] = r0; g_[f.us.cb] = r1; g_[2 * f.us.cb] = r2;
+    }
+    block_atomic_max(f.us.maxes, um_du);
+    block_atomic_max(f.us.maxes + kWbfAmaxWays, um_xh);
   }
 }
 
@@ -1354,6 +1440,7 @@
   const float* w_amax;
   int scaled;
   float* stat_partial;
+  WbfUsumDev us;
 };
 
 template <int K>
@@ -1374,11 +1461,23 @@
   }
 }
 
-template <bool STATS, int K>
+template <bool STATS, int K, bool USUM = false>
 __global__ void __launch_bounds__(256)
 wbf_tout_k(ToutArgs a) {
   constexpr int NXI = nxi_of(K);
   const int c4n = a.CN >> 2;
+  const int uc = (int)(threadIdx.x % c4n) * 4 - a.us.c0;
+  const bool uact = USUM && uc >= 0 && uc < a.us.cu;
+  float4 usc = make_float4(0.f, 0.f, 0.f, 0.f), usf = usc, ual = usc, umu = usc, uis = usc;
+  float u_du[4] = {0.f, 0.f, 0.f, 0.f}, u_dux[4] = {0.f, 0.f, 0.f, 0.f}, u_da[4] = {0.f, 0.f, 0.f, 0.f};
+  float um_du = 0.f, um_xh = 0.f;
+  if (uact) {
+    usc = *reinterpret_cast<const float4*>(a.us.scale + uc);
+    usf = *reinterpret_cast<const float4*>(a.us.shift + uc);
+    ual = *reinterpret_cast<const float4*>(a.us.alpha + uc);
+    umu = *reinterpret_cast<const float4*>(a.us.mean + uc);
+    uis = *reinterpret_cast<const float4*>(a.us.invstd + uc);
+  }
   float sk[4] = {0.f, 0.f, 0.f, 0.f}, s1[4] = {0.f, 0.f, 0.f, 0.f}, s2[4] = {0.f, 0.f, 0.f, 0.f};
   float cnt = 0.f;
   const float osc = a.scaled ? 1.f / (wbf_scale_of(a.in_amax) * wbf_scale_of(a.w_amax)) : 1.f;
@@ -1428,6 +1527,13 @@
 #pragma unroll
     for (int i = 0; i < 4; ++i)
       old4[i] = (a.accumulate && 4 * t + i < a.LW) ? *reinterpret_cast<const float4*>((a.acc_src ? a.acc_src + (o - a.dst) : o) + (long)i * a.dvw * a.dld) : make_float4(0.f, 0.f, 0.f, 0.f);
+    float4 y4[4];
+    if constexpr (USUM) {
+      const float* yp = a.us.y + ((long)n * a.dvn + (long)d * a.dvd + (long)h * a.dvh + (long)(4 * t) * a.dvw) * a.us.yld + uc;
+#pragma unroll
+      for (int i = 0; i < 4; ++i)
+        y4[i] = (uact && 4 * t + i < a.LW) ? *reinterpret_cast<const float4*>(yp + (long)i * a.dvw * a.us.yld) : make_float4(0.f, 0.f, 0.f, 0.f);
+    }
 #pragma unroll
     for (int i = 0; i < 4; ++i) {
       if (4 * t + i < a.LW) {
@@ -1442,6 +1548,28 @@
         r.z = r.z > 0.f ? r.z : sl.z * r.z;
         r.w = r.w > 0.f ? r.w : sl.w * r.w;
         *op = r;
+        if constexpr (USUM) {
+          if (uact) {
+            const float dv[4] = {r.x, r.y, r.z, r.w}, xv[4] = {y4[i].x, y4[i].y, y4[i].z, y4[i].w};
+            const float sc_[4] = {usc.x, usc.y, usc.z, usc.w}, sf_[4] = {usf.x, usf.y, usf.z, usf.w}, al_[4] = {ual.x, ual.y, ual.z, ual.w};
+            const float mu_[4] = {umu.x, umu.y, umu.z, umu.w}, is_[4] = {uis.x, uis.y, uis.z, uis.w};
+#pragma unroll
+            for (int j = 0; j < 4; ++j) {
+              const float tt = fmaf(xv[j], sc_[j], sf_[j]);
+              const float u = tt + 0.f;
+              float g = dv[j];
+              if (!(u > 0.f)) {
+                g = al_[j] * dv[j];
+                u_da[j] = fmaf(dv[j], u, u_da[j]);
+              }
+              const float xh = (xv[j] - mu_[j]) * is_[j];
+              u_du[j] += g;
+              u_dux[j] = fmaf(g, xh, u_dux[j]);
+              um_du = fmaxf(um_du, fabsf(g));
+              um_xh = fmaxf(um_xh, fabsf(xh));
+            }
+          }
+        }
         if (STATS) {
           const float rv[4] = {r.x, r.y, r.z, r.w};
           if (cnt == 0.f) {
@@ -1490,6 +1618,33 @@
         p_[2] = sh[j][t].m2;
       }
     }
+  }
+  if constexpr (USUM) {
+    __shared__ float ush[12][256];
+    const int t = threadIdx.x, vl = t / c4n, VL = 256 / c4n;
+#pragma unroll
+    for (int j = 0; j < 4; ++j) {
+      ush[j][t] = u_du[j];
+      ush[4 + j][t] = u_dux[j];
+      ush[8 + j][t] = u_da[j];
+    }
+    __syncthreads();
+    for (int s_ = VL >> 1; s_ > 0; s_ >>= 1) {
+      if (vl < s_) {
+#pragma unroll
+        for (int k = 0; k < 12; ++k) ush[k][t] += ush[k][t + s_ * c4n];
+      }
+      __syncthreads();
+    }
+    if (vl == 0 && uact) {
+      float* p_ = a.us.partial + (long)blockIdx.x * 3 * a.us.cb + uc;
+#pragma unroll
+      for (int q = 0; q < 3; ++q)
+#pragma unroll
+        for (int j = 0; j < 4; ++j) p_[q * a.us.cb + j] = ush[q * 4 + j][t];
+    }
+    block_atomic_max(a.us.maxes, um_du);
+    block_atomic_max(a.us.maxes + kWbfAmaxWays, um_xh);
   }
 }
 
@@ -1702,9 +1857,20 @@
 }
 
 template <int MR, int WM, int WN, int TD, int TH, int K, int NP>
+constexpr bool kFusedUsum = K == 5 && NP == 2 && ((WM == 2 && WN == 2) || WN == 1) && (2 * NP * (TD + K - 1) * (TH + K - 1)) % 64 == 0;
+bool wbf_fused_usum_ok(const msk_ctx* ctx, int K, int NP, int variant, int CN) {
+  return K == 5 && NP == 2 && ctx->wbf_fused_bl == 2 && ((variant == 4 && CN == 32) || (variant == 5 && CN == 64));
+}
+template <int MR, int WM, int WN, int TD, int TH, int K, int NP>
 void launch_fused(msk_ctx* ctx, const char* tag, const FusedArgs& fa, bool stats, bool fork) {
   const dim3 grid((unsigned)(8 * fa.per_xcd));
   constexpr int NITc = 2 * NP * (TD + K - 1) * (TH + K - 1);
+  if constexpr (kFusedUsum<MR, WM, WN, TD, TH, K, NP>) {
+    if (fa.us.y && !stats && ctx->wbf_fused_bl == 2 && fa.g.CN == WN * 32) {
+      MSK_LAUNCH_TIMED_F(ctx, tag, fork, (wbf_gemm_fused_k<MR, WM, WN, TD, TH, K, NP, false, 1, 2, true>), grid, dim3(WM * WN * 64), 0, fa);
+      return;
+    }
+  }
   if constexpr (WN == 2 && WM == 2 && NP == 2 && NITc % 64 == 0) {
     if (ctx->wbf_fused_bl == 2 && fa.g.CN == 64) {
       if (stats) MSK_LAUNCH_TIMED_F(ctx, tag, fork, (wbf_gemm_fused_k<MR, WM, WN, TD, TH, K, NP, true, 1, 2>), grid, dim3(WM * WN * 64), 0, fa);
@@ -1767,22 +1933,43 @@
   if (v_xi >= 0xFFFFFFF0ull) return 0;
   const size_t u_xi = (size_t)K * K * KC * NPL * g.CN * 16;
   if (u_xi >= 0xFFFFFFF0ull) return 0;
-  if (dry) return 1;
   const bool fuse_out = ctx->wbf_fuse != 0 && ksplit == 1 && ngrp == 1 && (variant == 3 || variant == 4 || variant == 5) &&
                         NXI * u_xi <= ((size_t)3584 << 10) && (base_blocks / NXI >= 2L * ctx->num_cu || ctx->wbf_fuse == 2);
-  const size_t v_bytes = (NXI * v_xi + 255) & ~(size_t)255;
-  const size_t m_bytes = fuse_out ? 0 : (((size_t)ksplit * NXI * m_xi * sizeof(float) + 255) & ~(size_t)255);
   long tout_blocks = ((long)m_xi / 4 + 255) / 256;
   if (tout_blocks > 16L * ctx->num_cu) tout_blocks = 16L * ctx->num_cu;
   const int c4n = g.CN / 4;
+  const WbfUnitSums* us = g.usum;
+  int us_cb = 0;
+  if (us) {
+    const WbfUsumDev& ud = us->d;
+    if (!ctx->dgrad_sums || (fuse_out ? ctx->dgrad_sums == 3 : ctx->dgrad_sums == 2) || g.stats || g.prelu || !ud.y || !ud.alpha || ud.c0 < 0 || ud.cu <= 0 || ud.c0 % 4 || ud.cu % 4 || ud.c0 + ud.cu > g.CN ||
+        ud.yld % 4 || (((uintptr_t)ud.y) & 15) || (((uintptr_t)ud.scale | (uintptr_t)ud.shift | (uintptr_t)ud.alpha | (uintptr_t)ud.mean | (uintptr_t)ud.invstd) & 15))
+      return 0;
+    if (fuse_out ? !wbf_fused_usum_ok(ctx, K, NP, variant, g.CN) : !(c4n <= 256 && (c4n & (c4n - 1)) == 0)) return 0;
+    if (fuse_out && (size_t)g.DD * g.DH * g.DW * ud.yld * sizeof(float) >= 0xFFFFFFF0ull) return 0;
+    us_cb = 4;
+    while (us_cb < ud.cu) us_cb <<= 1;
+  }
+  if (dry) return 1;
+  const size_t v_bytes = (NXI * v_xi + 255) & ~(size_t)255;
+  const size_t m_bytes = fuse_out ? 0 : (((size_t)ksplit * NXI * m_xi * sizeof(float) + 255) & ~(size_t)255);
   const bool fuse_stats = g.stats != nullptr && !g.accumulate && !g.prelu && (fuse_out || (!g.stats_ps && c4n <= 256 && (c4n & (c4n - 1)) == 0));
   const long stat_rows = fuse_out ? base_blocks / NXI : tout_blocks;
   const size_t s_bytes = fuse_stats ? (size_t)stat_rows * g.CN * 3 * sizeof(float) : 0;
-  char* wsp = (char*)msk_workspace(ctx, (g.xform ? 0 : v_bytes) + m_bytes + s_bytes + 256);
+  const long us_rows = fuse_out ? base_blocks / NXI : tout_blocks;
+  const size_t us_bytes = us ? (size_t)us_rows * 3 * us_cb * sizeof(float) : 0;
+  char* wsp = (char*)msk_workspace(ctx, (g.xform ? 0 : v_bytes) + m_bytes + s_bytes + us_bytes + 256);
   if (!wsp) return -1;
   char* V = g.xform ? (char*)g.xform + kWbfXformHeader : wsp;
   float* M = (float*)(g.xform ? wsp : wsp + v_bytes);
   float* SP = (float*)((char*)M + m_bytes);
+  float* UP = (float*)((char*)SP + s_bytes);
+  WbfUsumDev usd{};
+  if (us) {
+    usd = us->d;
+    usd.cb = us_cb;
+    usd.partial = UP;
+  }
   char* U = nullptr;
   const float* w_amax = nullptr;
   {
@@ -1850,9 +2037,11 @@
   const char* tag = NP == 3 ? "wbf_gemm_k" : (NP == 2 ? "wbf_gemm_h2_k" : "wbf_gemm_f16_k");
   if (ctx->prof && ctx->prof_shapes) {
     char buf[200];
-    snprintf(buf, sizeof(buf), "%s[ck=%d,cn=%d,n=%d,dhw=%dx%dx%d,k=%d,ks=%d%s]", tag, g.CK, g.CN, g.N, g.DD, g.DH, g.DW, K, ksplit,
-             fuse_out ? ",fused" : "");
+    snprintf(buf, sizeof(buf), "%s%s[ck=%d,cn=%d,n=%d,dhw=%dx%dx%d,k=%d,ks=%d%s]", tag, (us && fuse_out) ? "_usum" : "", g.CK, g.CN, g.N, g.DD, g.DH,
+             g.DW, K, ksplit, fuse_out ? ",fused" : "");
     tag = msk_intern_tag(ctx, buf);
+  } else if (us && fuse_out) {
+    tag = NP == 3 ? "wbf_gemm_k_usum" : (NP == 2 ? "wbf_gemm_h2_k_usum" : "wbf_gemm_f16_k_usum");
   }
   if (fuse_out) {
     FusedArgs fa{};
@@ -1870,8 +2059,10 @@
       fa.st_lo = g.dst_lo; fa.st_hi = g.dst_hi; fa.csplit = g.dst_csplit;
       ctx->dst_split_done = true;
     }
+    fa.us = usd;
     launch_fused_variant<K, NP>(ctx, tag, variant, fa, fuse_stats, fork_after);
     MSK_LAUNCH_CHECK(ctx);
+    if (us && msk_unit_sums_merge(ctx, UP, (int)us_rows, usd.cu, us_cb, us->sums, us->dbeta, us->dgamma, us->dalpha) != 0) return -1;
     if (fuse_stats) {
       if (g.stats_ps) {
         const int tps = fa.g.nblk / g.N;
@@ -1906,9 +2097,12 @@
     oa.in_amax = in_amax;
     oa.w_amax = w_amax;
     oa.scaled = NP != 3 ? 1 : 0;
-    if (fuse_stats) MSK_LAUNCH_TIMED_F(ctx, "wbf_tout_k", false, (wbf_tout_k<true, K>), dim3((unsigned)tout_blocks), dim3(256), 0, oa);
+    oa.us = usd;
+    if (us) MSK_LAUNCH_TIMED_F(ctx, "wbf_tout_k_usum", fork_after, (wbf_tout_k<false, K, true>), dim3((unsigned)tout_blocks), dim3(256), 0, oa);
+    else if (fuse_stats) MSK_LAUNCH_TIMED_F(ctx, "wbf_tout_k", false, (wbf_tout_k<true, K>), dim3((unsigned)tout_blocks), dim3(256), 0, oa);
     else MSK_LAUNCH_TIMED_F(ctx, "wbf_tout_k", fork_after, (wbf_tout_k<false, K>), dim3((unsigned)tout_blocks), dim3(256), 0, oa);
     MSK_LAUNCH_CHECK(ctx);
+    if (us && msk_unit_sums_merge(ctx, UP, (int)tout_blocks, usd.cu, us_cb, us->sums, us->dbeta, us->dgamma, us->dalpha) != 0) return -1;
     if (fuse_stats) {
       if (msk_bn_stats_merge(ctx, SP, (int)tout_blocks, g.CN, g.stats, g.fin) != 0) return -1;
       ctx->stats_fused = true;
diff --git a/medicalseg_amd/csrc/msk_ctx.hip b/medicalseg_amd/csrc/msk_ctx.hip
--- a/medicalseg_amd/csrc/msk_ctx.hip
+++ b/medicalseg_amd/csrc/msk_ctx.hip
@@ -601,6 +601,10 @@
     ctx->tk_join = value != 0;
     return 0;
   }
+  if (strcmp(key, "dgrad_sums") == 0) {
+    ctx->dgrad_sums = value < 0 || value > 3 ? 1 : value;
+    return 0;
+  }
   if (strcmp(key, "foldn_wgs") == 0) {
     ctx->foldn_wgs = value > 0 ? value : 0;
     return 0;
diff --git a/medicalseg_amd/csrc/msk_elementwise.hip b/medicalseg_amd/csrc/msk_elementwise.hip
--- a/medicalseg_amd/csrc/msk_elementwise.hip
+++ b/medicalseg_amd/csrc/msk_elementwise.hip
@@ -1207,6 +1207,15 @@
   return 0;
 }
 
+int msk_unit_sums_merge(msk_ctx* ctx, const float* partial, int nb, int C, int CB, float* sums, float* dbeta, float* dgamma, float* dalpha) {
+  msk_launch_scope ls(ctx, "sums_merge");
+  hipLaunchKernelGGL(sums_merge_k, dim3(3 * C), dim3(nb > 256 ? 256 : 64), 0, ctx->stream, partial, nb, C, CB, 3, sums, 0, dbeta, dgamma, dalpha,
+                     (float*)nullptr);
+  MSK_LAUNCH_CHECK(ctx);
+  noop_launches(ctx);
+  return 0;
+}
+
 extern "C" {
 
 int msk_bn_stats(msk_ctx* ctx, msk_tensor x, float* stats_local) { return msk_bn_stats_fin(ctx, x, stats_local, nullptr); }
diff --git a/medicalseg_amd/csrc/msk_wbf.h b/medicalseg_amd/csrc/msk_wbf.h
--- a/medicalseg_amd/csrc/msk_wbf.h
+++ b/medicalseg_amd/csrc/msk_wbf.h
@@ -153,6 +153,19 @@
   int sums_stride;
   int res_is_input;
 };
+struct WbfUsumDev {
+  const float* y;
+  int yld, c0, cu, cb;
+  const float *scale, *shift, *alpha, *mean, *invstd;
+  float* partial;
+  unsigned* maxes;
+};
+struct WbfUnitSums {
+  WbfUsumDev d;
+  float* sums;
+  float *dgamma, *dbeta, *dalpha;
+};
+int msk_unit_sums_merge(msk_ctx* ctx, const float* partial, int nb, int C, int CB, float* sums, float* dbeta, float* dgamma, float* dalpha);
 int msk_wbf_transform_dual(msk_ctx* ctx, int K, int NP, const WbfTinArgs& a, const WbfBnBwd& bn, bool write_v);
 inline int wbf_pieces(const msk_ctx* ctx, int K) { return (K == 3 && ctx->conv_fp16) ? 1 : (ctx->conv_split == 2 ? 2 : 3); }
 
diff --git a/medicalseg_amd/models/vnet.py b/medicalseg_amd/models/vnet.py
--- a/medicalseg_amd/models/vnet.py
+++ b/medicalseg_amd/models/vnet.py
@@ -25,8 +25,8 @@
     def forward(self, x):
         return self._unit.forward(x)
 
-    def backward(self, dout):
-        self._unit.backward(dout)
+    def backward(self, dout, producer=None):
+        self._unit.backward(dout, producer=producer)
 
 
 def _join_fusable(t, res):
@@ -46,6 +46,18 @@
         out = last._unit.forward(out, defer_act=True)
         return out, (last._unit if last._unit.deferred else None)
     return last(out), None
+
+
+def _producer_of(ops, k, first_unit, first_x):
+    if not isinstance(ops[k], LUConv):
+        return None
+    x = ops[k]._unit.x
+    if k > 0:
+        prev = ops[k - 1]
+        return (prev._unit, 0) if isinstance(prev, LUConv) and prev._unit.out is x else None
+    if first_unit is None or x is not first_x or first_unit.out is None or first_unit.out.ptr != x.ptr:
+        return None
+    return first_unit, 0
 
 
 def _make_nConv(nchan, depth, elu):
@@ -105,9 +117,10 @@
         down = self._t_down
         ops = list(self.ops)
         self._join.backward(dout, share_b=bool(ops) and self._mask is None and ops[0]._unit.x is down)
-        for op in reversed(ops):
+        for k in range(len(ops) - 1, -1, -1):
+            op = ops[k]
             g = op._unit.out.grad
-            op.backward(g)
+            op.backward(g, producer=_producer_of(ops, k, self._down if self._mask is None else None, down))
         nn.materialize_grad(down)
         if self._mask is not None:
             copy_scale(self._dropped.grad, self._mask, down.grad, accumulate=True)
@@ -198,8 +211,8 @@
             first.dx_split = (g_lo, g_hi)
         if first is not None:
             first.dx_split_done = False
-        for op in reversed(ops):
-            op.backward(op._unit.out.grad)
+        for k in range(len(ops) - 1, -1, -1):
+            ops[k].backward(ops[k]._unit.out.grad, producer=_producer_of(ops, k, self._up, xcat))
         nn.materialize_grad(xcat)
         gcat = xcat.grad
         split_done = g_lo is not None and getattr(first, "dx_split_done", False)
diff --git a/medicalseg_amd/nn.py b/medicalseg_amd/nn.py
--- a/medicalseg_amd/nn.py
+++ b/medicalseg_amd/nn.py
@@ -563,7 +563,21 @@
         self.out = out
         return out
 
-    def backward(self, dout: Tensor, need_dx=True, res_needs_grad=True, join=None):
+    def _sums_producer(self, producer, x, dev):
+        unit, c0 = producer
+        if getattr(dev.lib.msk_conv3d_bwd_bnact_sums, "missing", False):
+            warnings.warn(f"{_lib.LIB_PATH} does not export msk_conv3d_bwd_bnact_sums: every unit keeps its own reduce pass; "
+                          "rebuild with ./build.sh", RuntimeWarning)
+            return None
+        multi = dev.world > 1 and BatchNorm3D.sync and not BatchNorm3D.dry_run
+        y = unit.y
+        if (not FUSE_SMALL or multi or unit.bn_mode != 1 or unit.res is not None or not isinstance(unit.act, PReLU)
+                or getattr(unit, "presummed", False) or y is None or (y.n, y.d, y.h, y.w) != (x.n, x.d, x.h, x.w)
+                or c0 % 4 or y.c % 4 or c0 + y.c > x.c or y.ld % 4 or y.ptr % 16):
+            return None
+        return unit, c0
+
+    def backward(self, dout: Tensor, need_dx=True, res_needs_grad=True, join=None, producer=None):
         if self.bn_mode == 3:
             raise RuntimeError("backward through a forward pass run under nn.fused_inference() (BN folded into the "
                                "convolution: no pre-activation tensor was kept)")
@@ -647,7 +661,34 @@
             if old is not None and (old.ld != dx.ld or old.c != dx.c or x.grad_written):
                 materialize_grad(x)
                 old = None
-            if old is not None:
+            pu = self._sums_producer(producer, x, dev) if producer is not None else None
+            rc_sums = 1
+            if pu is not None:
+                unit, c0 = pu
+                usc = unit.bn.scratch(dev)
+                mx = dev.amax_new(2)
+                acc = old is not None or x.grad_written
+                sp = split if (split is not None and acc) else None
+                done = C.c_int(0)
+                rc_sums = dev.lib.msk_conv3d_bwd_bnact_sums(
+                    dev.ctx, conv.desc(), x.msk(), _fp(conv.weight.ptr), y.msk(), _fp(sc["scale"]), _fp(sc["shift"]), _fp(alpha),
+                    _fp(sc["mean"]), _fp(sc["invstd"]), _fp(bn.weight.ptr), dout.msk(), _fp(sums_total), C.c_double(m_total),
+                    dy.msk(), dx.msk(), 1 if acc else 0, _fp(conv.weight.grad_ptr), 1, _fp(xfp), _fp(ybuf),
+                    _fp(maxes) if want_maxes else None, old.msk() if old is not None else NULL_TENSOR,
+                    sp[0].msk() if sp is not None else NULL_TENSOR, sp[1].msk() if sp is not None else NULL_TENSOR, C.byref(done),
+                    c0, unit.y.msk(), _fp(usc["scale"]), _fp(usc["shift"]), _fp(_act_alpha(unit.act)), _fp(usc["mean"]),
+                    _fp(usc["invstd"]), _fp(usc["sums"]), _fp(mx), 0, _fp(unit.bn.weight.grad_ptr), _fp(unit.bn.bias.grad_ptr),
+                    _fp(_act_alpha_grad(unit.act)))
+                if rc_sums < 0:
+                    raise MskError(f"msk_conv3d_bwd_bnact_sums failed: {_lib.last_error(dev.ctx)}")
+                if rc_sums == 0:
+                    if old is not None:
+                        x.grad_from = None
+                    self.dx_split_done = bool(done.value)
+                    unit.presummed, unit.presummed_pg, unit.presummed_maxes = True, True, mx
+            if rc_sums == 0:
+                pass
+            elif old is not None:
                 x.grad_from = None
                 done = C.c_int(0)
                 dev.call("msk_conv3d_bwd_bnact_acc", conv.desc(), x.msk(), _fp(conv.weight.ptr), y.msk(), _fp(sc["scale"]),
```
